# cl-volume-renderer/cl-volume-renderer

Hardware: AMD Instinct MI355X
Metric: msamples_per_sec (higher is better)
Workload: dtype f32

## Files before the change

### cl_volume_renderer_amd/csrc/bounce_device.hpp

```cpp
#pragma once
#include "render_device.hpp"

namespace clvr {

__device__ __forceinline__ VolumePacked make_volume(const RenderArgs &a) {
  return VolumePacked{a.grec, a.stepb, a.volume_lin, a.sdf_lin, a.X, a.Y, a.Z, a.NBX, a.NBY};
}

__device__ __forceinline__ uint32_t udivmod24(uint32_t n, uint32_t d, uint32_t &rem) {
  uint32_t q = (uint32_t)((float)n * __builtin_amdgcn_rcpf((float)d));
  uint32_t qd;
  asm("v_mul_u32_u24 %0, %1, %2" : "=v"(qd) : "v"(q), "v"(d));
  int32_t r = (int32_t)(n - qd);
  if (r < 0) { q -= 1u; r += (int32_t)d; }
  if (r >= (int32_t)d) { q += 1u; r -= (int32_t)d; }
  rem = (uint32_t)r;
  return q;
}

__device__ __forceinline__ unsigned prefix_count(unsigned long long mask) {
  return __builtin_amdgcn_mbcnt_hi((unsigned)(mask >> 32), __builtin_amdgcn_mbcnt_lo((unsigned)mask, 0u));
}
__device__ __forceinline__ unsigned lane_id() { return prefix_count(~0ull); }

enum : int { ST_IDLE = 0, ST_MARCH = 1, ST_CERT = 2, ST_EVENT = 8 };
enum : int { EV_START = 3,
             EV_HIT_COLOR_PENDING = 4,
             EV_CHECK = 5 };
constexpr int kCertNever = 255;

template <int MODE>
__device__ __forceinline__ void finish_item(const RenderArgs &a, int64_t entry, uint32_t hit, uint32_t gx, uint32_t gy,
                                            uint32_t bv_r, uint32_t bv_g, uint32_t bv_b) {
  const uint32_t cr = (bv_r / 2u) & 0xFFFFu, cg = (bv_g / 2u) & 0xFFFFu, cb = (bv_b / 2u) & 0xFFFFu;
  if (MODE == CLWH_ACCUM_VOXEL_CACHE && a.grants == nullptr) {
    cache_add(a.cache, entry, cr, cg, cb, 0u);
  } else {
    const unsigned long long packed = (unsigned long long)cr | ((unsigned long long)cg << 16) |
                                      ((unsigned long long)cb << 32) | (1ull << 48);
    atomicAdd(a.delta + hit, packed);
  }
  if (a.contrib_out) {
    uint32_t *q = a.contrib_out + ((size_t)gy * (size_t)a.launch_w + gx) * 4;
    q[0] = cr; q[1] = cg; q[2] = cb; q[3] = 1u;
  }
}

constexpr int kFixupDwords = 32;

__device__ __forceinline__ bool certify_exit(const RenderArgs &a, f3 p, f3 d, int budget, int &away) {
  const unsigned cx = min((unsigned)(int)p.x >> a.macro_shift, (unsigned)a.MNX - 1u), cy = min((unsigned)(int)p.y >> a.macro_shift, (unsigned)a.MNY - 1u),
                 cz = min((unsigned)(int)p.z >> a.macro_shift, (unsigned)a.MNZ - 1u);
  const unsigned octant = (d.x < 0.0f ? 1u : 0u) | (d.y < 0.0f ? 2u : 0u) | (d.z < 0.0f ? 4u : 0u);
  const int entry = a.macro[(((cz * (unsigned)a.MNY + cy) * (unsigned)a.MNX + cx) << 3) | octant];
  const bool refused = (entry & (int)kCertRefused) != 0;
  const int box_min = refused ? 0 : entry;
  away = refused ? ((entry & 0x7F) - 1) << a.macro_shift : 0;
  const float dmin = fminf(fminf(fabsf(d.x), fabsf(d.y)), fabsf(d.z));
  const float dsum = d.x + d.y + d.z;
  const float T = (float)((budget - 5) * box_min);
  const float fx = d.x < 0.0f ? p.x : (float)a.X - p.x, fy = d.y < 0.0f ? p.y : (float)a.Y - p.y, fz = d.z < 0.0f ? p.z : (float)a.Z - p.z;
  const bool leaves = T * fabsf(d.x) >= fx || T * fabsf(d.y) >= fy || T * fabsf(d.z) >= fz;
  return box_min != 0 && budget > 5 && leaves && dmin >= 0.0009765625f && dsum == dsum;
}
__device__ __forceinline__ bool certify_exit(const RenderArgs &a, f3 p, f3 d, int budget) {
  int away;
  return certify_exit(a, p, d, budget, away);
}

template <int SMALL>
__device__ __forceinline__ void index_tables_to_lds(VolumePacked &vol, const RenderArgs &a, int threads) {
  extern __shared__ uint32_t lds_parts[];
  if (SMALL == 2) {
    vol.parts = lds_parts;
    vol.parts_y0 = a.X;
    vol.parts_z0 = a.X + a.Y;
    for (int k = (int)threadIdx.x; k < a.X + a.Y + a.Z; k += threads)
      lds_parts[k] = k < a.X ? vol.part_x<1>((unsigned)k) : (k < a.X + a.Y ? vol.part_y<1>((unsigned)(k - a.X)) : vol.part_z<1>((unsigned)(k - a.X - a.Y)));
  }
}
__device__ __forceinline__ unsigned home_queue_of(const RenderArgs &a, unsigned waves_per_block) {
  unsigned home_queue = (unsigned)__builtin_amdgcn_s_getreg((3 << 11) | 20) & 7u;
  if (a.unit_affinity == 1) home_queue = (blockIdx.x * waves_per_block + (threadIdx.x >> 6)) & 7u;
  if (a.unit_affinity == 2) home_queue = 0u;
  return home_queue;
}

#ifdef CLVR_BOUNCE_STATS
constexpr bool kBounceStats = true;
#else
constexpr bool kBounceStats = false;
#endif
template <bool ON> struct BounceStatsT;
template <> struct BounceStatsT<false> {
  __device__ void step(int) {}
  __device__ void cert_begin(int, int) {}
  __device__ void cert_end(int, int) {}
  __device__ void closing_half(int) {}
  __device__ void event_phase(int) {}
  __device__ void refill(uint32_t) {}
  __device__ void fresh_items(int, int) {}
  __device__ void swap_point() {}
  template <bool TWO_RAYS> __device__ void flush(uint32_t *) {}
};
template <> struct BounceStatsT<true> {
  uint32_t step_iters = 0, step_lanes = 0, event_phases = 0, event_lanes = 0, refills = 0, refill_lanes = 0;
  uint32_t ev_kind[4] = {0, 0, 0, 0};
  uint32_t cert_phases = 0, cert_lanes = 0, cert_granted = 0;
  uint32_t step_idle = 0;
  uint32_t swaps = 0;
  uint32_t closing = 0, marching_before = 0;
  __device__ __forceinline__ void step(int st) {
    step_iters += 1; step_lanes += (uint32_t)__popcll(__ballot(st == ST_MARCH));
    step_idle += (uint32_t)__popcll(__ballot(st == ST_IDLE));
  }
  __device__ __forceinline__ void cert_begin(int st, int n_cert) {
    cert_phases += 1; cert_lanes += (uint32_t)n_cert;
    marching_before = (uint32_t)__popcll(__ballot(st == ST_MARCH));
  }
  __device__ __forceinline__ void cert_end(int st, int n_cert) { cert_granted += (uint32_t)(n_cert - (__popcll(__ballot(st == ST_MARCH)) - (int)marching_before)); }
  __device__ __forceinline__ void closing_half(int st) {
    closing = (uint32_t)__popcll(__ballot(st >= ST_EVENT));
    event_lanes += closing;
    ev_kind[1] += (uint32_t)__popcll(__ballot(st == ST_EVENT + EV_EXIT || st == ST_EVENT + EV_CHECK));
    ev_kind[2] += (uint32_t)__popcll(__ballot(st == ST_EVENT + EV_HIT || st == ST_EVENT + EV_HIT_COLOR_PENDING));
    ev_kind[3] += (uint32_t)__popcll(__ballot(st == ST_EVENT + EV_NONE));
  }
  __device__ __forceinline__ void event_phase(int st) {
    if (__ballot(st >= ST_EVENT) != 0ull) { event_phases += 1; event_lanes += (uint32_t)__popcll(__ballot(st >= ST_EVENT)); }
  }
  __device__ __forceinline__ void refill(uint32_t count) { refills += 1; refill_lanes += count; }
  __device__ __forceinline__ void fresh_items(int st, int o) {
    const uint32_t n_fresh = (uint32_t)__popcll(__ballot(st == ST_EVENT + EV_START && o == 1));
    ev_kind[0] += n_fresh; event_lanes += n_fresh;
    if (closing + n_fresh != 0u) event_phases += 1;
  }
  __device__ __forceinline__ void swap_point() { swaps += 1; }
  template <bool TWO_RAYS> __device__ __forceinline__ void flush(uint32_t *counters) {
    atomicAdd(&counters[CTR_STEP_ITERS], step_iters); atomicAdd(&counters[CTR_STEP_LANES], step_lanes);
    atomicAdd(&counters[CTR_EVENT_PHASES], event_phases); atomicAdd(&counters[CTR_EVENT_LANES], event_lanes);
    atomicAdd(&counters[CTR_REFILLS], refills); atomicAdd(&counters[CTR_REFILL_LANES], refill_lanes);
    if (TWO_RAYS) { atomicAdd(&counters[CTR_SWAPS], swaps); return; }
    for (int k = 0; k < 4; ++k) atomicAdd(&counters[CTR_EV_KIND + k], ev_kind[k]);
    atomicAdd(&counters[CTR_CERT_PHASES], cert_phases); atomicAdd(&counters[CTR_CERT_LANES], cert_lanes);
    atomicAdd(&counters[CTR_CERT_GRANTED], cert_granted); atomicAdd(&counters[CTR_STEP_IDLE], step_idle);
  }
};
using BounceStats = BounceStatsT<kBounceStats>;

}
```

### cl_volume_renderer_amd/csrc/clwh_context.hip

```cpp
#include <algorithm>
#include <cstdio>
#include <cstdlib>
#include <cstring>
#include <mutex>
#include <new>

#include "clwh_host.hpp"

using namespace clvr;

static thread_local int g_last_hip_error = 0;
void clvr::note_hip_error(hipError_t e) { g_last_hip_error = (int)e; }

static std::atomic<uint64_t> g_content_version{0};
static std::mutex g_cells_mutex;
static std::map<const void *, std::weak_ptr<VersionCell>> g_version_cells;
void clwh_touch(clwh_mem *m) { m->cell->v.store(++g_content_version, std::memory_order_relaxed); }

static std::shared_ptr<VersionCell> version_cell_of(const void *dptr) {
  std::lock_guard<std::mutex> lock(g_cells_mutex);
  auto it = g_version_cells.find(dptr);
  if (it != g_version_cells.end())
    if (auto live = it->second.lock()) return live;
  auto cell = std::make_shared<VersionCell>();
  g_version_cells[dptr] = cell;
  if (g_version_cells.size() > 4096) {
    for (auto i = g_version_cells.begin(); i != g_version_cells.end();)
      i = i->second.expired() ? g_version_cells.erase(i) : std::next(i);
  }
  return cell;
}

static size_t elem_size(int kind) {
  switch (kind) {
    case CLWH_ELEM_S8: case CLWH_ELEM_U8: return 1;
    case CLWH_ELEM_S16: case CLWH_ELEM_U16: return 2;
    case CLWH_ELEM_S32: case CLWH_ELEM_U32: case CLWH_ELEM_F32: return 4;
    default: return 0;
  }
}


void clvr::tf_to_dev(const clwh_tf &tf, TfDev &d) {
  std::memset(&d, 0, sizeof d);
  d.n = tf.n;
  for (int k = 0; k < tf.n; ++k) {
    const clwh_tf_rule &r = tf.rules[k];
    TfRuleDev &o = d.rules[k];
    o.v_lo = r.v_lo; o.v_hi = r.v_hi; o.g_lo = r.g_lo; o.g_hi = r.g_hi;
    o.flags = (r.use_gradient ? TF_USE_GRADIENT : 0u) | (r.writes_color ? TF_WRITES_COLOR : 0u) |
              (r.terminal ? TF_TERMINAL : 0u);
    o.color = ((uint32_t)r.color[0] & 255u) | (((uint32_t)r.color[1] & 255u) << 8) |
              (((uint32_t)r.color[2] & 255u) << 16) | (((uint32_t)r.color[3] & 255u) << 24);
    if (r.use_gradient) d.uses_gradient = 1;
  }
  for (int k = 0; k < tf.n && !d.uses_gradient; ++k) {
    const clwh_tf_rule &r = tf.rules[k];
    if (r.v_lo <= 0 && 0 <= r.v_hi) { d.border_class = k + 1; break; }
    if (r.terminal) break;
  }
}

int clvr::jit_for_source(clwh_ctx *ctx, const char *source, std::shared_ptr<JitTf> &out) {
  auto it = ctx->classes.cache.find(source);
  if (it != ctx->classes.cache.end()) {
    out = it->second;
    return CLWH_OK;
  }
  auto j = std::make_shared<JitTf>();
  j->source = source;
  std::string log;
  const int rc = tf_jit_compile(source, j->code, log);
  if (rc != CLWH_OK) {
    if (!log.empty()) std::fprintf(stderr, "clwhip: transfer-function source is neither in the rule grammar nor compilable:\n%s\n", log.c_str());
    return rc;
  }
  ctx->classes.cache[source] = j;
  out = j;
  return CLWH_OK;
}

int clvr::ensure_classes(clwh_ctx *ctx, const std::shared_ptr<JitTf> &jit, const clwh_mem *volume, TfDev &tf_out, const uint8_t **cls_out) {
  TfClasses &c = ctx->classes;
  if (c.cls.ptr && c.vol == volume->dptr && c.vol_ver == volume->version() && c.source == jit->source) {
    tf_out = c.tf;
    *cls_out = c.cls.as<uint8_t>();
    return CLWH_OK;
  }
  if (!jit->module) {
    HIP_TRY(hipModuleLoadData(&jit->module, jit->code.data()));
    HIP_TRY(hipModuleGetFunction(&jit->classify, jit->module, "clvr_tf_classify"));
  }
  const size_t voxels = volume->dims[0] * volume->dims[1] * volume->dims[2];
  CLWH_TRY(c.cls.reserve(ctx->stream, voxels));
  constexpr int kColors = CLWH_TF_MAX_RULES;
  CLWH_TRY(c.palette.reserve(ctx->stream, (kColors + 2) * sizeof(unsigned long long)));
  unsigned long long *palette = c.palette.as<unsigned long long>();
  HIP_TRY(hipMemsetAsync(palette, 0xFF, kColors * sizeof(unsigned long long), ctx->stream));
  HIP_TRY(hipMemsetAsync(palette + kColors, 0, 2 * sizeof(unsigned long long), ctx->stream));
  const void *vol = volume->dptr;
  int X = (int)volume->dims[0], Y = (int)volume->dims[1], Z = (int)volume->dims[2], max_colors = kColors;
  unsigned char *cls = c.cls.as<unsigned char>();
  int *error = reinterpret_cast<int *>(palette + kColors);
  int *border = reinterpret_cast<int *>(palette + kColors + 1);
  void *args[] = {&vol, &X, &Y, &Z, &cls, &palette, &max_colors, &error, &border};
  const size_t blocks = std::min<size_t>((voxels + 255u) / 256u, (size_t)1u << 23);
  HIP_TRY(hipModuleLaunchKernel(jit->classify, (unsigned)blocks, 1, 1, 256, 1, 1, 0, ctx->stream, args, nullptr));
  unsigned long long host[kColors + 2];
  HIP_TRY(hipMemcpyAsync(host, palette, sizeof host, hipMemcpyDeviceToHost, ctx->stream));
  HIP_TRY(hipStreamSynchronize(ctx->stream));
  c.vol = nullptr;
  if ((int)(host[kColors] & 0xFFFFFFFFull) != 0) return CLWH_ERR_TF_UNSUPPORTED;
  TfDev t;
  std::memset(&t, 0, sizeof t);
  t.opaque = 1;
  for (int k = 0; k < kColors && host[k] != ~0ull; ++k) {
    t.rules[k].flags = (host[k] >> 32) & 1ull ? TF_WRITES_COLOR : 0u;
    t.rules[k].color = (uint32_t)(host[k] & 0xFFFFFFFFull);
    t.n = k + 1;
  }
  t.border_class = (int32_t)(host[kColors + 1] & 0xFFull);
  c.tf = t;
  c.vol = volume->dptr;
  c.vol_ver = volume->version();
  c.source = jit->source;
  tf_out = t;
  *cls_out = cls;
  return CLWH_OK;
}


Tuning clvr::tuning_from_environment() {
  Tuning t;
  auto clamped = [](const char *e, int lo, int hi) { return std::max(lo, std::min(hi, std::atoi(e))); };
  if (const char *e = std::getenv("CLWH_TUNE_STEP")) t.step_min_lanes = clamped(e, 0, 64);
  if (const char *e = std::getenv("CLWH_TUNE_REFILL")) t.refill_min_lanes = clamped(e, 0, 64);
  if (const char *e = std::getenv("CLWH_TUNE_LITERAL_GRADIENT")) t.literal_gradient = std::atoi(e) != 0;
  if (const char *e = std::getenv("CLWH_TUNE_AFFINITY")) t.unit_affinity = std::atoi(e);
  if (const char *e = std::getenv("CLWH_TUNE_QUEUES")) t.unit_queues = clamped(e, 1, 8);
  if (const char *e = std::getenv("CLWH_TUNE_GROUP")) t.unit_group = std::max(1, std::atoi(e));
  if (const char *e = std::getenv("CLWH_TUNE_CHUNK_BLOCK_LOG2")) t.unit_block_log2 = clamped(e, 0, 8);
  if (const char *e = std::getenv("CLWH_TUNE_BLOCKS")) t.bounce_max_blocks = (uint32_t)std::max(1, std::atoi(e));
  if (const char *e = std::getenv("CLWH_TUNE_MACRO_SHIFT")) t.macro_shift = std::atoi(e);
  if (const char *e = std::getenv("CLWH_TUNE_LONG_LAUNCH")) t.force_long_launch = std::atoi(e) != 0;
  if (const char *e = std::getenv("CLWH_TUNE_BOUNCE_RAYS")) t.bounce_rays = std::atoi(e) == 2 ? 2 : 1;
  if (const char *e = std::getenv("CLWH_TUNE_SDF")) t.sdf_front = std::strcmp(e, "front") == 0;
  if (const char *e = std::getenv("CLWH_TUNE_SLICE_COARSE")) t.slice_coarse = std::atoi(e) != 0;
  if (const char *e = std::getenv("CLWH_TUNE_SDFBIT_WAVES")) t.sdfbit_waves = std::atoi(e) == 16 ? 16 : 8;
  if (const char *e = std::getenv("CLWH_TUNE_SDFBIT_GRID")) t.sdfbit_grid = std::max(1, std::atoi(e));
  if (const char *e = std::getenv("CLWH_TUNE_SDFBIT_REC")) t.sdfbit_rec_lds = std::strcmp(e, "lds") == 0 ? 1 : 0;
  if (const char *e = std::getenv("CLWH_TUNE_CERT")) t.cert_min_step = clamped(e, 0, 127);
  if (const char *e = std::getenv("CLWH_TUNE_CERT_HINT")) t.cert_hint = std::atoi(e) != 0;
  return t;
}

int clvr::check_device_flags(clwh_ctx *ctx) {
  PassScratch &p = ctx->pass;
  if (!p.fixup_overflow_pending || !p.sticky_flags.ptr) return CLWH_OK;
  uint32_t flag = 0;
  HIP_TRY(hipMemcpyAsync(&flag, p.sticky_flags.ptr, sizeof flag, hipMemcpyDeviceToHost, ctx->stream));
  HIP_TRY(hipStreamSynchronize(ctx->stream));
  p.fixup_overflow_pending = false;
  if (!flag) return CLWH_OK;
  HIP_TRY(hipMemsetAsync(p.sticky_flags.ptr, 0, sizeof(uint32_t), ctx->stream));
  return CLWH_ERR_INTERNAL_OVERFLOW;
}

int clvr::timed_begin(clwh_ctx *ctx, int which, hipEvent_t *end) {
  LaunchTimers &t = ctx->timers;
  if (!t.enabled) return CLWH_OK;
  if (t.used == t.pairs.size()) {
    LaunchTimers::Pair &fresh = t.pairs.emplace_back();
    int rc = fresh.begin.ensure(hipEventDefault);
    if (rc == CLWH_OK) rc = fresh.end.ensure(hipEventDefault);
    if (rc != CLWH_OK) {
      t.pairs.pop_back();
      return rc;
    }
  }
  LaunchTimers::Pair &p = t.pairs[t.used++];
  p.which = which;
  HIP_TRY(hipEventRecord(p.begin.ev, ctx->stream));
  *end = p.end.ev;
  return CLWH_OK;
}

static int order_streams(clwh_ctx *ctx, hipStream_t first, hipStream_t then) {
  HIP_TRY(hipSetDevice(ctx->device));
  CLWH_TRY(ctx->handoff.ensure(hipEventDisableTiming));
  HIP_TRY(hipEventRecord(ctx->handoff.ev, first));
  HIP_TRY(hipStreamWaitEvent(then, ctx->handoff.ev, 0));
  return CLWH_OK;
}

extern "C" {

int clwh_ctx_create_on_stream(int device, void *hip_stream, clwh_ctx **out) {
  if (!out) return CLWH_ERR_INVALID_VALUE;
  *out = nullptr;
  int count = 0;
  hipError_t e = hipGetDeviceCount(&count);
  if (e != hipSuccess || count <= 0) {
    note_hip_error(e);
    return CLWH_ERR_NO_DEVICE;
  }
  if (device < 0 || device >= count) return CLWH_ERR_NO_DEVICE;
  HIP_TRY(hipSetDevice(device));
  clwh_ctx *c = new (std::nothrow) clwh_ctx();
  if (!c) return CLWH_ERR_OUT_OF_MEMORY;
  c->device = device;
  c->stream = (hipStream_t)hip_stream;
  c->own_stream = false;
  c->tune = tuning_from_environment();
  *out = c;
  return CLWH_OK;
}

int clwh_ctx_create(int device, clwh_ctx **out) {
  CLWH_TRY(clwh_ctx_create_on_stream(device, nullptr, out));
  hipStream_t s;
  hipError_t e = hipStreamCreateWithFlags(&s, hipStreamNonBlocking);
  if (e != hipSuccess) {
    note_hip_error(e);
    delete *out;
    *out = nullptr;
    return CLWH_ERR_HIP;
  }
  (*out)->stream = s;
  (*out)->own_stream = true;
  return CLWH_OK;
}

int clwh_ctx_destroy(clwh_ctx *ctx) {
  if (!ctx) return CLWH_ERR_INVALID_VALUE;
  (void)hipSetDevice(ctx->device);
  (void)hipStreamSynchronize(ctx->stream);
  for (auto &kv : ctx->classes.cache)
    if (kv.second->module) (void)hipModuleUnload(kv.second->module);
  ctx->scene.reset();
  const hipStream_t owned = ctx->own_stream ? ctx->stream : nullptr;
  delete ctx;
  if (owned) (void)hipStreamDestroy(owned);
  return CLWH_OK;
}

int clwh_ctx_finish(clwh_ctx *ctx) {
  if (!ctx) return CLWH_ERR_INVALID_VALUE;
  HIP_TRY(hipStreamSynchronize(ctx->stream));
  return check_device_flags(ctx);
}

int clwh_ctx_acquire_from(clwh_ctx *ctx, void *hip_stream) {
  if (!ctx) return CLWH_ERR_INVALID_VALUE;
  return order_streams(ctx, (hipStream_t)hip_stream, ctx->stream);
}

int clwh_ctx_release_to(clwh_ctx *ctx, void *hip_stream) {
  if (!ctx) return CLWH_ERR_INVALID_VALUE;
  return order_streams(ctx, ctx->stream, (hipStream_t)hip_stream);
}

void *clwh_ctx_stream(clwh_ctx *ctx) { return ctx ? (void *)ctx->stream : nullptr; }
int clwh_ctx_device(clwh_ctx *ctx) { return ctx ? ctx->device : -1; }

int clwh_ctx_set_timing(clwh_ctx *ctx, int enabled) {
  if (!ctx) return CLWH_ERR_INVALID_VALUE;
  ctx->timers.enabled = enabled != 0;
  ctx->timers.used = 0;
  return CLWH_OK;
}

int clwh_ctx_timing_read_all(clwh_ctx *ctx, float *ms, int32_t *launches, int32_t n) {
  if (!ctx || !ms || !launches || n <= 0) return CLWH_ERR_INVALID_VALUE;
  for (int k = 0; k < n; ++k) { ms[k] = 0.0f; launches[k] = 0; }
  HIP_TRY(hipSetDevice(ctx->device));
  LaunchTimers &timers = ctx->timers;
  for (size_t i = 0; i < timers.used; ++i) {
    const LaunchTimers::Pair &p = timers.pairs[i];
    HIP_TRY(hipEventSynchronize(p.end.ev));
    float t = 0.0f;
    HIP_TRY(hipEventElapsedTime(&t, p.begin.ev, p.end.ev));
    if (p.which >= 0 && p.which < n) { ms[p.which] += t; launches[p.which] += 1; }
  }
  timers.used = 0;
  return CLWH_OK;
}

int clwh_ctx_timing_read(clwh_ctx *ctx, float *total_ms, int32_t *launches) {
  if (!ctx || !total_ms || !launches) return CLWH_ERR_INVALID_VALUE;
  float ms[CLWH_TIMER_COUNT];
  int32_t n[CLWH_TIMER_COUNT];
  const int rc = clwh_ctx_timing_read_all(ctx, ms, n, CLWH_TIMER_COUNT);
  *total_ms = ms[CLWH_TIMER_BOUNCE];
  *launches = n[CLWH_TIMER_BOUNCE];
  return rc;
}


static int mem_new(clwh_ctx *ctx, void *dptr, size_t bytes, bool owned, clwh_mem **out) {
  clwh_mem *m = new (std::nothrow) clwh_mem();
  if (!m) return CLWH_ERR_OUT_OF_MEMORY;
  m->ctx = ctx;
  m->dptr = dptr;
  m->bytes = bytes;
  m->owned = owned;
  m->cell = version_cell_of(dptr);
  touch(m);
  *out = m;
  return CLWH_OK;
}

int clwh_mem_create(clwh_ctx *ctx, size_t bytes, int flags, clwh_mem **out) {
  if (!ctx || !out || bytes == 0) return CLWH_ERR_INVALID_VALUE;
  *out = nullptr;
  HIP_TRY(hipSetDevice(ctx->device));
  DeviceBuffer fresh;
  CLWH_TRY(fresh.reserve(ctx->stream, bytes));
  CLWH_TRY(mem_new(ctx, fresh.ptr, bytes, true, out));
  (void)fresh.release();
  (*out)->flags = flags;
  return CLWH_OK;
}

int clwh_mem_wrap(clwh_ctx *ctx, void *device_ptr, size_t bytes, clwh_mem **out) {
  if (!ctx || !out || !device_ptr || bytes == 0) return CLWH_ERR_INVALID_VALUE;
  *out = nullptr;
  return mem_new(ctx, device_ptr, bytes, false, out);
}

static bool image_format_ok(int channels, int elem_kind) {
  return elem_size(elem_kind) != 0 && (channels == 1 || channels == 2 || channels == 4);
}

static int image_describe(clwh_mem *m, const size_t dims[3], int channels, int elem_kind) {
  if (!image_format_ok(channels, elem_kind)) return CLWH_ERR_INVALID_VALUE;
  m->is_image = true;
  for (int k = 0; k < 3; ++k) m->dims[k] = dims[k];
  m->channels = channels;
  m->elem_kind = elem_kind;
  return CLWH_OK;
}

static void image_dims(const size_t in[3], size_t d[3]) {
  for (int k = 0; k < 3; ++k) d[k] = in[k] == 0 ? 1 : in[k];
}

int clwh_image_create(clwh_ctx *ctx, const size_t dims[3], int channels, int elem_kind, int flags, clwh_mem **out) {
  if (!ctx || !out || !dims) return CLWH_ERR_INVALID_VALUE;
  *out = nullptr;
  if (!image_format_ok(channels, elem_kind)) return CLWH_ERR_INVALID_VALUE;
  size_t d[3];
  image_dims(dims, d);
  if (!(d[0] > 1)) return CLWH_ERR_INVALID_VALUE;
  const size_t bytes = d[0] * d[1] * d[2] * (size_t)channels * elem_size(elem_kind);
  CLWH_TRY(clwh_mem_create(ctx, bytes, flags, out));
  return image_describe(*out, d, channels, elem_kind);
}

int clwh_image_wrap(clwh_ctx *ctx, void *device_ptr, const size_t dims[3], int channels, int elem_kind, clwh_mem **out) {
  if (!ctx || !out || !dims || !device_ptr) return CLWH_ERR_INVALID_VALUE;
  *out = nullptr;
  const size_t es = elem_size(elem_kind);
  if (es == 0) return CLWH_ERR_INVALID_VALUE;
  size_t d[3];
  image_dims(dims, d);
  CLWH_TRY(mem_new(ctx, device_ptr, d[0] * d[1] * d[2] * (size_t)channels * es, false, out));
  const int rc = image_describe(*out, d, channels, elem_kind);
  if (rc != CLWH_OK) {
    delete *out;
    *out = nullptr;
  }
  return rc;
}

int clwh_mem_push(clwh_ctx *ctx, clwh_mem *mem, const void *host, size_t bytes) {
  if (!ctx || !mem || !host) return CLWH_ERR_INVALID_VALUE;
  if (bytes != mem->bytes) return CLWH_ERR_SIZE_MISMATCH;
  HIP_TRY(hipSetDevice(ctx->device));
  HIP_TRY(hipMemcpyAsync(mem->dptr, host, bytes, hipMemcpyHostToDevice, ctx->stream));
  HIP_TRY(hipStreamSynchronize(ctx->stream));
  touch(mem);
  return CLWH_OK;
}

int clwh_mem_pull(clwh_ctx *ctx, clwh_mem *mem, void *host, size_t bytes) {
  if (!ctx || !mem || !host) return CLWH_ERR_INVALID_VALUE;
  if (bytes != mem->bytes) return CLWH_ERR_SIZE_MISMATCH;
  HIP_TRY(hipSetDevice(ctx->device));
  HIP_TRY(hipMemcpyAsync(host, mem->dptr, bytes, hipMemcpyDeviceToHost, ctx->stream));
  HIP_TRY(hipStreamSynchronize(ctx->stream));
  return check_device_flags(ctx);
}

int clwh_mem_release(clwh_mem *mem) {
  if (!mem) return CLWH_ERR_INVALID_VALUE;
  int rc = CLWH_OK;
  if (mem->owned && mem->dptr) {
    (void)hipSetDevice(mem->ctx->device);
    (void)hipStreamSynchronize(mem->ctx->stream);
    hipError_t e = hipFree(mem->dptr);
    if (e != hipSuccess) {
      note_hip_error(e);
      rc = CLWH_ERR_HIP;
    }
  }
  delete mem;
  return rc;
}

int clwh_host_register(void *host, size_t bytes) {
  if (!host || bytes == 0) return CLWH_ERR_INVALID_VALUE;
  HIP_TRY(hipHostRegister(host, bytes, hipHostRegisterDefault));
  return CLWH_OK;
}

int clwh_host_unregister(void *host) {
  if (!host) return CLWH_ERR_INVALID_VALUE;
  HIP_TRY(hipHostUnregister(host));
  return CLWH_OK;
}

void *clwh_mem_device_ptr(clwh_mem *mem) { return mem ? mem->dptr : nullptr; }
size_t clwh_mem_size(clwh_mem *mem) { return mem ? mem->bytes : 0; }
int clwh_mem_mark_dirty(clwh_mem *mem) {
  if (!mem) return CLWH_ERR_INVALID_VALUE;
  touch(mem);
  return CLWH_OK;
}

int clwh_buffer_reset(clwh_ctx *ctx, clwh_mem *buffer_volume) {
  if (!ctx || !buffer_volume) return CLWH_ERR_INVALID_VALUE;
  HIP_TRY(hipSetDevice(ctx->device));
  HIP_TRY(hipMemsetAsync(buffer_volume->dptr, 0, buffer_volume->bytes, ctx->stream));
  touch(buffer_volume);
  return CLWH_OK;
}


const char *clwh_strerror(int status) {
  switch (status) {
    case CLWH_OK: return "CLWH_OK";
    case CLWH_ERR_INVALID_VALUE: return "CLWH_ERR_INVALID_VALUE";
    case CLWH_ERR_NO_DEVICE: return "CLWH_ERR_NO_DEVICE";
    case CLWH_ERR_OUT_OF_MEMORY: return "CLWH_ERR_OUT_OF_MEMORY";
    case CLWH_ERR_HIP: return "CLWH_ERR_HIP";
    case CLWH_ERR_UNKNOWN_KERNEL: return "CLWH_ERR_UNKNOWN_KERNEL";
    case CLWH_ERR_TF_UNSUPPORTED: return "CLWH_ERR_TF_UNSUPPORTED";
    case CLWH_ERR_BAD_ARGS: return "CLWH_ERR_BAD_ARGS";
    case CLWH_ERR_BAD_NDRANGE: return "CLWH_ERR_BAD_NDRANGE";
    case CLWH_ERR_SIZE_MISMATCH: return "CLWH_ERR_SIZE_MISMATCH";
    case CLWH_ERR_INTERNAL_OVERFLOW: return "CLWH_ERR_INTERNAL_OVERFLOW";
    default: return "CLWH_ERR_UNKNOWN";
  }
}

int clwh_last_hip_error(void) { return g_last_hip_error; }
const char *clwh_version(void) { return "clwhip 0.1 (gfx950)"; }

}
```

### cl_volume_renderer_amd/csrc/clwh_host.hpp

```cpp
#pragma once

#include <atomic>
#include <deque>
#include <map>
#include <memory>
#include <string>
#include <vector>

#include "clwh_internal.hpp"

namespace clvr {

void note_hip_error(hipError_t e);
inline int hip_failed(hipError_t e) {
  note_hip_error(e);
  return e == hipErrorOutOfMemory ? CLWH_ERR_OUT_OF_MEMORY : CLWH_ERR_HIP;
}
#define HIP_TRY(expr)                                   \
  do {                                                  \
    hipError_t _e = (expr);                             \
    if (_e != hipSuccess) return clvr::hip_failed(_e);  \
  } while (0)
#define CLWH_TRY(expr)                \
  do {                                \
    int _rc = (expr);                 \
    if (_rc != CLWH_OK) return _rc;   \
  } while (0)

struct NoCopy {
  NoCopy() = default;
  NoCopy(const NoCopy &) = delete;
  NoCopy &operator=(const NoCopy &) = delete;
};

struct DeviceBuffer : NoCopy {
  void *ptr = nullptr;
  size_t bytes = 0;
  ~DeviceBuffer() { if (ptr) (void)hipFree(ptr); }
  template <class T>
  T *as() const { return static_cast<T *>(ptr); }
  void *release() {
    void *p = ptr;
    ptr = nullptr;
    bytes = 0;
    return p;
  }
  int reserve(hipStream_t stream, size_t need, bool *reallocated = nullptr) {
    if (reallocated) *reallocated = bytes < need;
    if (bytes >= need) return CLWH_OK;
    if (ptr) {
      HIP_TRY(hipStreamSynchronize(stream));
      HIP_TRY(hipFree(ptr));
      (void)release();
    }
    HIP_TRY(hipMalloc(&ptr, need));
    bytes = need;
    return CLWH_OK;
  }
};

struct Event : NoCopy {
  hipEvent_t ev = nullptr;
  ~Event() { if (ev) (void)hipEventDestroy(ev); }
  int ensure(unsigned flags) {
    if (!ev) HIP_TRY(hipEventCreateWithFlags(&ev, flags));
    return CLWH_OK;
  }
};

struct PinnedWord : NoCopy {
  uint32_t *ptr = nullptr;
  ~PinnedWord() { if (ptr) (void)hipHostFree(ptr); }
  int ensure() {
    if (!ptr) HIP_TRY(hipHostMalloc((void **)&ptr, 64, hipHostMallocDefault));
    return CLWH_OK;
  }
};

int tf_jit_compile(const char *user_source, std::vector<char> &code, std::string &log);
struct JitTf {
  std::string source;
  std::vector<char> code;
  hipModule_t module = nullptr;
  hipFunction_t classify = nullptr;
};

struct PackedScene {
  int device = 0;
  DeviceBuffer data;
  const void *vol = nullptr, *sdf = nullptr;
  uint64_t vol_ver = 0, sdf_ver = 0;
  TfDev tf{};
  std::string tf_identity;
  int32_t macro_shift = 0;
  int32_t dims[3] = {0, 0, 0};
  uint64_t generation = 0;
  Event ready;
  bool stale = false;
  ~PackedScene();
};

struct VersionCell {
  std::atomic<uint64_t> v{0};
};


struct Tuning {
  int32_t step_min_lanes = 0;
  int32_t refill_min_lanes = 0;
  int32_t macro_shift = 0;
  int32_t bounce_rays = 1;
  int32_t force_long_launch = 0;
  int32_t literal_gradient = 0;
  int32_t unit_block_log2 = 4;
  int32_t unit_group = 1, unit_affinity = 0, unit_queues = 8;
  int32_t cert_hint = 1;
  int32_t cert_min_step = -1;
  uint32_t bounce_max_blocks = 2048;
  int32_t sdfbit_waves = 8;
  int32_t sdfbit_grid = 512;
  int32_t sdfbit_rec_lds = 0;
  int32_t sdf_front = 0;
  int32_t slice_coarse = 1;
};
Tuning tuning_from_environment();

struct PrimaryHits {
  struct Key {
    float cam_pos[3], cam_dir[3];
    int32_t frame_w, frame_h, launch_w, launch_h, tile_rank, tile_world;
    int64_t cache_entries;
    int32_t mode, shading;
    uint64_t packed_generation;
    const void *env;
    uint64_t env_version;
    int32_t env_w, env_h;
  } key{};
  bool valid = false;
  DeviceBuffer pix_slot, hits;
  uint32_t n_hits = 0;
  bool n_hits_known = false;
  PinnedWord host_n_hits;
  Event n_hits_event;
  bool n_hits_in_flight = false;
  uint32_t last_known_n_hits = 0;
};

struct PassScratch {
  static constexpr size_t kCounters = CTR_QUEUE_STRIDE * 9;
  DeviceBuffer counters;
  DeviceBuffer fixups, delta;
  DeviceBuffer sticky_flags;
  bool fixup_overflow_pending = false;
};

struct VoxelPlan {
  DeviceBuffer plan;
  DeviceBuffer temp;
  bool valid = false;
  uint32_t n = 0;
};

struct TfClasses {
  std::map<std::string, std::shared_ptr<JitTf>> cache;
  DeviceBuffer cls;
  DeviceBuffer palette;
  const void *vol = nullptr;
  uint64_t vol_ver = 0;
  std::string source;
  TfDev tf{};
};

struct SdfScratch {
  DeviceBuffer counters;
  DeviceBuffer flags;
  DeviceBuffer bits;
#ifdef CLVR_SDFBIT_TIMING
  DeviceBuffer timing;
#endif
};

struct GrowScratch {
  DeviceBuffer admissible, tiles, seeds;
  PinnedWord host;
};

struct ProjectionData {
  DeviceBuffer data;
  bool valid = false;
  const void *vol = nullptr;
  uint64_t vol_ver = 0;
  size_t dims[3] = {0, 0, 0};
  DeviceBuffer dilated;
  bool dilated_valid = false;
  DeviceBuffer mesh_counts, mesh_temp, mesh_points;
  DeviceBuffer lut_prefix;
  bool lut_valid = false;
  const void *lut = nullptr;
  uint64_t lut_ver = 0;
  int32_t lut_len = 0;
};

struct LaunchTimers {
  struct Pair {
    Event begin, end;
    int which = 0;
  };
  bool enabled = false;
  std::deque<Pair> pairs;
  size_t used = 0;
};

}

struct clwh_ctx {
  int device = 0;
  hipStream_t stream = nullptr;
  bool own_stream = false;
  clvr::Event handoff;
  clvr::Tuning tune;
  clvr::PrimaryHits primary;
  clvr::PassScratch pass;
  clvr::VoxelPlan vox;
  clvr::TfClasses classes;
  clvr::SdfScratch sdf;
  clvr::GrowScratch grow;
  clvr::ProjectionData proj;
  clvr::DeviceBuffer bilateral_weights;
  std::shared_ptr<clvr::PackedScene> scene;
  clvr::LaunchTimers timers;
};

struct clwh_mem {
  clwh_ctx *ctx = nullptr;
  void *dptr = nullptr;
  size_t bytes = 0;
  bool owned = false;
  bool is_image = false;
  size_t dims[3] = {1, 1, 1};
  int channels = 1;
  int elem_kind = CLWH_ELEM_U8;
  int flags = 0;
  std::shared_ptr<clvr::VersionCell> cell;
  uint64_t version() const { return cell ? cell->v.load(std::memory_order_relaxed) : 0; }
};

enum clwh_kernel_id {
  CLWH_K_EMPTY = 0,
  CLWH_K_RENDER,
  CLWH_K_SDF_BASE,
  CLWH_K_SDF_LAYER,
  CLWH_K_BUFFER_RESET,
  CLWH_K_FETCH_STATS,
  CLWH_K_APPLY_CLIP,
  CLWH_K_TF_SORT_VALUES,
  CLWH_K_TF_FLUSH_COLOR_FRAME,
  CLWH_K_BILATERAL_FILTER
};

struct clwh_kernel {
  clwh_ctx *ctx = nullptr;
  int id = CLWH_K_EMPTY;
  clwh_tf tf{};
  bool has_tf = false;
  std::shared_ptr<clvr::JitTf> jit;
};

void clwh_touch(clwh_mem *m);

namespace clvr {

inline void touch(clwh_mem *m) { clwh_touch(m); }

int check_device_flags(clwh_ctx *ctx);

void tf_to_dev(const clwh_tf &tf, TfDev &d);
int jit_for_source(clwh_ctx *ctx, const char *source, std::shared_ptr<JitTf> &out);
int ensure_classes(clwh_ctx *ctx, const std::shared_ptr<JitTf> &jit, const clwh_mem *volume, TfDev &tf_out, const uint8_t **cls_out);
inline int kernel_tf(clwh_kernel *k, const clwh_mem *volume, TfDev &tf_out, const uint8_t **cls_out) {
  if (k->jit) return ensure_classes(k->ctx, k->jit, volume, tf_out, cls_out);
  tf_to_dev(k->tf, tf_out);
  return CLWH_OK;
}

inline bool is_image(const clwh_mem *m, int dims_n, int channels, int elem_kind) {
  if (!m || !m->is_image || m->channels != channels || m->elem_kind != elem_kind) return false;
  if (dims_n == 2) return m->dims[2] == 1;
  return true;
}
inline bool is_plain_buffer(const clwh_mem *m) { return m && m->dptr && !m->is_image; }
inline bool same_dims(const clwh_mem *a, const clwh_mem *b) {
  return a->dims[0] == b->dims[0] && a->dims[1] == b->dims[1] && a->dims[2] == b->dims[2];
}
inline bool launch_size_ok(uint32_t w, uint32_t h) { return w != 0 && h != 0 && (w % 8) == 0 && (h % 8) == 0; }
inline bool fits_grid_yz(const clwh_mem *m) { return m->dims[1] <= 65535 && m->dims[2] <= 65535; }
inline bool dims_fit_int32(const clwh_mem *m) { return m->dims[0] <= 0x7fffffffu && m->dims[1] <= 0x7fffffffu && m->dims[2] <= 0x7fffffffu; }
inline void env_into_args(RenderArgs &a, const clwh_mem *env) {
  a.env = (const uint32_t *)env->dptr;
  a.env_w = (int32_t)env->dims[0];
  a.env_h = (int32_t)env->dims[1];
}

int ensure_projection_data(clwh_ctx *ctx, const clwh_mem *volume, ViewVolume &v);
int ensure_dilated_table(clwh_ctx *ctx, ViewVolume &v);

int timed_begin(clwh_ctx *ctx, int which, hipEvent_t *end);
template <class F>
int timed(clwh_ctx *ctx, int which, F &&launches) {
  hipEvent_t end = nullptr;
  CLWH_TRY(timed_begin(ctx, which, &end));
  HIP_TRY(launches());
  if (end) HIP_TRY(hipEventRecord(end, ctx->stream));
  return CLWH_OK;
}

}
```

### cl_volume_renderer_amd/csrc/clwh_internal.hpp

```cpp
#pragma once

#include <hip/hip_runtime.h>
#include <stdint.h>

#include "../../include/clwh.h"

namespace clvr {

struct TfRuleDev {
  int32_t v_lo, v_hi, g_lo, g_hi;
  uint32_t flags;
  uint32_t color;
};
struct TfDev {
  int32_t n;
  int32_t uses_gradient;
  int32_t literal_gradient_taps;
  int32_t opaque;
  int32_t border_class;
  TfRuleDev rules[CLWH_TF_MAX_RULES];
};

enum : uint32_t { TF_USE_GRADIENT = 1u, TF_WRITES_COLOR = 2u, TF_TERMINAL = 4u };

struct HitRec {
  float origin[3];
  float direction[3];
  float normal[3];
  uint32_t color;
  int32_t entry_lo;
  int32_t entry_hi;
  uint32_t xy;
  uint32_t pslot;
  uint32_t pad[2];
};
static_assert(sizeof(HitRec) == 64, "HitRec must be one 64-byte line");

enum : uint32_t { PIX_HIT = 0x80000000u };

constexpr uint32_t kCertMinStep = 2u;
constexpr uint32_t kCertRefused = 0x80u;

enum : uint32_t {
  CTR_HITS = 0, CTR_FIXUPS = 2,
  CTR_STEP_ITERS = 8, CTR_STEP_LANES, CTR_EVENT_PHASES, CTR_EVENT_LANES, CTR_REFILLS, CTR_REFILL_LANES,
  CTR_EV_KIND,
  CTR_CERT_PHASES = CTR_EV_KIND + 4, CTR_CERT_LANES, CTR_CERT_GRANTED,
  CTR_SWAPS, CTR_STEP_IDLE, CTR_STATS_END,
  CTR_QUEUE_STRIDE = 32,
};
struct RenderArgs {
  int32_t X, Y, Z;
  const uint2 *grec;
  const uint8_t *stepb;
  const int16_t *volume_lin;
  const int8_t *sdf_lin;
  const uint8_t *macro;
  int32_t MNX, MNY, MNZ, macro_shift;
  int32_t cert_min_step;
  int32_t cert_min_lanes;
  int32_t cert_hint;
  int32_t NBX, NBY;
  const uint32_t *env;
  int32_t env_w, env_h;
  uint32_t *cache;
  int64_t cache_entries;
  uint32_t *frame;
  int32_t frame_w, frame_h;
  int32_t launch_w, launch_h;
  int32_t tiles_x, tiles_y, tiles_per_row;
  int32_t tile_rank, tile_world;
  float cam_pos[3];
  float cam_dir[3];
  int32_t mode;
  float4 *accum;
  unsigned long long *delta;
  const uint32_t *grants;
  uint32_t *pix_slot;
  HitRec *hits;
  uint32_t *counters;
  uint32_t *fixups;
  uint32_t fixup_capacity;
  uint32_t *sticky_flags;
  uint32_t n_hits;
  uint32_t n_hits_estimate;
  int32_t n_hits_on_device;
  int32_t shading;
  int64_t *hit_index_out;
  uint32_t *contrib_out;
  uint32_t num_tile_slots;
  int32_t n_seeds;
  int32_t seeds[CLWH_MAX_SEEDS];
  int32_t step_min_lanes;
  int32_t refill_min_lanes;
  int32_t force_long_launch;
  int32_t bounce_rays;
  uint32_t bounce_max_blocks;
  int32_t unit_group;
  int32_t unit_block_log2;
  int32_t unit_queues;
  int32_t unit_affinity;
  TfDev tf;
};

struct RepackArgs {
  const int16_t *volume;
  const int8_t *sdf;
  int32_t X, Y, Z;
  int32_t NBX, NBY, NBZ;
  uint2 *grec;
  uint8_t *stepb;
  uint32_t *brick_min;
  const uint8_t *cls_in;
  TfDev tf;
};

struct SdfArgs {
  const int16_t *volume;
  int32_t X, Y, Z;
  int8_t *ping;
  int8_t *pong;
  int32_t max_iterations;
  int32_t iteration;
  int32_t *counters;
  int32_t *done;
  int32_t *counter_out;
  const uint8_t *cls_in;
  TfDev tf;
};

hipError_t launch_repack(const RepackArgs &a, hipStream_t s);
inline int macro_cell_shift(int X, int Y, int Z, int forced) {
  if (forced >= 3 && forced <= 8) return forced;
  auto cells = [&](int sh) { return (int64_t)((X >> sh) + 1) * ((Y >> sh) + 1) * ((Z >> sh) + 1); };
  int shift = 4;
  if (cells(4) > 40000) {
    shift = 5;
    while (shift < 8 && cells(shift) > 300000) ++shift;
  }
  return shift;
}
hipError_t launch_macro_table(const uint32_t *brick_min, int NBX, int NBY, int NBZ, uint8_t *macro, int X, int Y, int Z, int shift, hipStream_t s);
hipError_t launch_primary(const RenderArgs &a, hipStream_t s);
hipError_t launch_bounce(const RenderArgs &a, hipStream_t s);
inline bool bounce_queues_fit(uint32_t n_hits, int32_t unit_block_log2, int32_t n_seeds) {
  return (uint64_t)(((n_hits + 63u) >> 6) + 8u * (1u << unit_block_log2)) * (uint64_t)n_seeds < (1ull << 24);
}
hipError_t launch_env_fixup(const RenderArgs &a, hipStream_t s);
hipError_t launch_commit(const RenderArgs &a, hipStream_t s);
constexpr int64_t kVoxKeyInvalid = (int64_t)1 << 38;
constexpr int64_t kVoxKeyNone = ((int64_t)1 << 38) + 1;
hipError_t launch_vox_keys(const RenderArgs &a, int64_t *keys, uint32_t *iota, uint32_t n, hipStream_t s);
hipError_t launch_vox_grant(const RenderArgs &a, const int64_t *sorted_keys, const uint32_t *order, uint32_t n, uint32_t *grants, hipStream_t s);
hipError_t launch_commit_voxel(const RenderArgs &a, hipStream_t s);
hipError_t sort_entry_pairs(void *temp, size_t &temp_bytes, const int64_t *keys_in, int64_t *keys_out, const uint32_t *vals_in,
                            uint32_t *vals_out, size_t n, unsigned end_bit, hipStream_t s);
hipError_t launch_resolve(const RenderArgs &a, hipStream_t s);
hipError_t launch_ao(const RenderArgs &a, hipStream_t s);
hipError_t launch_accum_resolve(const RenderArgs &a, const float4 *accum_all, hipStream_t s);
hipError_t launch_accum_resolve_tiles(const RenderArgs &a, const float4 *accum, uint32_t *tiles_out, hipStream_t s);
hipError_t launch_frame_from_tiles(const RenderArgs &a, const uint32_t *tiles_all, hipStream_t s);
struct SdfFrontArgs {
  int8_t *sdf;
  int32_t X, Y, Z;
  int32_t TX, TY, TZ;
  const uint8_t *flags_cur;
  uint8_t *flags_next;
  uint8_t *flags_clear;
  uint8_t *tile_done;
  int32_t iteration;
  int32_t max_iterations;
  int32_t *counters;
};

struct SdfBitArgs {
  int8_t *sdf;
  const uint32_t *ev;
  const uint32_t *r_in;
  uint32_t *r_out;
  uint8_t *state;
  uint8_t *wake;
  int32_t launch;
  int32_t *presence;
  int32_t X, Y, Z, WP;
  int32_t BX, BY, BZ, core_z;
  int32_t r0, steps;
  uint32_t *planes;
  size_t plane_words;
  uint32_t *list;
  uint32_t *list_count;
  uint32_t *list_head;
#ifdef CLVR_SDFBIT_TIMING
  unsigned long long *timing;
#endif
};
void sdfbit_block_grid(int X, int Y, int Z, int waves, int32_t *BX, int32_t *BY, int32_t *BZ, int32_t *core_z);
hipError_t launch_sdfbit_events(const SdfArgs &a, uint32_t *ev, int32_t WP, hipStream_t s);
hipError_t launch_sdfbit_seed(const SdfBitArgs &a, hipStream_t s);
hipError_t launch_sdfbit_expand(const SdfBitArgs &a, const uint32_t *reached, int32_t max_iterations, hipStream_t s);
hipError_t launch_sdfbit_state(const SdfBitArgs &a, hipStream_t s);
hipError_t launch_sdfbit_layers(const SdfBitArgs &a, int waves, unsigned grid_blocks, bool rec_in_lds, hipStream_t s);

inline unsigned row_block(int X) { return X <= 64 ? 64u : (X <= 128 ? 128u : 256u); }
inline dim3 row_grid(int X, int Y, int Z) { return dim3(((unsigned)X + row_block(X) - 1u) / row_block(X), (unsigned)Y, (unsigned)Z); }
hipError_t launch_sdf_base(const SdfArgs &a, hipStream_t s);
hipError_t launch_sdf_base_front(const SdfArgs &a, uint8_t *flags, int32_t TX, int32_t TY, hipStream_t s);
hipError_t launch_sdf_front(const SdfFrontArgs &a, hipStream_t s);
hipError_t launch_sdf_layer(const SdfArgs &a, hipStream_t s);
hipError_t launch_fetch_stats(const int16_t *vol, int X, int Y, int Z, int32_t *stats, hipStream_t s);
hipError_t launch_tf_sort_values(const int16_t *vol, int X, int Y, int Z, uint32_t *frame, int width, int height,
                                 float min_v, float max_v, float min_g, float max_g, hipStream_t s);
hipError_t launch_tf_flush_color_frame(uint32_t *color_frame, int fw, int fh, const int32_t *frame, const int32_t *lookup,
                                       int lookup_len, hipStream_t s);
hipError_t launch_bilateral_filter(const int16_t *src, int X, int Y, int Z, int16_t *dst, const float *weights, hipStream_t s);
hipError_t launch_apply_clip(const int16_t *src, int SX, int SY, int SZ, int16_t *dst, int DX, int DY, int DZ,
                             const uint32_t *start, const uint32_t *len, hipStream_t s);


struct ViewVolume {
  const int16_t *bricks;
  const uint32_t *table, *dilated, *coarse;
  int32_t X, Y, Z, NBX, NBY, NBZ, CNX, CNY;
};
struct ViewFrame {
  uint32_t *frame;
  int32_t frame_w, frame_h;
  int32_t launch_w, launch_h, tiles_x, num_tiles;
};
struct ViewCamera {
  float cam_pos[3], cam_dir[3];
  float step, t_near, t_far;
  int32_t k_cap;
};

struct ProjRepackArgs {
  const int16_t *volume;
  int32_t X, Y, Z, NBX, NBY, NBZ;
  int16_t *bricks;
  uint32_t *table;
};
struct ProjArgs {
  ViewVolume vol;
  ViewFrame fr;
  ViewCamera cam;
  float window_center, window_width;
  float *values;
  float *t_extreme;
};
hipError_t launch_proj_repack(const ProjRepackArgs &a, hipStream_t s);
hipError_t launch_projection(const ProjArgs &a, int mode, bool dense, hipStream_t s);

struct CompArgs {
  ViewVolume vol;
  ViewFrame fr;
  ViewCamera cam;
  const float4 *lut;
  const uint32_t *prefix;
  int32_t lut_first, lut_len;
  float alpha_stop, ambient;
  float4 *rgba;
  float *t_first;
  float *t_stop;
};
hipError_t launch_comp_prefix(const float4 *lut, int32_t lut_len, uint32_t *prefix, hipStream_t s);
hipError_t launch_composite(const CompArgs &a, bool shade, bool dense, hipStream_t s);

struct IsoArgs {
  ViewVolume vol;
  ViewFrame fr;
  ViewCamera cam;
  int64_t threshold;
  int32_t skip_bound;
  int32_t refine;
  float color[3], ambient;
  float *t_hit;
  float4 *normal;
};
hipError_t launch_iso_dilate(const ViewVolume &v, uint32_t *dilated, hipStream_t s);
hipError_t launch_isosurface(const IsoArgs &a, bool below, bool dense, hipStream_t s);

struct SliceArgs {
  ViewVolume vol;
  ViewFrame fr;
  int32_t use_coarse;
  float origin[3], du[3], dv[3], normal[3];
  float step;
  float window_center, window_width;
  int32_t slab_samples;
  float *values;
  float *t_extreme;
};
hipError_t launch_slice(const SliceArgs &a, int mode, bool dense, hipStream_t s);

struct MeshArgs {
  ViewVolume vol;
  uint64_t n_bricks;
  int32_t lo[3], hi[3];
  int64_t threshold;
  int32_t in_bound;
  int32_t below, skip;
  uint64_t *counts;
  const uint64_t *bases;
  uint32_t *points;
  float *positions;
  float *normals;
  uint64_t *keys;
  uint32_t *triangles;
};
hipError_t launch_mesh_count(const MeshArgs &a, hipStream_t s);
hipError_t launch_mesh_scan(void *temp, size_t &temp_bytes, const uint64_t *counts, uint64_t *bases, size_t n, hipStream_t s);
hipError_t launch_mesh_fill(const MeshArgs &a, hipStream_t s);

constexpr int kGrowBatch = 8;
struct GrowDeviceResult {
  unsigned long long count, sum, sum_sq;
  int32_t vmin, vmax;
  uint32_t lo[3], hi[3];
};
struct GrowArgs {
  const int16_t *volume;
  unsigned long long *mask;
  unsigned long long *adm;
  int32_t X, Y, Z, W64;
  int32_t TX, TY, TZ;
  int32_t lo, hi;
  int32_t box_lo[3], box_hi[3];
  int32_t conn26, from_mask, dense;
  uint32_t *stamps;
  uint32_t *list;
  uint32_t *counters;
  const uint32_t *seeds;
  uint32_t n_seeds;
  GrowDeviceResult *result;
};
hipError_t launch_grow_admissible(const GrowArgs &a, hipStream_t s);
hipError_t launch_grow_seeds(const GrowArgs &a, hipStream_t s);
hipError_t launch_grow_round(const GrowArgs &a, uint32_t round, int slot, hipStream_t s);
hipError_t launch_grow_reduce(const GrowArgs &a, hipStream_t s);
hipError_t launch_apply_mask(const int16_t *in, int16_t *out, const unsigned long long *mask, int32_t X, int32_t Y, int32_t Z, int32_t W64,
                             int32_t fill, int32_t invert, hipStream_t s);

}
```

### cl_volume_renderer_amd/csrc/clwh_render.hip

```cpp
#include <algorithm>
#include <cstdio>
#include <cstring>
#include <mutex>

#include "clwh_host.hpp"

using namespace clvr;


static std::mutex g_scenes_mutex;
static std::vector<std::weak_ptr<PackedScene>> g_packed_scenes;
static std::atomic<uint64_t> g_packed_generation{0};

PackedScene::~PackedScene() {
  (void)hipSetDevice(device);
  (void)hipDeviceSynchronize();
}

struct PackedLayout {
  int X, Y, Z, NBX, NBY, NBZ, mshift, MNX, MNY, MNZ;
  size_t records, n_bricks, off_stepb, off_brick_min, off_macro, bytes;
};
static PackedLayout packed_layout(const clwh_mem *volume, int forced_macro_shift) {
  PackedLayout L;
  L.X = (int)volume->dims[0]; L.Y = (int)volume->dims[1]; L.Z = (int)volume->dims[2];
  L.NBX = (L.X + 7) / 8; L.NBY = (L.Y + 7) / 8; L.NBZ = (L.Z + 7) / 8;
  L.records = (size_t)L.NBX * L.NBY * L.NBZ * 512u;
  L.n_bricks = (size_t)L.NBX * L.NBY * L.NBZ;
  L.mshift = macro_cell_shift(L.X, L.Y, L.Z, forced_macro_shift);
  const int mcell = 1 << L.mshift;
  L.MNX = (L.X + mcell - 1) >> L.mshift; L.MNY = (L.Y + mcell - 1) >> L.mshift; L.MNZ = (L.Z + mcell - 1) >> L.mshift;
  L.off_stepb = L.records * sizeof(uint2);
  L.off_brick_min = (L.records * (sizeof(uint2) + 1u) + 15u) & ~(size_t)15u;
  L.off_macro = (L.off_brick_min + L.n_bricks * sizeof(uint32_t) + 15u) & ~(size_t)15u;
  L.bytes = L.off_macro + (size_t)L.MNX * L.MNY * L.MNZ * 8u;
  return L;
}

static bool packed_matches(const PackedScene &p, int device, const PackedLayout &L, const clwh_mem *volume, const clwh_mem *sdf,
                           const TfDev &tf, const std::string &tf_identity) {
  return !p.stale && p.device == device && p.data.bytes == L.bytes && p.macro_shift == L.mshift && p.vol == volume->dptr &&
         p.sdf == sdf->dptr && p.vol_ver == volume->version() && p.sdf_ver == sdf->version() &&
         !std::memcmp(&p.tf, &tf, sizeof tf) && p.tf_identity == tf_identity;
}

static int ensure_packed(clwh_ctx *ctx, const PackedLayout &L, const clwh_mem *volume, const clwh_mem *sdf, const TfDev &tf,
                         const uint8_t *cls_in, const std::string &tf_identity) {
  if (ctx->scene && packed_matches(*ctx->scene, ctx->device, L, volume, sdf, tf, tf_identity)) return CLWH_OK;
  std::shared_ptr<PackedScene> entry;
  {
    std::lock_guard<std::mutex> lock(g_scenes_mutex);
    for (auto it = g_packed_scenes.begin(); it != g_packed_scenes.end();) {
      std::shared_ptr<PackedScene> live = it->lock();
      if (!live) { it = g_packed_scenes.erase(it); continue; }
      if (!entry && packed_matches(*live, ctx->device, L, volume, sdf, tf, tf_identity)) entry = live;
      ++it;
    }
  }
  if (entry) {
    ctx->scene.reset();
    HIP_TRY(hipStreamWaitEvent(ctx->stream, entry->ready.ev, 0));
    ctx->scene = entry;
    return CLWH_OK;
  }
  if (ctx->scene && ctx->scene.use_count() == 1 && ctx->scene->data.bytes == L.bytes) {
    entry = ctx->scene;
  } else {
    ctx->scene.reset();
    entry = std::make_shared<PackedScene>();
    entry->device = ctx->device;
    CLWH_TRY(entry->data.reserve(ctx->stream, L.bytes));
    CLWH_TRY(entry->ready.ensure(hipEventDisableTiming));
  }
  ctx->scene.reset();
  {
    std::lock_guard<std::mutex> lock(g_scenes_mutex);
    entry->stale = true;
  }
  uint8_t *data = entry->data.as<uint8_t>();
  RepackArgs r;
  std::memset(&r, 0, sizeof r);
  r.volume = (const int16_t *)volume->dptr;
  r.sdf = (const int8_t *)sdf->dptr;
  r.X = L.X; r.Y = L.Y; r.Z = L.Z;
  r.NBX = L.NBX; r.NBY = L.NBY; r.NBZ = L.NBZ;
  r.grec = reinterpret_cast<uint2 *>(data);
  r.stepb = data + L.off_stepb;
  r.brick_min = reinterpret_cast<uint32_t *>(data + L.off_brick_min);
  HIP_TRY(hipMemsetAsync(r.brick_min, 0xFF, L.n_bricks * sizeof(uint32_t), ctx->stream));
  r.cls_in = cls_in;
  r.tf = tf;
  CLWH_TRY(timed(ctx, CLWH_TIMER_REPACK, [&] {
    const hipError_t e = launch_repack(r, ctx->stream);
    if (e != hipSuccess) return e;
    return launch_macro_table(r.brick_min, L.NBX, L.NBY, L.NBZ, data + L.off_macro, L.X, L.Y, L.Z, L.mshift, ctx->stream);
  }));
  HIP_TRY(hipEventRecord(entry->ready.ev, ctx->stream));
  ctx->scene = entry;
  {
    std::lock_guard<std::mutex> lock(g_scenes_mutex);
    entry->vol = volume->dptr;
    entry->sdf = sdf->dptr;
    entry->vol_ver = volume->version();
    entry->sdf_ver = sdf->version();
    entry->tf = tf;
    entry->tf_identity = tf_identity;
    entry->macro_shift = L.mshift;
    entry->dims[0] = L.X; entry->dims[1] = L.Y; entry->dims[2] = L.Z;
    entry->generation = ++g_packed_generation;
    entry->stale = false;
    bool listed = false;
    for (auto &w : g_packed_scenes)
      if (w.lock() == entry) listed = true;
    if (!listed) g_packed_scenes.push_back(entry);
  }
  return CLWH_OK;
}


static void describe_frame(RenderArgs &a, int32_t launch_w, int32_t launch_h, int32_t frame_w, int32_t frame_h,
                           int32_t rank, int32_t world, const float cam_pos[3], const float cam_dir[3]) {
  a.launch_w = launch_w;
  a.launch_h = launch_h;
  a.frame_w = frame_w;
  a.frame_h = frame_h;
  a.tiles_x = launch_w / 8;
  a.tiles_y = launch_h / 8;
  a.tile_rank = rank;
  a.tile_world = world;
  a.tiles_per_row = (a.tiles_x + world - 1) / world;
  a.num_tile_slots = (uint32_t)a.tiles_y * (uint32_t)a.tiles_per_row;
  for (int q = 0; q < 3; ++q) {
    a.cam_pos[q] = cam_pos[q];
    a.cam_dir[q] = cam_dir[q];
  }
}

static size_t pixel_slots(const RenderArgs &a) { return (size_t)a.num_tile_slots * 64u; }
static size_t launch_pixels(const RenderArgs &a) { return (size_t)a.launch_w * (size_t)a.launch_h; }
static bool is_planned(const RenderArgs &a) { return a.mode == CLWH_ACCUM_VOXEL_CACHE && a.n_seeds > 1; }

static int validate_desc(const clwh_render_desc *d) {
  if (!is_image(d->volume, 3, 1, CLWH_ELEM_S16) || !is_image(d->sdf, 3, 1, CLWH_ELEM_S8) ||
      !is_image(d->env, 2, 4, CLWH_ELEM_U8))
    return CLWH_ERR_BAD_ARGS;
  if (d->frame && !is_image(d->frame, 2, 4, CLWH_ELEM_U8)) return CLWH_ERR_BAD_ARGS;
  if (!same_dims(d->volume, d->sdf)) return CLWH_ERR_SIZE_MISMATCH;
  if (!launch_size_ok(d->width, d->height)) return CLWH_ERR_BAD_NDRANGE;
  if (d->width > 65535u || d->height > 65535u) return CLWH_ERR_BAD_NDRANGE;
  if (d->env->dims[0] > 32768u || d->env->dims[1] > 32768u) return CLWH_ERR_INVALID_VALUE;
  if (!dims_fit_int32(d->volume)) return CLWH_ERR_INVALID_VALUE;
  const int world = d->tile_world < 1 ? 1 : d->tile_world;
  if (d->tile_rank < 0 || d->tile_rank >= world) return CLWH_ERR_INVALID_VALUE;
  if (d->n_seeds < 0 || d->n_seeds > CLWH_MAX_SEEDS) return CLWH_ERR_INVALID_VALUE;
  if (d->n_seeds > 1 && d->contrib) return CLWH_ERR_BAD_ARGS;
  if (d->shading != CLWH_SHADE_LIGHT && d->shading != CLWH_SHADE_AO) return CLWH_ERR_INVALID_VALUE;
  if (d->shading == CLWH_SHADE_AO && d->accum_mode != CLWH_ACCUM_VOXEL_CACHE) return CLWH_ERR_BAD_ARGS;
  return CLWH_OK;
}

static int describe_launch(const clwh_ctx *ctx, const clwh_render_desc *d, RenderArgs &a) {
  std::memset(&a, 0, sizeof a);
  a.X = (int32_t)d->volume->dims[0];
  a.Y = (int32_t)d->volume->dims[1];
  a.Z = (int32_t)d->volume->dims[2];
  env_into_args(a, d->env);
  const int32_t fw = d->frame ? (int32_t)d->frame->dims[0] : (int32_t)d->width;
  const int32_t fh = d->frame ? (int32_t)d->frame->dims[1] : (int32_t)d->height;
  const int world = d->tile_world < 1 ? 1 : d->tile_world;
  describe_frame(a, (int32_t)d->width, (int32_t)d->height, fw, fh, d->tile_rank, world, d->cam_pos, d->cam_dir);
  a.frame = d->frame ? (uint32_t *)d->frame->dptr : nullptr;
  a.mode = d->accum_mode;
  a.shading = d->shading;
  if (a.mode == CLWH_ACCUM_VOXEL_CACHE) {
    if (!d->buffer_volume || d->buffer_volume->bytes < 8) return CLWH_ERR_BAD_ARGS;
    a.cache = (uint32_t *)d->buffer_volume->dptr;
    a.cache_entries = (int64_t)(d->buffer_volume->bytes / (d->shading == CLWH_SHADE_AO ? 4 : 8));
  } else if (a.mode == CLWH_ACCUM_IMAGE_SPACE) {
    const int64_t need = clwh_accum_len(d->width, d->height, world) * 16;
    if (!d->accum || (int64_t)d->accum->bytes < need) return CLWH_ERR_BAD_ARGS;
    a.accum = (float4 *)d->accum->dptr;
  } else {
    return CLWH_ERR_INVALID_VALUE;
  }
  if (d->hit_index) {
    if (d->hit_index->bytes < launch_pixels(a) * 8) return CLWH_ERR_SIZE_MISMATCH;
    a.hit_index_out = (int64_t *)d->hit_index->dptr;
  }
  if (d->contrib) {
    if (d->contrib->bytes < launch_pixels(a) * 16) return CLWH_ERR_SIZE_MISMATCH;
    a.contrib_out = (uint32_t *)d->contrib->dptr;
  }
  if (d->n_seeds > 0) {
    a.n_seeds = d->n_seeds;
    for (int q = 0; q < d->n_seeds; ++q) a.seeds[q] = d->seeds[q];
  } else {
    a.n_seeds = 1;
    a.seeds[0] = d->seed;
  }
  const Tuning &t = ctx->tune;
  a.step_min_lanes = t.step_min_lanes;
  a.refill_min_lanes = t.refill_min_lanes;
  a.force_long_launch = t.force_long_launch;
  a.bounce_rays = t.bounce_rays;
  a.bounce_max_blocks = t.bounce_max_blocks;
  a.unit_group = t.unit_group;
  a.unit_block_log2 = t.unit_block_log2;
  a.unit_affinity = t.unit_affinity;
  a.unit_queues = t.unit_queues;
  a.cert_hint = t.cert_hint;
  return CLWH_OK;
}

static int bind_scene(clwh_kernel *k, const clwh_render_desc *d, RenderArgs &a) {
  clwh_ctx *ctx = k->ctx;
  const uint8_t *cls_in = nullptr;
  CLWH_TRY(kernel_tf(k, d->volume, a.tf, &cls_in));
  a.tf.literal_gradient_taps = ctx->tune.literal_gradient;
  const PackedLayout L = packed_layout(d->volume, ctx->tune.macro_shift);
  CLWH_TRY(ensure_packed(ctx, L, d->volume, d->sdf, a.tf, cls_in, k->jit ? k->jit->source : std::string()));
  const uint8_t *packed = ctx->scene->data.as<uint8_t>();
  a.grec = reinterpret_cast<const uint2 *>(packed);
  a.NBX = L.NBX;
  a.NBY = L.NBY;
  a.stepb = packed + L.off_stepb;
  a.volume_lin = (const int16_t *)d->volume->dptr;
  a.sdf_lin = (const int8_t *)d->sdf->dptr;
  a.macro = packed + L.off_macro;
  a.macro_shift = L.mshift;
  a.MNX = L.MNX; a.MNY = L.MNY; a.MNZ = L.MNZ;
  bool zero_may_hit = a.tf.border_class != 0;
  for (int q = 0; q < a.tf.n && a.tf.uses_gradient && !a.tf.opaque; ++q)
    if (a.tf.rules[q].v_lo <= 0 && 0 <= a.tf.rules[q].v_hi) zero_may_hit = true;
  const int cert_auto = a.macro_shift < 4 ? 12 >> (4 - a.macro_shift) : std::min(12 << (a.macro_shift - 4), 48);
  a.cert_min_step = zero_may_hit ? 0 : (ctx->tune.cert_min_step >= 0 ? ctx->tune.cert_min_step : cert_auto);
  return CLWH_OK;
}

static int ensure_primary_hits(clwh_ctx *ctx, const clwh_render_desc *d, RenderArgs &a) {
  PrimaryHits &p = ctx->primary;
  PassScratch &s = ctx->pass;
  const size_t slots = pixel_slots(a);
  CLWH_TRY(p.pix_slot.reserve(ctx->stream, slots * sizeof(uint32_t)));
  CLWH_TRY(p.hits.reserve(ctx->stream, slots * sizeof(HitRec)));
  CLWH_TRY(s.counters.reserve(ctx->stream, PassScratch::kCounters * sizeof(uint32_t)));
  bool fresh_flags = false;
  CLWH_TRY(s.sticky_flags.reserve(ctx->stream, 64, &fresh_flags));
  if (fresh_flags) HIP_TRY(hipMemsetAsync(s.sticky_flags.ptr, 0, 64, ctx->stream));
  a.sticky_flags = s.sticky_flags.as<uint32_t>();
  a.pix_slot = p.pix_slot.as<uint32_t>();
  a.hits = p.hits.as<HitRec>();
  a.counters = s.counters.as<uint32_t>();

  PrimaryHits::Key key;
  std::memset(&key, 0, sizeof key);
  for (int q = 0; q < 3; ++q) {
    key.cam_pos[q] = a.cam_pos[q];
    key.cam_dir[q] = a.cam_dir[q];
  }
  key.frame_w = a.frame_w; key.frame_h = a.frame_h;
  key.launch_w = a.launch_w; key.launch_h = a.launch_h;
  key.tile_rank = a.tile_rank; key.tile_world = a.tile_world;
  key.cache_entries = a.cache_entries;
  key.mode = a.mode;
  key.shading = a.shading;
  key.packed_generation = ctx->scene->generation;
  key.env = d->env->dptr;
  key.env_version = d->env->version();
  key.env_w = a.env_w; key.env_h = a.env_h;
  if (p.valid && std::memcmp(&key, &p.key, sizeof key) == 0 && !a.hit_index_out) return CLWH_OK;
  p.valid = false;
  HIP_TRY(hipMemsetAsync(a.counters, 0, PassScratch::kCounters * sizeof(uint32_t), ctx->stream));
  CLWH_TRY(timed(ctx, CLWH_TIMER_PRIMARY, [&] { return launch_primary(a, ctx->stream); }));
  CLWH_TRY(p.host_n_hits.ensure());
  CLWH_TRY(p.n_hits_event.ensure(hipEventDisableTiming));
  HIP_TRY(hipMemcpyAsync(p.host_n_hits.ptr, a.counters + CTR_HITS, sizeof(uint32_t), hipMemcpyDeviceToHost, ctx->stream));
  HIP_TRY(hipEventRecord(p.n_hits_event.ev, ctx->stream));
  p.n_hits_in_flight = true;
  ctx->vox.valid = false;
  p.n_hits_known = false;
  p.key = key;
  p.valid = true;
  return CLWH_OK;
}

static int pick_up_hit_count(clwh_ctx *ctx, RenderArgs &a) {
  PrimaryHits &p = ctx->primary;
  if (p.n_hits_in_flight && !p.n_hits_known) {
    if (hipEventQuery(p.n_hits_event.ev) == hipSuccess) {
      p.n_hits = *p.host_n_hits.ptr;
      p.n_hits_known = true;
      p.n_hits_in_flight = false;
      p.last_known_n_hits = p.n_hits;
    } else {
      (void)hipGetLastError();
    }
  }
  const size_t slots = pixel_slots(a);
  a.n_hits_on_device = !p.n_hits_known;
  a.n_hits = p.n_hits_known ? p.n_hits : (uint32_t)std::min<size_t>(slots, 0xFFFFFFFFu);
  a.n_hits_estimate = a.n_hits;
  if (!p.n_hits_known && p.last_known_n_hits != 0)
    a.n_hits_estimate = (uint32_t)std::min<uint64_t>(a.n_hits, std::max<uint64_t>(2ull * p.last_known_n_hits, slots / 4u));
  if (!bounce_queues_fit(a.n_hits, ctx->tune.unit_block_log2, a.n_seeds)) return CLWH_ERR_INVALID_VALUE;
  return CLWH_OK;
}

static int size_pass_buffers(clwh_ctx *ctx, RenderArgs &a) {
  PassScratch &s = ctx->pass;
  const double rate = std::min(1.0, std::max(1.0 / 64.0, 3.0 * 8.0e-6 * (0.16 * a.env_w + 0.32 * a.env_h)));
  const size_t fix_cap = std::max<size_t>((size_t)((double)a.n_hits_estimate * (double)a.n_seeds * rate), 4096u);
  CLWH_TRY(s.fixups.reserve(ctx->stream, fix_cap * 128u));
  a.fixups = s.fixups.as<uint32_t>();
  a.fixup_capacity = (uint32_t)std::min<size_t>(s.fixups.bytes / 128u, 0x7fffffffu);
  if (a.mode == CLWH_ACCUM_IMAGE_SPACE || is_planned(a)) {
    bool fresh = false;
    CLWH_TRY(s.delta.reserve(ctx->stream, std::max<size_t>(pixel_slots(a), 1) * sizeof(unsigned long long), &fresh));
    a.delta = s.delta.as<unsigned long long>();
    if (fresh) HIP_TRY(hipMemsetAsync(s.delta.ptr, 0, s.delta.bytes, ctx->stream));
  }
  return CLWH_OK;
}

static int plan_voxel_grants(clwh_ctx *ctx, RenderArgs &a) {
  if (!is_planned(a)) return CLWH_OK;
  VoxelPlan &v = ctx->vox;
  constexpr size_t kPerElement = 2 * sizeof(int64_t) + 3 * sizeof(uint32_t);
  bool moved = false;
  CLWH_TRY(v.plan.reserve(ctx->stream, pixel_slots(a) * kPerElement, &moved));
  if (moved) v.valid = false;
  const size_t have = v.plan.bytes / kPerElement;
  int64_t *keys_in = v.plan.as<int64_t>(), *keys = keys_in + have;
  uint32_t *iota = reinterpret_cast<uint32_t *>(keys + have), *order = iota + have, *grants = order + have;
  if (!v.valid) {
    const uint32_t n = a.n_hits;
    HIP_TRY(launch_vox_keys(a, keys_in, iota, n, ctx->stream));
    size_t need = 0;
    HIP_TRY(sort_entry_pairs(nullptr, need, keys_in, keys, iota, order, n, 39u, ctx->stream));
    CLWH_TRY(v.temp.reserve(ctx->stream, std::max<size_t>(need, 16)));
    size_t tb = v.temp.bytes;
    HIP_TRY(sort_entry_pairs(v.temp.ptr, tb, keys_in, keys, iota, order, n, 39u, ctx->stream));
    v.valid = true;
    v.n = n;
  }
  HIP_TRY(launch_vox_grant(a, keys, order, v.n, grants, ctx->stream));
  a.grants = grants;
  return CLWH_OK;
}

#ifdef CLVR_BOUNCE_STATS
static int print_bounce_stats(clwh_ctx *ctx, const RenderArgs &a) {
  uint32_t h[CTR_STATS_END];
  HIP_TRY(hipMemcpyAsync(h, a.counters, sizeof h, hipMemcpyDeviceToHost, ctx->stream));
  HIP_TRY(hipStreamSynchronize(ctx->stream));
  auto per = [&](int sum, int n) { return h[n] ? (double)h[sum] / h[n] : 0.0; };
  std::fprintf(stderr, "[bounce stats] items=%llu step_iters=%u avg_march_lanes=%.2f event_phases=%u avg_event_lanes=%.2f "
               "refills=%u avg_refill=%.2f events start/exit/hit/none=%u/%u/%u/%u cert_phases=%u avg_cert_lanes=%.2f cert_granted=%u\n",
               (unsigned long long)h[CTR_HITS] * (unsigned long long)a.n_seeds, h[CTR_STEP_ITERS], per(CTR_STEP_LANES, CTR_STEP_ITERS),
               h[CTR_EVENT_PHASES], per(CTR_EVENT_LANES, CTR_EVENT_PHASES), h[CTR_REFILLS], per(CTR_REFILL_LANES, CTR_REFILLS), h[CTR_EV_KIND],
               h[CTR_EV_KIND + 1], h[CTR_EV_KIND + 2], h[CTR_EV_KIND + 3], h[CTR_CERT_PHASES], per(CTR_CERT_LANES, CTR_CERT_PHASES), h[CTR_CERT_GRANTED]);
  if (h[CTR_SWAPS]) std::fprintf(stderr, "[bounce stats] two rays per lane: %u swap points\n", h[CTR_SWAPS]);
  std::fprintf(stderr, "[bounce stats] per step iteration: avg_idle_lanes=%.2f (lane sum %u)\n", per(CTR_STEP_IDLE, CTR_STEP_ITERS), h[CTR_STEP_IDLE]);
  return CLWH_OK;
}
#endif

static int run_pass(clwh_ctx *ctx, const RenderArgs &a) {
  CLWH_TRY(timed(ctx, CLWH_TIMER_BOUNCE, [&] { return launch_bounce(a, ctx->stream); }));
#ifdef CLVR_BOUNCE_STATS
  CLWH_TRY(print_bounce_stats(ctx, a));
#endif
  CLWH_TRY(timed(ctx, CLWH_TIMER_FIXUP, [&] {
    hipError_t e = launch_env_fixup(a, ctx->stream);
    if (e == hipSuccess) e = launch_commit(a, ctx->stream);
    if (e == hipSuccess && is_planned(a)) e = launch_commit_voxel(a, ctx->stream);
    return e;
  }));
  ctx->pass.fixup_overflow_pending = true;
  return CLWH_OK;
}

extern "C" {

int64_t clwh_cache_len(uint32_t X, uint32_t Y, uint32_t Z) {
  return ((int64_t)X * Z * Y + (int64_t)X * Z + X + 1) * 4;
}

int64_t clwh_accum_len(uint32_t width, uint32_t height, int32_t tile_world) {
  if (tile_world < 1) tile_world = 1;
  const int64_t tiles_x = width / 8, tiles_y = height / 8;
  const int64_t tiles_per_row = (tiles_x + tile_world - 1) / tile_world;
  return tiles_y * tiles_per_row * 64;
}

int clwh_render(clwh_kernel *k, const clwh_render_desc *d) {
  if (!k || !d || k->id != CLWH_K_RENDER || !k->has_tf) return CLWH_ERR_INVALID_VALUE;
  clwh_ctx *ctx = k->ctx;
  RenderArgs a;
  CLWH_TRY(validate_desc(d));
  CLWH_TRY(describe_launch(ctx, d, a));
  HIP_TRY(hipSetDevice(ctx->device));
  CLWH_TRY(bind_scene(k, d, a));
  CLWH_TRY(ensure_primary_hits(ctx, d, a));
  CLWH_TRY(pick_up_hit_count(ctx, a));

  HIP_TRY(hipMemsetAsync(a.counters + CTR_HITS + 1, 0, (PassScratch::kCounters - CTR_HITS - 1) * sizeof(uint32_t), ctx->stream));
  if (a.contrib_out) HIP_TRY(hipMemsetAsync(a.contrib_out, 0, launch_pixels(a) * 16, ctx->stream));

  if (d->resolve_only) {
    if (!a.frame) return CLWH_ERR_BAD_ARGS;
  } else if (d->shading == CLWH_SHADE_AO) {
    CLWH_TRY(timed(ctx, CLWH_TIMER_AO, [&] { return launch_ao(a, ctx->stream); }));
  } else {
    CLWH_TRY(size_pass_buffers(ctx, a));
    CLWH_TRY(plan_voxel_grants(ctx, a));
    CLWH_TRY(run_pass(ctx, a));
  }
  if ((d->write_frame || d->resolve_only) && a.frame)
    CLWH_TRY(timed(ctx, CLWH_TIMER_RESOLVE, [&] { return launch_resolve(a, ctx->stream); }));
  if (d->frame) touch(d->frame);
  return CLWH_OK;
}


int clwh_accum_resolve(clwh_ctx *ctx, clwh_mem *accum_all, int32_t tile_world, uint32_t width, uint32_t height,
                       clwh_mem *frame, clwh_mem *env, const float cam_pos[3], const float cam_dir[3]) {
  if (!ctx || !accum_all || !frame || !env || !cam_pos || !cam_dir || tile_world < 1) return CLWH_ERR_INVALID_VALUE;
  if (!is_image(frame, 2, 4, CLWH_ELEM_U8) || !is_image(env, 2, 4, CLWH_ELEM_U8)) return CLWH_ERR_BAD_ARGS;
  if (!launch_size_ok(width, height)) return CLWH_ERR_BAD_NDRANGE;
  const int64_t need = clwh_accum_len(width, height, tile_world) * 16 * tile_world;
  if ((int64_t)accum_all->bytes < need) return CLWH_ERR_SIZE_MISMATCH;
  RenderArgs a;
  std::memset(&a, 0, sizeof a);
  describe_frame(a, (int32_t)width, (int32_t)height, (int32_t)frame->dims[0], (int32_t)frame->dims[1], 0, tile_world,
                 cam_pos, cam_dir);
  a.frame = (uint32_t *)frame->dptr;
  env_into_args(a, env);
  HIP_TRY(hipSetDevice(ctx->device));
  CLWH_TRY(timed(ctx, CLWH_TIMER_RESOLVE, [&] { return launch_accum_resolve(a, (const float4 *)accum_all->dptr, ctx->stream); }));
  touch(frame);
  return CLWH_OK;
}

int clwh_accum_resolve_tiles(clwh_ctx *ctx, clwh_mem *accum, int32_t tile_rank, int32_t tile_world, uint32_t width, uint32_t height,
                             clwh_mem *tiles_rgba8, clwh_mem *env, const float cam_pos[3], const float cam_dir[3]) {
  if (!ctx || !accum || !tiles_rgba8 || !env || !cam_pos || !cam_dir || tile_world < 1 || tile_rank < 0 || tile_rank >= tile_world)
    return CLWH_ERR_INVALID_VALUE;
  if (!is_image(env, 2, 4, CLWH_ELEM_U8)) return CLWH_ERR_BAD_ARGS;
  if (!launch_size_ok(width, height)) return CLWH_ERR_BAD_NDRANGE;
  const int64_t n = clwh_accum_len(width, height, tile_world);
  if ((int64_t)accum->bytes < n * 16 || (int64_t)tiles_rgba8->bytes < n * 4) return CLWH_ERR_SIZE_MISMATCH;
  RenderArgs a;
  std::memset(&a, 0, sizeof a);
  describe_frame(a, (int32_t)width, (int32_t)height, (int32_t)width, (int32_t)height, tile_rank, tile_world, cam_pos, cam_dir);
  env_into_args(a, env);
  HIP_TRY(hipSetDevice(ctx->device));
  CLWH_TRY(timed(ctx, CLWH_TIMER_RESOLVE, [&] {
    return launch_accum_resolve_tiles(a, (const float4 *)accum->dptr, (uint32_t *)tiles_rgba8->dptr, ctx->stream);
  }));
  touch(tiles_rgba8);
  return CLWH_OK;
}

int clwh_frame_from_tiles(clwh_ctx *ctx, clwh_mem *tiles_all, int32_t tile_world, uint32_t width, uint32_t height, clwh_mem *frame) {
  if (!ctx || !tiles_all || !frame || tile_world < 1) return CLWH_ERR_INVALID_VALUE;
  if (!is_image(frame, 2, 4, CLWH_ELEM_U8)) return CLWH_ERR_BAD_ARGS;
  if (!launch_size_ok(width, height)) return CLWH_ERR_BAD_NDRANGE;
  if ((int64_t)tiles_all->bytes < clwh_accum_len(width, height, tile_world) * 4 * tile_world) return CLWH_ERR_SIZE_MISMATCH;
  const float zero[3] = {0.0f, 0.0f, 0.0f};
  RenderArgs a;
  std::memset(&a, 0, sizeof a);
  describe_frame(a, (int32_t)width, (int32_t)height, (int32_t)frame->dims[0], (int32_t)frame->dims[1], 0, tile_world, zero, zero);
  a.frame = (uint32_t *)frame->dptr;
  HIP_TRY(hipSetDevice(ctx->device));
  HIP_TRY(launch_frame_from_tiles(a, (const uint32_t *)tiles_all->dptr, ctx->stream));
  touch(frame);
  return CLWH_OK;
}


int clwh_ctx_invalidate_derived(clwh_ctx *ctx, int what) {
  if (!ctx) return CLWH_ERR_INVALID_VALUE;
  if ((what & CLWH_DERIVED_SCENE) && ctx->scene) {
    {
      std::lock_guard<std::mutex> lock(g_scenes_mutex);
      ctx->scene->stale = true;
    }
    if (ctx->scene.use_count() > 1) ctx->scene.reset();
  }
  if (what & (CLWH_DERIVED_SCENE | CLWH_DERIVED_CAMERA)) ctx->primary.valid = false;
  if (what & CLWH_DERIVED_PROJECTION) ctx->proj.valid = ctx->proj.lut_valid = ctx->proj.dilated_valid = false;
  return CLWH_OK;
}

int clwh_ctx_scene_info(clwh_ctx *ctx, uint64_t *scene_id, uint64_t *bytes, int32_t *holders) {
  if (!ctx) return CLWH_ERR_INVALID_VALUE;
  std::lock_guard<std::mutex> lock(g_scenes_mutex);
  if (scene_id) *scene_id = ctx->scene ? ctx->scene->generation : 0;
  if (bytes) *bytes = ctx->scene ? ctx->scene->data.bytes : 0;
  if (holders) *holders = ctx->scene ? (int32_t)ctx->scene.use_count() : 0;
  return CLWH_OK;
}

int clwh_debug_macro_table(clwh_ctx *ctx, void *host_out, uint64_t capacity, int32_t info_out[4]) {
  if (!ctx || !info_out) return CLWH_ERR_INVALID_VALUE;
  if (!ctx->scene) return CLWH_ERR_BAD_ARGS;
  PackedLayout L;
  {
    std::lock_guard<std::mutex> lock(g_scenes_mutex);
    clwh_mem shape{};
    for (int q = 0; q < 3; ++q) shape.dims[q] = (size_t)ctx->scene->dims[q];
    L = packed_layout(&shape, ctx->scene->macro_shift);
  }
  info_out[0] = L.MNX; info_out[1] = L.MNY; info_out[2] = L.MNZ; info_out[3] = L.mshift;
  const size_t bytes = L.bytes - L.off_macro;
  if (!host_out) return CLWH_OK;
  if (capacity < bytes || ctx->scene->data.bytes != L.bytes) return CLWH_ERR_SIZE_MISMATCH;
  HIP_TRY(hipSetDevice(ctx->device));
  HIP_TRY(hipMemcpyAsync(host_out, ctx->scene->data.as<uint8_t>() + L.off_macro, bytes, hipMemcpyDeviceToHost, ctx->stream));
  HIP_TRY(hipStreamSynchronize(ctx->stream));
  return CLWH_OK;
}

}
```

### cl_volume_renderer_amd/csrc/primary_kernels.hip

```cpp
#include "bounce_device.hpp"

namespace clvr {

template <bool USE_GRAD>
__global__ __launch_bounds__(64) void k_primary(const RenderArgs a) {
  const uint32_t slot = xcd_contiguous_slot(blockIdx.x, a.num_tile_slots);
  int tx, ty;
  if (!tile_from_slot(a, slot, tx, ty)) return;
  const uint32_t lane = threadIdx.x;
  const uint32_t x = (uint32_t)tx * 8u + (lane & 7u);
  const uint32_t y = (uint32_t)ty * 8u + (lane >> 3);
  const uint32_t pslot = slot * 64u + lane;

  const VolumePacked vol = make_volume(a);
  const f3 cam_o = f3{a.cam_pos[0], a.cam_pos[1], a.cam_pos[2]};
  const f3 cam_d = f3{a.cam_dir[0], a.cam_dir[1], a.cam_dir[2]};
  const Ray vray = generate_ray(cam_o, cam_d, (int)x, (int)y, a.frame_w, a.frame_h);
  const float dx = (float)a.X, dy = (float)a.Y, dz = (float)a.Z;

  bool cut_ok;
  f3 cut_point;
  if (!(within(vray.origin.x, dx) && within(vray.origin.y, dy) && within(vray.origin.z, dz))) {
    cut_ok = cut_box(dx, dy, dz, vray, cut_point);
  } else {
    cut_ok = true;
    cut_point = vray.origin;
  }

  bool hit = false;
  Ray current_ray{cut_point, vray.direction};
  uint32_t current_color = 0u;
  if (cut_ok) {
    int ev;
    current_ray = march_to_next_event<USE_GRAD>(vol, a.tf, current_ray, ev, current_color);
    hit = (ev == EV_HIT);
  }

  const unsigned long long hit_mask = __ballot(hit);
  uint32_t base = 0u;
  if (hit_mask != 0ull) {
    const int leader = __ffsll((long long)hit_mask) - 1;
    if ((int)lane == leader) base = atomicAdd(&a.counters[CTR_HITS], (uint32_t)__popcll(hit_mask));
    base = __shfl(base, leader);
  }

  int64_t raw_entry = -1;
  if (hit) {
    const uint32_t h = base + prefix_count(hit_mask);
    const f3 normal = -normalize3(gradient_nn(vol, current_ray.origin));
    raw_entry = cache_entry_of(a.X, a.Z, current_ray.origin);
    int64_t entry = raw_entry;
    if (a.mode == CLWH_ACCUM_VOXEL_CACHE && !(entry >= 0 && entry < a.cache_entries)) entry = -2;
    uint4 q0, q1, q2, q3;
    q0.x = __float_as_uint(current_ray.origin.x); q0.y = __float_as_uint(current_ray.origin.y);
    q0.z = __float_as_uint(current_ray.origin.z); q0.w = __float_as_uint(current_ray.direction.x);
    q1.x = __float_as_uint(current_ray.direction.y); q1.y = __float_as_uint(current_ray.direction.z);
    q1.z = __float_as_uint(normal.x); q1.w = __float_as_uint(normal.y);
    q2.x = __float_as_uint(normal.z); q2.y = current_color;
    q2.z = (uint32_t)((uint64_t)entry & 0xFFFFFFFFull); q2.w = (uint32_t)((uint64_t)entry >> 32);
    q3.x = x | (y << 16); q3.y = pslot; q3.z = 0u; q3.w = 0u;
    uint4 *dst = reinterpret_cast<uint4 *>(&a.hits[h]);
    dst[0] = q0; dst[1] = q1; dst[2] = q2; dst[3] = q3;
    a.pix_slot[pslot] = PIX_HIT | h;
  } else {
    const uint32_t e = sample_environment_map(a.env, a.env_w, a.env_h, vray.direction);
    a.pix_slot[pslot] = e & 0x00FFFFFFu;
  }
  if (a.hit_index_out) a.hit_index_out[(size_t)y * (size_t)a.launch_w + x] = raw_entry;
}

template <bool USE_GRAD>
__global__ __launch_bounds__(256) void k_ao(const RenderArgs a) {
  const uint32_t n_hits = a.n_hits_on_device ? a.counters[CTR_HITS] : a.n_hits;
  const uint32_t h = blockIdx.x * blockDim.x + threadIdx.x;
  if (h >= n_hits) return;
  const VolumePacked vol = make_volume(a);
  const uint4 *src = reinterpret_cast<const uint4 *>(&a.hits[h]);
  const uint4 q0 = src[0], q1 = src[1], q2 = src[2], q3 = src[3];
  const f3 hit_origin = f3{__uint_as_float(q0.x), __uint_as_float(q0.y), __uint_as_float(q0.z)};
  const f3 hit_direction = f3{__uint_as_float(q0.w), __uint_as_float(q1.x), __uint_as_float(q1.y)};
  const f3 normal = f3{__uint_as_float(q1.z), __uint_as_float(q1.w), __uint_as_float(q2.x)};
  const int64_t entry = (int64_t)(((uint64_t)q2.w << 32) | (uint64_t)q2.z);
  const uint32_t gx = q3.x & 0xFFFFu, gy = q3.x >> 16;
  if (entry < 0) return;
  uint32_t *word = a.cache + entry;
  for (int s = 0; s < a.n_seeds; ++s) {
    const uint32_t old = atomicAdd(word, 1u);
    uint32_t granted = 1u, occluded = 0u;
    if ((old & 0xFFFFu) >= 100u) {
      atomicSub(word, 1u);
      granted = 0u;
    } else {
      Ray r{hit_origin + hit_direction, hemisphere_direction(gx, gy, normal, a.seeds[s])};
      for (int k = 0; k < 7; ++k) {
        const int sd = (int)(vol.step_i(f2i(r.origin.x), f2i(r.origin.y), f2i(r.origin.z)) & 0x7Fu);
        r.origin = r.origin + r.direction * cl_max((float)sd, 0.5f);
      }
      int ev;
      uint32_t color = 0u;
      march_to_next_event<USE_GRAD>(vol, a.tf, r, ev, color);
      if (ev == EV_HIT) {
        atomicAdd(word, 0x10000u);
        occluded = 1u;
      }
    }
    if (a.contrib_out) {
      uint32_t *q = a.contrib_out + ((size_t)gy * (size_t)a.launch_w + gx) * 4;
      q[0] = occluded; q[1] = 0u; q[2] = 0u; q[3] = granted;
    }
  }
}

hipError_t launch_primary(const RenderArgs &a, hipStream_t s) {
  if (a.tf.uses_gradient)
    hipLaunchKernelGGL(k_primary<true>, dim3(a.num_tile_slots), dim3(64), 0, s, a);
  else
    hipLaunchKernelGGL(k_primary<false>, dim3(a.num_tile_slots), dim3(64), 0, s, a);
  return hipGetLastError();
}
hipError_t launch_ao(const RenderArgs &a, hipStream_t s) {
  if (a.n_hits == 0) return hipSuccess;
  const dim3 grid((a.n_hits + 255u) / 256u), block(256);
  if (a.tf.uses_gradient) hipLaunchKernelGGL(k_ao<true>, grid, block, 0, s, a);
  else hipLaunchKernelGGL(k_ao<false>, grid, block, 0, s, a);
  return hipGetLastError();
}

}
```

### cl_volume_renderer_amd/csrc/render_kernels.hip

```cpp
#include <algorithm>

#include "bounce_two_rays.hpp"

namespace clvr {

#ifndef CLVR_CERT_PHASE_MIN_LANES
#define CLVR_CERT_PHASE_MIN_LANES 16
#endif
constexpr int kCertPhaseMinLanes = CLVR_CERT_PHASE_MIN_LANES;
#ifndef CLVR_BOUNCE_WAVES_PER_SIMD
#define CLVR_BOUNCE_WAVES_PER_SIMD 7
#endif
#ifndef CLVR_BOUNCE_THREADS
#define CLVR_BOUNCE_THREADS 256
#endif
constexpr int kBounceThreads = CLVR_BOUNCE_THREADS;

template <bool USE_GRAD, int MODE, bool SMALL_VOLUME>
__global__ __launch_bounds__(kBounceThreads, CLVR_BOUNCE_WAVES_PER_SIMD) void k_bounce(const RenderArgs a) {
  constexpr int SMALL = SMALL_VOLUME ? 2 : 0;
  VolumePacked vol = make_volume(a);
  index_tables_to_lds<SMALL>(vol, a, kBounceThreads);
  __shared__ float div255[256];
  if (threadIdx.x < 256u) div255[threadIdx.x] = (float)threadIdx.x / 255.0f;
  __syncthreads();
  const uint32_t n_hits = a.n_hits_on_device ? a.counters[CTR_HITS] : a.n_hits;
  const uint32_t n_chunks = (n_hits + 63u) >> 6;
  const unsigned lane = lane_id();
  const unsigned home_queue = home_queue_of(a, (unsigned)(kBounceThreads / 64));
  unsigned queue_dry = 0u;
  enum : int { C_START_X, C_START_Y, C_START_Z,
               C_NORMAL_X, C_NORMAL_Y, C_NORMAL_Z,
               C_ENTRY_LO, C_ENTRY_HI, C_PIXEL, C_HIT, C_SEED,
               C_FIX,
               C_BV_R, C_BV_G, C_BV_B, C_FIELDS };
  __shared__ uint32_t cold[C_FIELDS][kBounceThreads];
#define COLD(f) cold[f][threadIdx.x]
  Ray ray{{0, 0, 0}, {0, 0, 0}};
  float atten = 0.0f, r_energy = 0.0f, g_energy = 0.0f, b_energy = 0.0f;
  uint32_t color = 0u;
  int o = 0, i = 0;
  int st = ST_IDLE;
  int sd = 0;
  uint32_t march = 0u;
  constexpr uint32_t kOneStep = 1u << 24, kCertReady = 1u << 23;
  const bool cert_hint = a.cert_hint != 0;
  const int cert_min_lanes = a.cert_min_lanes;
  const int cert_at = a.cert_min_step != 0 ? a.cert_min_step : kCertNever;
  bool exhausted = false;
  BounceStats stats;

  for (;;) {
    if (__ballot(st == ST_MARCH) != 0ull) {
      do {
        stats.step(st);
        if (st == ST_MARCH) {
          ray.origin = ray.origin + ray.direction * fmaxf((float)sd, 0.5f);
          march += (uint32_t)sd - kOneStep;
          if (!USE_GRAD) {
            const bool has_voxel = __float_as_uint(ray.origin.x) < __float_as_uint((float)a.X) &&
                                   __float_as_uint(ray.origin.y) < __float_as_uint((float)a.Y) &&
                                   __float_as_uint(ray.origin.z) < __float_as_uint((float)a.Z);
            if (has_voxel) {
              const unsigned q = vol.template step_marched<SMALL>(ray.origin.x, ray.origin.y, ray.origin.z);
              sd = (int)(q & 0x7Fu);
              if (q & 0x80u) st = ST_EVENT + EV_HIT_COLOR_PENDING;
              else if (march < kOneStep) st = ST_EVENT + EV_NONE;
              else if (sd >= cert_at && (march & kCertReady)) st = ST_CERT;
            } else {
              st = ST_EVENT + EV_CHECK;
            }
          } else if (exited_volume(vol, ray.origin)) {
            st = ST_EVENT + EV_EXIT;
          } else {
            int next_sd;
            bool pending = false;
            const bool is_hit = classify_step<USE_GRAD, SMALL, true>(vol, a.tf, ray.origin, color, next_sd, &pending);
            if (is_hit) {
              st = ST_EVENT + (pending ? EV_HIT_COLOR_PENDING : EV_HIT);
            } else if (march < kOneStep) {
              st = ST_EVENT + EV_NONE;
            } else {
              sd = next_sd;
              if (sd >= cert_at && (march & kCertReady)) st = ST_CERT;
            }
          }
        }
        const int n_cert = __popcll(__ballot(st == ST_CERT));
        if (n_cert != 0 && (n_cert >= cert_min_lanes || __popcll(__ballot(st == ST_MARCH)) < a.step_min_lanes)) {
          stats.cert_begin(st, n_cert);
          if (st == ST_CERT) {
            int away;
            if (certify_exit(a, ray.origin, ray.direction, (int)(march >> 24), away)) {
              st = ST_EVENT + EV_EXIT;
            } else {
              march = (march & ~(kOneStep - 1u)) | (kCertReady - (uint32_t)(cert_hint ? away : 0));
              st = ST_MARCH;
            }
          }
          stats.cert_end(st, n_cert);
        }
      } while (__popcll(__ballot(st == ST_MARCH)) >= a.step_min_lanes);
    }

    stats.closing_half(st);
    if (st >= ST_EVENT) {
      int ev = st - ST_EVENT;
      if (ev == EV_CHECK) {
        for (;;) {
          if (exited_volume(vol, ray.origin)) { ev = EV_EXIT; break; }
          int next_sd;
          bool pending = false;
          if (classify_step<USE_GRAD, SMALL, true>(vol, a.tf, ray.origin, color, next_sd, &pending)) {
            ev = pending ? EV_HIT_COLOR_PENDING : EV_HIT;
            break;
          }
          if (march < kOneStep) { ev = EV_NONE; break; }
          ray.origin = ray.origin + ray.direction * fmaxf((float)next_sd, 0.5f);
          march -= kOneStep;
        }
      }
      bool ended = false;

      if (ev == EV_EXIT) {
        const float factor = i == 8 ? 8.0f / 8.0f : (i == 9 ? 8.0f / 9.0f : (i == 10 ? 8.0f / 10.0f : 8.0f / (float)i));
        const float p_r = atten * r_energy, p_g = atten * g_energy, p_b = atten * b_energy;
        uint32_t light = 0u;
        const uint32_t fix_word = COLD(C_FIX);
        int fix = (int)(fix_word >> 2) - 2, npend = (int)(fix_word & 3u);
        bool certain = (fix == -1) && sample_environment_map_fast(a.env, a.env_w, a.env_h, ray.direction, light);
        if (certain) {
          COLD(C_BV_R) = f2u((float)COLD(C_BV_R) + p_r * (float)(light & 255u) * factor / 1.0f);
          COLD(C_BV_G) = f2u((float)COLD(C_BV_G) + p_g * (float)((light >> 8) & 255u) * factor / 1.0f);
          COLD(C_BV_B) = f2u((float)COLD(C_BV_B) + p_b * (float)((light >> 16) & 255u) * factor / 1.0f);
        } else {
          if (fix == -1) {
            const uint32_t slot = atomicAdd(&a.counters[CTR_FIXUPS], 1u);
            if (slot < a.fixup_capacity) {
              fix = (int)slot;
              uint32_t *rec = a.fixups + (size_t)slot * kFixupDwords;
              rec[0] = COLD(C_HIT);
              rec[1] = COLD(C_ENTRY_LO);
              rec[2] = COLD(C_ENTRY_HI);
              rec[3] = COLD(C_PIXEL);
              rec[4] = COLD(C_BV_R); rec[5] = COLD(C_BV_G); rec[6] = COLD(C_BV_B);
            } else {
              a.sticky_flags[0] = 1u;
              fix = -2;
            }
          }
          if (fix >= 0) {
            uint32_t *e = a.fixups + (size_t)fix * kFixupDwords + 8 + 7 * npend;
            e[0] = __float_as_uint(p_r); e[1] = __float_as_uint(p_g); e[2] = __float_as_uint(p_b);
            e[3] = __float_as_uint(factor);
            e[4] = __float_as_uint(ray.direction.x); e[5] = __float_as_uint(ray.direction.y);
            e[6] = __float_as_uint(ray.direction.z);
            npend += 1;
          }
          COLD(C_FIX) = ((uint32_t)(fix + 2) << 2) | (uint32_t)npend;
        }
        o += 1;
        ev = EV_START;
        ended = true;
      } else if (ev == EV_HIT || ev == EV_HIT_COLOR_PENDING) {
        i += 1;
        if (i > 10) {
          o += 1;
          ended = true;
        }
      } else if (ev == EV_NONE) {
        i += 1;
        if (i > 10) {
          o += 1;
          ev = EV_START;
          ended = true;
        }
      }

      if (ended && o > 2) {
        const int fix = (int)(COLD(C_FIX) >> 2) - 2;
        if (fix == -1)
          finish_item<MODE>(a, (int64_t)(((uint64_t)COLD(C_ENTRY_HI) << 32) | (uint64_t)COLD(C_ENTRY_LO)), COLD(C_HIT), COLD(C_PIXEL) & 0xFFFFu,
                            COLD(C_PIXEL) >> 16, COLD(C_BV_R), COLD(C_BV_G), COLD(C_BV_B));
        else if (fix >= 0) a.fixups[(size_t)fix * kFixupDwords + 7] = COLD(C_FIX) & 3u;
        st = ST_IDLE;
      } else {
        st = ST_EVENT + ev;
      }
    }

    const unsigned long long idle_mask = __ballot(st == ST_IDLE);
    const uint32_t n_idle = (uint32_t)__popcll(idle_mask);
    if (!exhausted && n_idle >= (uint32_t)a.refill_min_lanes) {
      const uint32_t NQ = (uint32_t)a.unit_queues, S = (uint32_t)a.n_seeds, G = (uint32_t)a.unit_group;
      const uint32_t KB = (uint32_t)a.unit_block_log2, n_blocks = (n_chunks + (1u << KB) - 1u) >> KB;
      uint32_t base = 0u, count = 0u, q_sel = 0u;
      if (lane == 0u) {
        for (uint32_t tries = 0; tries < NQ && count == 0u; ++tries) {
          const uint32_t q = (home_queue + tries) % NQ;
          const uint32_t blocks_q = (n_blocks + NQ - 1u - q) / NQ;
          const uint32_t chunks_q = blocks_q << KB;
          if (chunks_q == 0u || ((queue_dry >> q) & 1u)) continue;
          const uint32_t total = chunks_q * S * 64u;
          const uint32_t p = atomicAdd(&a.counters[CTR_QUEUE_STRIDE * (q + 1u)], n_idle);
          if (p + n_idle >= total) queue_dry |= 1u << q;
          if (p < total) {
            base = p;
            count = min(n_idle, total - p);
            q_sel = q;
          }
        }
      }
      base = __shfl(base, 0);
      count = __shfl(count, 0);
      q_sel = __shfl(q_sel, 0);
      stats.refill(count);
      if (count == 0u) {
        exhausted = true;
      } else if (st == ST_IDLE) {
        const uint32_t rank = (uint32_t)__popcll(idle_mask & ((1ull << lane) - 1ull));
        if (rank < count) {
          const uint32_t item = base + rank, p = item >> 6;
          const uint32_t chunks_q = ((n_blocks + NQ - 1u - q_sel) / NQ) << KB;
          uint32_t r, c_in;
          const uint32_t g = udivmod24(p, G * S, r);
          const uint32_t in_group = min(G, chunks_q - g * G);
          const uint32_t s = udivmod24(r, in_group, c_in), ch = g * G + c_in;
          const uint32_t chunk = ((q_sel + NQ * (ch >> KB)) << KB) + (ch & ((1u << KB) - 1u));
          const uint32_t h = chunk * 64u + (item & 63u);
          if (h < n_hits) {
            const uint4 *src = reinterpret_cast<const uint4 *>(&a.hits[h]);
            const uint4 q0 = src[0], q1 = src[1], q2 = src[2], q3 = src[3];
            const f3 hit_origin = f3{__uint_as_float(q0.x), __uint_as_float(q0.y), __uint_as_float(q0.z)};
            const f3 hit_direction = f3{__uint_as_float(q0.w), __uint_as_float(q1.x), __uint_as_float(q1.y)};
            const f3 start = hit_origin + hit_direction;
            color = q2.y;
            const int64_t entry = (int64_t)(((uint64_t)q2.w << 32) | (uint64_t)q2.z);
            bool granted = true;
            if (MODE == CLWH_ACCUM_VOXEL_CACHE)
              granted = a.grants ? s < a.grants[h] : (entry >= 0 && cache_take_token(a.cache, entry, 256u));
            if (granted) {
              COLD(C_START_X) = __float_as_uint(start.x); COLD(C_START_Y) = __float_as_uint(start.y); COLD(C_START_Z) = __float_as_uint(start.z);
              COLD(C_NORMAL_X) = q1.z; COLD(C_NORMAL_Y) = q1.w; COLD(C_NORMAL_Z) = q2.x;
              COLD(C_ENTRY_LO) = q2.z; COLD(C_ENTRY_HI) = q2.w;
              COLD(C_PIXEL) = q3.x;
              COLD(C_HIT) = h;
              COLD(C_SEED) = (uint32_t)a.seeds[s];
              COLD(C_FIX) = (uint32_t)(-1 + 2) << 2;
              COLD(C_BV_R) = 0u; COLD(C_BV_G) = 0u; COLD(C_BV_B) = 0u;
              r_energy = div255[color & 255u];
              g_energy = div255[(color >> 8) & 255u];
              b_energy = div255[(color >> 16) & 255u];
              o = 1;
              st = ST_EVENT + EV_START;
            } else if (a.contrib_out) {
              uint32_t *q = a.contrib_out + ((size_t)(q3.x >> 16) * (size_t)a.launch_w + (q3.x & 0xFFFFu)) * 4;
              q[0] = 0u; q[1] = 0u; q[2] = 0u; q[3] = 0u;
            }
          }
        }
      }
    }
    stats.fresh_items(st, o);
    if (__ballot(st != ST_IDLE) == 0ull) {
      if (exhausted && lane == 0u) stats.flush<false>(a.counters);
      if (exhausted) break;
      continue;
    }

    if (st >= ST_EVENT) {
      const int ev = st - ST_EVENT;
      bool start_path = (ev == EV_START);
      bool bounce = false, from_hit = false;
      f3 bn{0, 0, 0}, bstart{0, 0, 0};
      int bseed = 0;

      if (ev == EV_HIT || ev == EV_HIT_COLOR_PENDING) {
        bn = -normalize3(hit_gradient_and_color<SMALL>(vol, a.tf, ray.origin, ev == EV_HIT_COLOR_PENDING, color));
        bstart = ray.origin + ray.direction;
        bseed = o + i - 1;
        bounce = true;
        from_hit = true;
        if (i > 10) {
          r_energy *= div255[color & 255u];
          g_energy *= div255[(color >> 8) & 255u];
          b_energy *= div255[(color >> 16) & 255u];
          bounce = false;
          start_path = true;
        }
      }

      if (start_path) {
        bn = f3{__uint_as_float(COLD(C_NORMAL_X)), __uint_as_float(COLD(C_NORMAL_Y)), __uint_as_float(COLD(C_NORMAL_Z))};
        bstart = f3{__uint_as_float(COLD(C_START_X)), __uint_as_float(COLD(C_START_Y)), __uint_as_float(COLD(C_START_Z))};
        bseed = o;
        bounce = true;
        from_hit = false;
      }

      if (bounce) {
        const float roughness = div255[color >> 24];
        const uint32_t pixel = COLD(C_PIXEL);
        Ray nr;
        nr.direction = hemisphere_reflective(pixel & 0xFFFFu, pixel >> 16, bn, (int)COLD(C_SEED) + bseed, roughness);
        nr.origin = bstart + bn * 2.0f;
        const float d = fabsf(dot3(nr.direction, bn));
        if (from_hit) {
          atten *= d;
          r_energy *= div255[color & 255u];
          g_energy *= div255[(color >> 8) & 255u];
          b_energy *= div255[(color >> 16) & 255u];
        } else {
          atten = d;
          i = 8;
        }
        ray = nr;
      }

      sd = (int)(vol.template step_i<SMALL>(f2i(ray.origin.x), f2i(ray.origin.y), f2i(ray.origin.z)) & 0x7Fu);
      march = 70u * kOneStep + kCertReady;
      st = ST_MARCH;
    }
  }
#undef COLD
}

hipError_t launch_bounce(const RenderArgs &a_in, hipStream_t s) {
  RenderArgs a = a_in;
  const uint64_t total = (uint64_t)a.n_hits * (uint64_t)a.n_seeds;
  if (total == 0) return hipSuccess;
  const uint64_t waves_needed = (total + 63u) / 64u;
  constexpr unsigned wpb = (unsigned)kBounceThreads / 64u;
  const unsigned blocks = (unsigned)std::min<uint64_t>((waves_needed + wpb - 1u) / wpb, ((uint64_t)a.bounce_max_blocks * 4u + wpb - 1u) / wpb);
  const dim3 grid(blocks), block(kBounceThreads);
  const uint64_t waves_likely = ((uint64_t)a.n_hits_estimate * (uint64_t)a.n_seeds + 63u) / 64u;
  const bool long_launch = a.force_long_launch || waves_likely >= 6u * (uint64_t)blocks * wpb;
  if (a.step_min_lanes <= 0) a.step_min_lanes = long_launch ? 16 : 1;
  if (a.refill_min_lanes <= 0) a.refill_min_lanes = long_launch ? 16 : 64;
  a.cert_min_lanes = kCertPhaseMinLanes;
  if (!long_launch) a.cert_min_step = 0;
  if (!bounce_queues_fit(a.n_hits, a.unit_block_log2, a.n_seeds)) return hipErrorInvalidValue;
  const bool g = a.tf.uses_gradient != 0;
  const bool small = (uint64_t)a.NBX * (uint64_t)a.NBY * (uint64_t)((a.Z + 7) / 8) < (1ull << 23) &&
                     a.X + a.Y + a.Z <= VolumePacked::kPartsMaxEntries;
  const size_t lds_parts_bytes = small ? (size_t)(a.X + a.Y + a.Z) * sizeof(uint32_t) : 0u;
  const bool two_rays = a.bounce_rays == 2 && long_launch && a.n_hits < (1u << 26) && kBounceThreads == 256;
  if (two_rays) a.fixup_capacity = std::min<uint32_t>(a.fixup_capacity, (1u << 27) - 4u);
#define CLVR_LAUNCH_BOUNCE(G, M)                                                                    \
  do {                                                                                              \
    if (two_rays) {                                                                                 \
      if (small) hipLaunchKernelGGL((k_bounce2<G, M, true>), grid, block, lds_parts_bytes, s, a);  \
      else hipLaunchKernelGGL((k_bounce2<G, M, false>), grid, block, 0, s, a);                     \
    } else if (small) hipLaunchKernelGGL((k_bounce<G, M, true>), grid, block, lds_parts_bytes, s, a); \
    else hipLaunchKernelGGL((k_bounce<G, M, false>), grid, block, 0, s, a);                        \
  } while (0)
  if (a.mode == CLWH_ACCUM_VOXEL_CACHE) {
    if (g) CLVR_LAUNCH_BOUNCE(true, CLWH_ACCUM_VOXEL_CACHE);
    else CLVR_LAUNCH_BOUNCE(false, CLWH_ACCUM_VOXEL_CACHE);
  } else {
    if (g) CLVR_LAUNCH_BOUNCE(true, CLWH_ACCUM_IMAGE_SPACE);
    else CLVR_LAUNCH_BOUNCE(false, CLWH_ACCUM_IMAGE_SPACE);
  }
#undef CLVR_LAUNCH_BOUNCE
  return hipGetLastError();
}

}
```

### cl_volume_renderer_amd/csrc/scene_kernels.hip

```cpp
#include "render_device.hpp"

namespace clvr {

#ifndef CLVR_REPACK_X
#define CLVR_REPACK_X 64
#endif
constexpr int kRepackX = CLVR_REPACK_X;
constexpr int kRepackPitch = kRepackX + 16;
constexpr int kRepackX0 = 8;
__global__ __launch_bounds__(256) void k_repack(const RepackArgs a) {
  __shared__ __attribute__((aligned(16))) int16_t s_val[10][10][kRepackPitch];
  __shared__ __attribute__((aligned(16))) int8_t s_sdf[8][8][kRepackX];
  const int x0 = (int)blockIdx.x * kRepackX, y0 = (int)blockIdx.y * 8, z0 = (int)blockIdx.z * 8;
  const unsigned tid = threadIdx.x;
  if ((a.X & 15) == 0 && x0 + kRepackX <= a.X && ((reinterpret_cast<uintptr_t>(a.volume) | reinterpret_cast<uintptr_t>(a.sdf)) & 15u) == 0u) {
    constexpr unsigned kChunks = kRepackX / 8;
    for (unsigned i = tid; i < 10u * 10u * kChunks; i += 256u) {
      const unsigned row = i / kChunks, c = i % kChunks;
      const int ry = (int)(row % 10u), rz = (int)(row / 10u);
      const int y = y0 - 1 + ry, z = z0 - 1 + rz;
      uint4 v = uint4{0u, 0u, 0u, 0u};
      int16_t left = 0, right = 0;
      if ((unsigned)y < (unsigned)a.Y && (unsigned)z < (unsigned)a.Z) {
        const int16_t *src = a.volume + ((size_t)z * (size_t)a.Y + (size_t)y) * (size_t)a.X + (size_t)x0;
        v = *reinterpret_cast<const uint4 *>(src + 8 * c);
        if (c == 0u && x0 > 0) left = src[-1];
        if (c == kChunks - 1u && x0 + kRepackX < a.X) right = src[kRepackX];
      }
      *reinterpret_cast<uint4 *>(&s_val[rz][ry][kRepackX0 + 8 * (int)c]) = v;
      if (c == 0u) s_val[rz][ry][kRepackX0 - 1] = left;
      if (c == kChunks - 1u) s_val[rz][ry][kRepackX0 + kRepackX] = right;
    }
    constexpr unsigned kSdfChunks = kRepackX / 16;
    for (unsigned i = tid; i < 8u * 8u * kSdfChunks; i += 256u) {
      const unsigned row = i / kSdfChunks, c = i % kSdfChunks;
      const int ry = (int)(row & 7u), rz = (int)(row >> 3);
      const int y = y0 + ry, z = z0 + rz;
      uint4 v = uint4{0u, 0u, 0u, 0u};
      if (y < a.Y && z < a.Z) v = *reinterpret_cast<const uint4 *>(a.sdf + ((size_t)z * (size_t)a.Y + (size_t)y) * (size_t)a.X + (size_t)x0 + 16u * c);
      *reinterpret_cast<uint4 *>(&s_sdf[rz][ry][16 * (int)c]) = v;
    }
  } else {
    constexpr unsigned kRX = kRepackX + 2;
    for (unsigned i = tid; i < 10u * 10u * kRX; i += 256u) {
      const int rx = (int)(i % kRX), ry = (int)((i / kRX) % 10u), rz = (int)(i / (10u * kRX));
      const int x = x0 - 1 + rx, y = y0 - 1 + ry, z = z0 - 1 + rz;
      int16_t v = 0;
      if ((unsigned)x < (unsigned)a.X && (unsigned)y < (unsigned)a.Y && (unsigned)z < (unsigned)a.Z)
        v = a.volume[((size_t)z * (size_t)a.Y + (size_t)y) * (size_t)a.X + (size_t)x];
      s_val[rz][ry][kRepackX0 - 1 + rx] = v;
    }
    for (unsigned i = tid; i < 8u * 8u * (unsigned)kRepackX; i += 256u) {
      const int rx = (int)(i % (unsigned)kRepackX), ry = (int)((i / (unsigned)kRepackX) % 8u), rz = (int)(i / (8u * (unsigned)kRepackX));
      const int x = x0 + rx, y = y0 + ry, z = z0 + rz;
      int8_t v = 0;
      if (x < a.X && y < a.Y && z < a.Z) v = a.sdf[((size_t)z * (size_t)a.Y + (size_t)y) * (size_t)a.X + (size_t)x];
      s_sdf[rz][ry][rx] = v;
    }
  }
  __syncthreads();
  const unsigned wave = tid >> 6, lane = tid & 63u;
  const size_t brick_row = ((size_t)blockIdx.z * (size_t)a.NBY + (size_t)blockIdx.y) * (size_t)a.NBX;
  for (unsigned half = 0u; half < 2u; ++half) {
   const unsigned sub = wave + 4u * half;
   unsigned ix, iy, iz;
   VolumePacked::inner_coords(sub * 64u + lane, ix, iy, iz);
   const int ly = (int)iy, lz = (int)iz, y = y0 + ly, z = z0 + lz;
   for (unsigned bq = 0u; bq < (unsigned)(kRepackX / 8); ++bq) {
    const int bx = (int)blockIdx.x * (kRepackX / 8) + (int)bq;
    if (bx >= a.NBX) break;
    const int lx = (int)(bq * 8u + ix);
    const int x = x0 + lx;
    uint2 r = uint2{0u, 0u};
    uint8_t q = 0u;
    bool record_read = false;
    uint32_t free_min = 255u;
    if (x < a.X && y < a.Y && z < a.Z) {
      const int cx = kRepackX0 + lx;
      const int value = s_val[lz + 1][ly + 1][cx];
      const int sd = s_sdf[lz][ly][lx];
      const int dx = s_val[lz + 1][ly + 1][cx + 1] - s_val[lz + 1][ly + 1][cx - 1];
      const int dy = s_val[lz + 1][ly + 2][cx] - s_val[lz + 1][ly][cx];
      const int dz = s_val[lz + 2][ly + 1][cx] - s_val[lz][ly + 1][cx];
      int gradient = 0;
      if (a.tf.uses_gradient) {
        const float gx = (float)dx, gy = (float)dy, gz = (float)dz;
        gradient = (int)(short)f2i(sqrtf((gx * gx + gy * gy) + gz * gz));
      }
      unsigned cls = a.cls_in ? a.cls_in[((size_t)z * (size_t)a.Y + (size_t)y) * (size_t)a.X + (size_t)x] : 0u;
      bool maybe = cls != 0u, decided = a.cls_in != nullptr;
      for (int k = 0; k < a.tf.n; ++k) {
        const TfRuleDev &rule = a.tf.rules[k];
        const bool in_window = value >= rule.v_lo && value <= rule.v_hi;
        bool m = in_window;
        if (rule.flags & TF_USE_GRADIENT) m = m && gradient >= rule.g_lo && gradient <= rule.g_hi;
        maybe = maybe || (!decided && in_window);
        if (!decided && m && cls == 0u) cls = (unsigned)k + 1u;
        decided = decided || m || (rule.flags & TF_TERMINAL) != 0;
      }
      r = VolumePacked::pack_hit(dx, dy, dz, cls);
      q = (uint8_t)((cls ? 0x80u : 0u) | (uint32_t)(sd > 0 ? sd : 0));
      free_min = (maybe || sd <= 0) ? 0u : (uint32_t)sd;
      record_read = maybe;
    }
    const size_t out = ((brick_row + (size_t)bx) << 9) + sub * 64u + lane;
    if (__ballot(record_read) != 0ull) a.grec[out] = r;
    a.stepb[out] = q;
    free_min = wave_min_u32(free_min);
    if (lane == 0u) atomicMin(&a.brick_min[brick_row + (size_t)bx], free_min);
   }
  }
}

__global__ __launch_bounds__(256) void k_macro_table(const uint32_t *__restrict__ brick_min, int NBX, int NBY, int NBZ,
                                                     uint2 *__restrict__ macro, int MNX, int MNY, int MNZ, int shift) {
  const int c = (int)(blockIdx.x * blockDim.x + threadIdx.x);
  if (c >= MNX * MNY * MNZ) return;
  const int cx = c % MNX, cy = (c / MNX) % MNY, cz = c / (MNX * MNY);
  uint32_t m = 255u;
  const int bpc = 1 << (shift - 3);
  for (int bz = cz * bpc; bz <= min(cz * bpc + bpc - 1, NBZ - 1); ++bz)
    for (int by = cy * bpc; by <= min(cy * bpc + bpc - 1, NBY - 1); ++by)
      for (int bx = cx * bpc; bx <= min(cx * bpc + bpc - 1, NBX - 1); ++bx)
        m = min(m, brick_min[((size_t)bz * (size_t)NBY + (size_t)by) * (size_t)NBX + (size_t)bx]);
  if (m < kCertMinStep) m = 0u;
  m *= 0x01010101u;
  macro[c] = make_uint2(m, m);
}

__device__ __forceinline__ uint2 min_bytes(uint2 a, uint2 b) {
  uint2 r;
  r.x = r.y = 0u;
  for (int k = 0; k < 32; k += 8) {
    r.x |= min((a.x >> k) & 0xFFu, (b.x >> k) & 0xFFu) << k;
    r.y |= min((a.y >> k) & 0xFFu, (b.y >> k) & 0xFFu) << k;
  }
  return r;
}
__global__ __launch_bounds__(64) void k_macro_octants(uint2 *__restrict__ macro, int MNX, int MNY, int MNZ, int axis) {
  const int n[3] = {MNX, MNY, MNZ};
  const int len = n[axis], u_n = n[(axis + 1) % 3], v_n = n[(axis + 2) % 3];
  const int line = (int)(blockIdx.x * blockDim.x + threadIdx.x);
  if (line >= u_n * v_n) return;
  int c[3];
  c[(axis + 1) % 3] = line % u_n;
  c[(axis + 2) % 3] = line / u_n;
  const uint2 neg = axis == 0 ? make_uint2(0xFF00FF00u, 0xFF00FF00u) : (axis == 1 ? make_uint2(0xFFFF0000u, 0xFFFF0000u) : make_uint2(0u, 0xFFFFFFFFu));
  auto at = [&](int i) -> uint2 & {
    c[axis] = i;
    return macro[((size_t)c[2] * (size_t)MNY + (size_t)c[1]) * (size_t)MNX + (size_t)c[0]];
  };
  uint2 run = make_uint2(0xFFFFFFFFu, 0xFFFFFFFFu);
  for (int i = len - 1; i >= 0; --i) {
    const uint2 v = at(i);
    run = min_bytes(run, v);
    at(i) = make_uint2((v.x & neg.x) | (run.x & ~neg.x), (v.y & neg.y) | (run.y & ~neg.y));
  }
  run = make_uint2(0xFFFFFFFFu, 0xFFFFFFFFu);
  for (int i = 0; i < len; ++i) {
    const uint2 v = at(i);
    run = min_bytes(run, v);
    at(i) = make_uint2((v.x & ~neg.x) | (run.x & neg.x), (v.y & ~neg.y) | (run.y & neg.y));
  }
}
__global__ __launch_bounds__(256) void k_macro_bounds(uint2 *__restrict__ macro, int MNX, int MNY, int MNZ) {
  const int c = (int)(blockIdx.x * blockDim.x + threadIdx.x);
  if (c >= MNX * MNY * MNZ) return;
  const uint2 v = macro[c];
  uint2 r = make_uint2(0u, 0u);
  for (int o = 0; o < 8; ++o) {
    uint32_t m = ((o < 4 ? v.x : v.y) >> ((o & 3) * 8)) & 0xFFu;
    if (m == 255u) m = 0u;
    if (o < 4) r.x |= m << (o * 8); else r.y |= m << ((o - 4) * 8);
  }
  macro[c] = r;
}
__global__ __launch_bounds__(256) void k_macro_hints(uint2 *__restrict__ macro, int MNX, int MNY, int MNZ) {
  const int c = (int)(blockIdx.x * blockDim.x + threadIdx.x);
  if (c >= MNX * MNY * MNZ) return;
  const int cx = c % MNX, cy = (c / MNX) % MNY, cz = c / (MNX * MNY);
  const uint8_t *bytes = reinterpret_cast<const uint8_t *>(macro);
  const uint2 v = macro[c];
  uint2 r = v;
  for (int o = 0; o < 8; ++o) {
    const uint32_t m = ((o < 4 ? v.x : v.y) >> ((o & 3) * 8)) & 0xFFu;
    if (m != 0u && !(m & kCertRefused)) continue;
    const int sx = (o & 1) ? -1 : 1, sy = (o & 2) ? -1 : 1, sz = (o & 4) ? -1 : 1;
    uint32_t g = 1u;
    for (; g < 127u; ++g) {
      const int x = cx + sx * (int)g, y = cy + sy * (int)g, z = cz + sz * (int)g;
      if ((unsigned)x >= (unsigned)MNX || (unsigned)y >= (unsigned)MNY || (unsigned)z >= (unsigned)MNZ) break;
      const uint32_t n = bytes[((((size_t)z * (size_t)MNY + (size_t)y) * (size_t)MNX + (size_t)x) << 3) | (size_t)o];
      if (n != 0u && !(n & kCertRefused)) break;
    }
    const uint32_t e = kCertRefused | g;
    if (o < 4) r.x = (r.x & ~(0xFFu << (o * 8))) | (e << (o * 8)); else r.y = (r.y & ~(0xFFu << ((o - 4) * 8))) | (e << ((o - 4) * 8));
  }
  macro[c] = r;
}

hipError_t launch_repack(const RepackArgs &a, hipStream_t s) {
  const dim3 grid(((unsigned)a.NBX + (unsigned)(kRepackX / 8) - 1u) / (unsigned)(kRepackX / 8), (unsigned)a.NBY, (unsigned)a.NBZ);
  hipLaunchKernelGGL(k_repack, grid, dim3(256), 0, s, a);
  return hipGetLastError();
}
hipError_t launch_macro_table(const uint32_t *brick_min, int NBX, int NBY, int NBZ, uint8_t *macro8, int X, int Y, int Z, int shift, hipStream_t s) {
  const int M = 1 << shift;
  const int MNX = (X + M - 1) >> shift, MNY = (Y + M - 1) >> shift, MNZ = (Z + M - 1) >> shift;
  uint2 *macro = reinterpret_cast<uint2 *>(macro8);
  const unsigned n = (unsigned)(MNX * MNY * MNZ);
  hipLaunchKernelGGL(k_macro_table, dim3((n + 255u) / 256u), dim3(256), 0, s, brick_min, NBX, NBY, NBZ, macro, MNX, MNY, MNZ, shift);
  const int lines[3] = {MNY * MNZ, MNZ * MNX, MNX * MNY};
  for (int axis = 0; axis < 3; ++axis)
    hipLaunchKernelGGL(k_macro_octants, dim3(((unsigned)lines[axis] + 63u) / 64u), dim3(64), 0, s, macro, MNX, MNY, MNZ, axis);
  hipLaunchKernelGGL(k_macro_bounds, dim3((n + 255u) / 256u), dim3(256), 0, s, macro, MNX, MNY, MNZ);
  hipLaunchKernelGGL(k_macro_hints, dim3((n + 255u) / 256u), dim3(256), 0, s, macro, MNX, MNY, MNZ);
  return hipGetLastError();
}

}
```

### cl_volume_renderer_amd/ffi.py

```python
from __future__ import annotations

import ctypes as C
import os

import numpy as np

_HERE = os.path.dirname(os.path.abspath(__file__))
LIB_PATH = os.environ.get("CLWH_LIBRARY") or os.path.join(_HERE, "libclwhip.so")

OK = 0
ELEM_S8, ELEM_S16, ELEM_S32, ELEM_U8, ELEM_U16, ELEM_U32, ELEM_F32 = range(7)
ARG_MEM, ARG_I32, ARG_U32, ARG_F32, ARG_I64, ARG_U64, ARG_F64 = range(7)
ACCUM_VOXEL_CACHE, ACCUM_IMAGE_SPACE = 0, 1
DERIVED_SCENE, DERIVED_CAMERA, DERIVED_PROJECTION = 1, 2, 4
PROJ_MAX, PROJ_MIN, PROJ_MEAN = 0, 1, 2
PROJ_DENSE = 1
COMP_DENSE, COMP_SHADE = 1, 2
ISO_DENSE, ISO_BELOW = 1, 2
SLICE_MAX, SLICE_MIN, SLICE_MEAN = 0, 1, 2
SLICE_DENSE = 1
MESH_DENSE, MESH_BELOW = 1, 2
GROW_26, GROW_FROM_MASK, GROW_DENSE = 1, 2, 4
GROW_MAX_SEEDS = 65536
MASK_INVERT = 1
SHADE_LIGHT, SHADE_AO = 0, 1
TIMERS = ("bounce", "primary", "fixup", "resolve", "repack", "ao")
MAX_SEEDS = 64
TF_MAX_RULES = 16

_ELEM_OF_DTYPE = {
    np.dtype(np.int8): ELEM_S8, np.dtype(np.int16): ELEM_S16, np.dtype(np.int32): ELEM_S32,
    np.dtype(np.uint8): ELEM_U8, np.dtype(np.uint16): ELEM_U16, np.dtype(np.uint32): ELEM_U32,
    np.dtype(np.float32): ELEM_F32,
}


class ClwhError(RuntimeError):
    def __init__(self, status, where):
        self.status = status
        name = lib().clwh_strerror(status).decode()
        super().__init__("%s failed: %s (hip error %d)" % (where, name, lib().clwh_last_hip_error()))


class _ArgValue(C.Union):
    _fields_ = [("mem", C.c_void_p), ("i32", C.c_int32), ("u32", C.c_uint32), ("f32", C.c_float),
                ("i64", C.c_int64), ("u64", C.c_uint64), ("f64", C.c_double)]


class Arg(C.Structure):
    _fields_ = [("kind", C.c_int32), ("reserved", C.c_int32), ("v", _ArgValue)]


class TfRule(C.Structure):
    _fields_ = [("v_lo", C.c_int32), ("v_hi", C.c_int32), ("g_lo", C.c_int32), ("g_hi", C.c_int32),
                ("use_gradient", C.c_int32), ("writes_color", C.c_int32), ("terminal", C.c_int32),
                ("color", C.c_int32 * 4)]


class Tf(C.Structure):
    _fields_ = [("n", C.c_int32), ("rules", TfRule * TF_MAX_RULES)]

    def as_tuples(self):
        return [(r.v_lo, r.v_hi, r.g_lo, r.g_hi, r.use_gradient, r.writes_color, r.terminal, tuple(r.color))
                for r in list(self.rules)[: self.n]]


class RenderDesc(C.Structure):
    _fields_ = [
        ("frame", C.c_void_p), ("volume", C.c_void_p), ("sdf", C.c_void_p), ("env", C.c_void_p),
        ("buffer_volume", C.c_void_p),
        ("cam_pos", C.c_float * 3), ("cam_dir", C.c_float * 3), ("seed", C.c_int32),
        ("width", C.c_uint32), ("height", C.c_uint32),
        ("accum_mode", C.c_int32), ("accum", C.c_void_p),
        ("tile_rank", C.c_int32), ("tile_world", C.c_int32),
        ("write_frame", C.c_int32),
        ("hit_index", C.c_void_p), ("contrib", C.c_void_p),
        ("n_seeds", C.c_int32), ("seeds", C.c_int32 * 64),
        ("shading", C.c_int32), ("resolve_only", C.c_int32),
    ]


class ProjectionDesc(C.Structure):
    _fields_ = [
        ("frame", C.c_void_p), ("volume", C.c_void_p),
        ("cam_pos", C.c_float * 3), ("cam_dir", C.c_float * 3),
        ("width", C.c_uint32), ("height", C.c_uint32),
        ("mode", C.c_int32), ("flags", C.c_int32),
        ("step", C.c_float), ("t_near", C.c_float), ("t_far", C.c_float),
        ("window_center", C.c_float), ("window_width", C.c_float),
        ("values", C.c_void_p), ("t_extreme", C.c_void_p),
    ]


class CompositeDesc(C.Structure):
    _fields_ = [
        ("frame", C.c_void_p), ("volume", C.c_void_p),
        ("cam_pos", C.c_float * 3), ("cam_dir", C.c_float * 3),
        ("width", C.c_uint32), ("height", C.c_uint32),
        ("flags", C.c_int32),
        ("step", C.c_float), ("t_near", C.c_float), ("t_far", C.c_float),
        ("lut", C.c_void_p), ("lut_first", C.c_int32), ("lut_len", C.c_int32),
        ("alpha_stop", C.c_float), ("ambient", C.c_float),
        ("rgba", C.c_void_p), ("t_first", C.c_void_p), ("t_stop", C.c_void_p),
    ]


class IsosurfaceDesc(C.Structure):
    _fields_ = [
        ("frame", C.c_void_p), ("volume", C.c_void_p),
        ("cam_pos", C.c_float * 3), ("cam_dir", C.c_float * 3),
        ("width", C.c_uint32), ("height", C.c_uint32),
        ("flags", C.c_int32),
        ("step", C.c_float), ("t_near", C.c_float), ("t_far", C.c_float),
        ("iso", C.c_float), ("refine", C.c_int32),
        ("color", C.c_float * 3), ("ambient", C.c_float),
        ("t_hit", C.c_void_p), ("normal", C.c_void_p),
    ]


class SliceDesc(C.Structure):
    _fields_ = [
        ("frame", C.c_void_p), ("volume", C.c_void_p),
        ("origin", C.c_float * 3), ("du", C.c_float * 3), ("dv", C.c_float * 3), ("normal", C.c_float * 3),
        ("width", C.c_uint32), ("height", C.c_uint32),
        ("mode", C.c_int32), ("flags", C.c_int32),
        ("slab_samples", C.c_int32), ("step", C.c_float),
        ("window_center", C.c_float), ("window_width", C.c_float),
        ("values", C.c_void_p), ("t_extreme", C.c_void_p),
    ]


class MeshDesc(C.Structure):
    _fields_ = [
        ("volume", C.c_void_p),
        ("iso", C.c_float), ("flags", C.c_int32),
        ("box_lo", C.c_uint32 * 3), ("box_hi", C.c_uint32 * 3),
        ("positions", C.c_void_p), ("normals", C.c_void_p), ("keys", C.c_void_p), ("triangles", C.c_void_p),
        ("vertex_capacity", C.c_uint64), ("triangle_capacity", C.c_uint64),
        ("n_vertices", C.POINTER(C.c_uint64)), ("n_triangles", C.POINTER(C.c_uint64)),
    ]


class GrowResult(C.Structure):
    _fields_ = [
        ("count", C.c_uint64),
        ("bbox_lo", C.c_uint32 * 3), ("bbox_hi", C.c_uint32 * 3),
        ("sum", C.c_int64), ("sum_sq", C.c_uint64),
        ("vmin", C.c_int32), ("vmax", C.c_int32),
        ("rounds", C.c_uint32), ("reserved", C.c_uint32),
    ]

    def as_dict(self):
        return {"count": int(self.count), "bbox_lo": tuple(self.bbox_lo), "bbox_hi": tuple(self.bbox_hi), "sum": int(self.sum),
                "sum_sq": int(self.sum_sq), "vmin": int(self.vmin), "vmax": int(self.vmax)}


class GrowDesc(C.Structure):
    _fields_ = [
        ("volume", C.c_void_p), ("mask", C.c_void_p),
        ("lo", C.c_int32), ("hi", C.c_int32), ("flags", C.c_int32),
        ("n_seeds", C.c_uint32), ("seeds", C.POINTER(C.c_uint32)),
        ("box_lo", C.c_uint32 * 3), ("box_hi", C.c_uint32 * 3),
        ("result", C.POINTER(GrowResult)),
    ]


class ApplyMaskDesc(C.Structure):
    _fields_ = [
        ("volume_in", C.c_void_p), ("volume_out", C.c_void_p), ("mask", C.c_void_p),
        ("fill", C.c_int32), ("flags", C.c_int32),
    ]


_SIZE3 = C.POINTER(C.c_size_t)
_PROTOTYPES = [
    ("clwh_ctx_create", C.c_int, [C.c_int, C.POINTER(C.c_void_p)]),
    ("clwh_ctx_create_on_stream", C.c_int, [C.c_int, C.c_void_p, C.POINTER(C.c_void_p)]),
    ("clwh_ctx_destroy", C.c_int, [C.c_void_p]),
    ("clwh_ctx_finish", C.c_int, [C.c_void_p]),
    ("clwh_ctx_stream", C.c_void_p, [C.c_void_p]),
    ("clwh_ctx_device", C.c_int, [C.c_void_p]),
    ("clwh_mem_create", C.c_int, [C.c_void_p, C.c_size_t, C.c_int, C.POINTER(C.c_void_p)]),
    ("clwh_mem_wrap", C.c_int, [C.c_void_p, C.c_void_p, C.c_size_t, C.POINTER(C.c_void_p)]),
    ("clwh_image_create", C.c_int, [C.c_void_p, _SIZE3, C.c_int, C.c_int, C.c_int, C.POINTER(C.c_void_p)]),
    ("clwh_image_wrap", C.c_int, [C.c_void_p, C.c_void_p, _SIZE3, C.c_int, C.c_int, C.POINTER(C.c_void_p)]),
    ("clwh_mem_push", C.c_int, [C.c_void_p, C.c_void_p, C.c_void_p, C.c_size_t]),
    ("clwh_mem_pull", C.c_int, [C.c_void_p, C.c_void_p, C.c_void_p, C.c_size_t]),
    ("clwh_mem_release", C.c_int, [C.c_void_p]),
    ("clwh_host_register", C.c_int, [C.c_void_p, C.c_size_t]),
    ("clwh_host_unregister", C.c_int, [C.c_void_p]),
    ("clwh_mem_device_ptr", C.c_void_p, [C.c_void_p]),
    ("clwh_mem_size", C.c_size_t, [C.c_void_p]),
    ("clwh_mem_mark_dirty", C.c_int, [C.c_void_p]),
    ("clwh_kernel_get", C.c_int, [C.c_void_p, C.c_char_p, C.c_char_p, C.c_char_p, C.POINTER(C.c_void_p)]),
    ("clwh_kernel_release", C.c_int, [C.c_void_p]),
    ("clwh_launch", C.c_int, [C.c_void_p, _SIZE3, _SIZE3, C.POINTER(Arg), C.c_int]),
    ("clwh_render", C.c_int, [C.c_void_p, C.POINTER(RenderDesc)]),
    ("clwh_cache_len", C.c_int64, [C.c_uint32, C.c_uint32, C.c_uint32]),
    ("clwh_accum_len", C.c_int64, [C.c_uint32, C.c_uint32, C.c_int32]),
    ("clwh_accum_resolve", C.c_int, [C.c_void_p, C.c_void_p, C.c_int32, C.c_uint32, C.c_uint32, C.c_void_p,
                                     C.c_void_p, C.POINTER(C.c_float), C.POINTER(C.c_float)]),
    ("clwh_accum_resolve_tiles", C.c_int, [C.c_void_p, C.c_void_p, C.c_int32, C.c_int32, C.c_uint32, C.c_uint32, C.c_void_p,
                                           C.c_void_p, C.POINTER(C.c_float), C.POINTER(C.c_float)]),
    ("clwh_frame_from_tiles", C.c_int, [C.c_void_p, C.c_void_p, C.c_int32, C.c_uint32, C.c_uint32, C.c_void_p]),
    ("clwh_ctx_invalidate_derived", C.c_int, [C.c_void_p, C.c_int]),
    ("clwh_ctx_scene_info", C.c_int, [C.c_void_p, C.POINTER(C.c_uint64), C.POINTER(C.c_uint64), C.POINTER(C.c_int32)]),
    ("clwh_render_projection", C.c_int, [C.c_void_p, C.POINTER(ProjectionDesc)]),
    ("clwh_render_composite", C.c_int, [C.c_void_p, C.POINTER(CompositeDesc)]),
    ("clwh_render_isosurface", C.c_int, [C.c_void_p, C.POINTER(IsosurfaceDesc)]),
    ("clwh_render_slice", C.c_int, [C.c_void_p, C.POINTER(SliceDesc)]),
    ("clwh_mesh_isosurface", C.c_int, [C.c_void_p, C.POINTER(MeshDesc)]),
    ("clwh_segment_grow", C.c_int, [C.c_void_p, C.POINTER(GrowDesc)]),
    ("clwh_volume_apply_mask", C.c_int, [C.c_void_p, C.POINTER(ApplyMaskDesc)]),
    ("clwh_sdf_build", C.c_int, [C.c_void_p, C.c_void_p, C.c_char_p, C.c_void_p, C.POINTER(C.c_int32)]),
    ("clwh_buffer_reset", C.c_int, [C.c_void_p, C.c_void_p]),
    ("clwh_cache_exchange_plan", C.c_int, [C.c_void_p, C.c_void_p, C.c_uint64, C.POINTER(C.c_void_p)]),
    ("clwh_cache_apply_contributions", C.c_int, [C.c_void_p, C.c_void_p, C.c_void_p, C.c_void_p, C.c_int32]),
    ("clwh_cache_exchange_plan_release", C.c_int, [C.c_void_p]),
    ("clwh_tf_parse", C.c_int, [C.c_char_p, C.POINTER(Tf)]),
    ("clwh_debug_float_conversions", C.c_int, [C.c_void_p, C.c_void_p, C.c_uint64, C.c_void_p, C.c_void_p]),
    ("clwh_debug_wave_min", C.c_int, [C.c_void_p, C.c_void_p, C.c_uint64, C.c_void_p]),
    ("clwh_debug_macro_table", C.c_int, [C.c_void_p, C.c_void_p, C.c_uint64, C.POINTER(C.c_int32)]),
    ("clwh_strerror", C.c_char_p, [C.c_int]),
    ("clwh_last_hip_error", C.c_int, []),
    ("clwh_version", C.c_char_p, []),
    ("clwh_ctx_acquire_from", C.c_int, [C.c_void_p, C.c_void_p]),
    ("clwh_ctx_release_to", C.c_int, [C.c_void_p, C.c_void_p]),
    ("clwh_ctx_set_timing", C.c_int, [C.c_void_p, C.c_int]),
    ("clwh_ctx_timing_read", C.c_int, [C.c_void_p, C.POINTER(C.c_float), C.POINTER(C.c_int32)]),
    ("clwh_ctx_timing_read_all", C.c_int, [C.c_void_p, C.POINTER(C.c_float), C.POINTER(C.c_int32), C.c_int32]),
]
EXPORTED_SYMBOLS = [p[0] for p in _PROTOTYPES]

_lib = None


def lib():
    global _lib
    if _lib is None:
        if not os.path.exists(LIB_PATH):
            raise RuntimeError(
                "libclwhip.so is missing (%s): build it with `python -m cl_volume_renderer_amd.build`; "
                "there is no CPU fallback for the product path" % LIB_PATH)
        L = C.CDLL(LIB_PATH)
        for name, res, args in _PROTOTYPES:
            if not hasattr(L, name) and os.environ.get("CLWH_LIBRARY"):
                continue
            f = getattr(L, name)
            f.restype = res
            f.argtypes = args
        _lib = L
    return _lib


def _check(status, where):
    if status != OK:
        raise ClwhError(status, where)


def parse_tf(source: str) -> Tf:
    tf = Tf()
    _check(lib().clwh_tf_parse(source.encode(), C.byref(tf)), "clwh_tf_parse")
    return tf


def cache_len(X, Y, Z) -> int:
    return int(lib().clwh_cache_len(X, Y, Z))


def accum_len(w, h, world=1) -> int:
    return int(lib().clwh_accum_len(w, h, world))


def _handle(mem):
    return mem.h if mem is not None else None


def _fill_view(d, frame, volume, cam_pos, cam_dir, width, height):
    d.frame, d.volume = frame.h, volume.h
    for k in range(3):
        d.cam_pos[k] = float(cam_pos[k])
        d.cam_dir[k] = float(cam_dir[k])
    d.width, d.height = int(width), int(height)


class Mem:
    def __init__(self, ctx, handle, nbytes, dtype=None, shape=None):
        self.ctx, self.h, self.nbytes, self.dtype, self.shape = ctx, C.c_void_p(handle), nbytes, dtype, shape

    def push(self, arr: np.ndarray):
        a = np.ascontiguousarray(arr)
        _check(lib().clwh_mem_push(self.ctx.h, self.h, a.ctypes.data, a.nbytes), "clwh_mem_push")

    def pull(self, dtype=None, shape=None) -> np.ndarray:
        dtype = np.dtype(dtype or self.dtype or np.uint8)
        out = np.empty(self.nbytes // dtype.itemsize, dtype=dtype)
        _check(lib().clwh_mem_pull(self.ctx.h, self.h, out.ctypes.data, out.nbytes), "clwh_mem_pull")
        shape = shape or self.shape
        return out.reshape(shape) if shape else out

    @property
    def device_ptr(self) -> int:
        return int(lib().clwh_mem_device_ptr(self.h) or 0)

    def release(self):
        if self.h:
            _check(lib().clwh_mem_release(self.h), "clwh_mem_release")
            self.h = None


class Kernel:
    def __init__(self, ctx, handle):
        self.ctx, self.h = ctx, C.c_void_p(handle)

    def launch(self, global_size, local_size, *args):
        g = (C.c_size_t * 3)(*(list(global_size) + [0, 0, 0])[:3])
        l = (C.c_size_t * 3)(*(list(local_size) + [0, 0, 0])[:3])
        arr = (Arg * max(len(args), 1))()
        for i, a in enumerate(args):
            if isinstance(a, Mem):
                arr[i].kind, arr[i].v.mem = ARG_MEM, a.h.value
            elif isinstance(a, (float, np.floating)):
                arr[i].kind, arr[i].v.f32 = ARG_F32, float(a)
            elif isinstance(a, np.unsignedinteger):
                arr[i].kind, arr[i].v.u32 = ARG_U32, int(a)
            elif isinstance(a, (int, np.integer)):
                arr[i].kind, arr[i].v.i32 = ARG_I32, int(a)
            else:
                raise TypeError("unsupported kernel argument %r" % (a,))
        _check(lib().clwh_launch(self.h, g, l, arr, len(args)), "clwh_launch")

    def render(self, *, frame, volume, sdf, env, cam_pos, cam_dir, seed, width, height, buffer_volume=None,
               accum=None, mode=ACCUM_VOXEL_CACHE, tile_rank=0, tile_world=1, write_frame=True,
               hit_index=None, contrib=None, seeds=None, shading=SHADE_LIGHT, resolve_only=False):
        d = RenderDesc()
        d.frame = frame.h if frame is not None else None
        d.volume, d.sdf, d.env = volume.h, sdf.h, env.h
        d.buffer_volume = buffer_volume.h if buffer_volume is not None else None
        for k in range(3):
            d.cam_pos[k] = float(cam_pos[k])
            d.cam_dir[k] = float(cam_dir[k])
        d.seed, d.width, d.height = int(seed), int(width), int(height)
        d.accum_mode = mode
        d.accum = accum.h if accum is not None else None
        d.tile_rank, d.tile_world = tile_rank, tile_world
        d.write_frame = 1 if write_frame else 0
        d.hit_index = hit_index.h if hit_index is not None else None
        d.contrib = contrib.h if contrib is not None else None
        d.shading = shading
        d.resolve_only = 1 if resolve_only else 0
        if seeds is not None:
            d.n_seeds = len(seeds)
            for i, sd in enumerate(seeds):
                d.seeds[i] = int(sd)
        _check(lib().clwh_render(self.h, C.byref(d)), "clwh_render")

    def release(self):
        if self.h:
            _check(lib().clwh_kernel_release(self.h), "clwh_kernel_release")
            self.h = None


class ExchangePlan:
    def __init__(self, ctx, handle):
        self.ctx, self.h = ctx, C.c_void_p(handle)

    def apply(self, buffer_volume: Mem, rgb: Mem, rgb_stride=3):
        _check(lib().clwh_cache_apply_contributions(self.ctx.h, self.h, buffer_volume.h, rgb.h, rgb_stride),
               "clwh_cache_apply_contributions")

    def release(self):
        if self.h:
            _check(lib().clwh_cache_exchange_plan_release(self.h), "clwh_cache_exchange_plan_release")
            self.h = None


class Context:
    def __init__(self, device=0, stream=None):
        h = C.c_void_p()
        if stream is None:
            _check(lib().clwh_ctx_create(device, C.byref(h)), "clwh_ctx_create")
        else:
            _check(lib().clwh_ctx_create_on_stream(device, C.c_void_p(stream), C.byref(h)),
                   "clwh_ctx_create_on_stream")
        self.h = h

    def buffer(self, nbytes, dtype=None, shape=None) -> Mem:
        h = C.c_void_p()
        _check(lib().clwh_mem_create(self.h, nbytes, 0, C.byref(h)), "clwh_mem_create")
        return Mem(self, h.value, nbytes, dtype, shape)

    def buffer_from(self, arr: np.ndarray) -> Mem:
        a = np.ascontiguousarray(arr)
        m = self.buffer(a.nbytes, a.dtype, a.shape)
        m.push(a)
        return m

    def wrap(self, device_ptr: int, nbytes: int, dtype=None, shape=None) -> Mem:
        h = C.c_void_p()
        _check(lib().clwh_mem_wrap(self.h, C.c_void_p(device_ptr), nbytes, C.byref(h)), "clwh_mem_wrap")
        return Mem(self, h.value, nbytes, dtype, shape)

    def image(self, dims, channels, dtype, shape=None) -> Mem:
        dtype = np.dtype(dtype)
        d = (C.c_size_t * 3)(*(list(dims) + [1, 1, 1])[:3])
        h = C.c_void_p()
        _check(lib().clwh_image_create(self.h, d, channels, _ELEM_OF_DTYPE[dtype], 0, C.byref(h)),
               "clwh_image_create")
        n = int(np.prod([max(int(x), 1) for x in list(dims)[:3]])) * channels * dtype.itemsize
        return Mem(self, h.value, n, dtype, shape)

    def image_from(self, arr: np.ndarray, channels=1) -> Mem:
        a = np.ascontiguousarray(arr)
        if channels == 1:
            dims = list(a.shape[::-1])
        else:
            assert a.shape[-1] == channels
            dims = list(a.shape[:-1][::-1])
        m = self.image(dims, channels, a.dtype, a.shape)
        m.push(a)
        return m

    def kernel(self, file: str, entry: str, prepend: str = "") -> Kernel:
        h = C.c_void_p()
        _check(lib().clwh_kernel_get(self.h, file.encode(), entry.encode(), prepend.encode(), C.byref(h)),
               "clwh_kernel_get")
        return Kernel(self, h.value)

    def sdf_build(self, volume: Mem, tf_source: str, sdf: Mem) -> int:
        n = C.c_int32(0)
        _check(lib().clwh_sdf_build(self.h, volume.h, tf_source.encode(), sdf.h, C.byref(n)), "clwh_sdf_build")
        return n.value

    def buffer_reset(self, buffer_volume: Mem):
        _check(lib().clwh_buffer_reset(self.h, buffer_volume.h), "clwh_buffer_reset")

    def exchange_plan(self, entries: Mem, n: int) -> "ExchangePlan":
        h = C.c_void_p()
        _check(lib().clwh_cache_exchange_plan(self.h, entries.h, int(n), C.byref(h)), "clwh_cache_exchange_plan")
        return ExchangePlan(self, h.value)

    def accum_resolve(self, accum_all: Mem, tile_world, width, height, frame: Mem, env: Mem, cam_pos, cam_dir):
        p = (C.c_float * 3)(*[float(x) for x in cam_pos])
        d = (C.c_float * 3)(*[float(x) for x in cam_dir])
        _check(lib().clwh_accum_resolve(self.h, accum_all.h, tile_world, width, height, frame.h, env.h, p, d),
               "clwh_accum_resolve")

    def accum_resolve_tiles(self, accum: Mem, tile_rank, tile_world, width, height, tiles_rgba8: Mem, env: Mem, cam_pos, cam_dir):
        p = (C.c_float * 3)(*[float(x) for x in cam_pos])
        d = (C.c_float * 3)(*[float(x) for x in cam_dir])
        _check(lib().clwh_accum_resolve_tiles(self.h, accum.h, tile_rank, tile_world, width, height, tiles_rgba8.h, env.h, p, d),
               "clwh_accum_resolve_tiles")

    def frame_from_tiles(self, tiles_all: Mem, tile_world, width, height, frame: Mem):
        _check(lib().clwh_frame_from_tiles(self.h, tiles_all.h, tile_world, width, height, frame.h), "clwh_frame_from_tiles")

    def invalidate_derived(self, scene=True, camera=True, projection=False):
        what = (DERIVED_SCENE if scene else 0) | (DERIVED_CAMERA if camera else 0) | (DERIVED_PROJECTION if projection else 0)
        _check(lib().clwh_ctx_invalidate_derived(self.h, what), "clwh_ctx_invalidate_derived")

    def render_projection(self, frame: Mem, volume: Mem, cam_pos, cam_dir, width, height, mode=PROJ_MAX, step=0.5,
                          window=(0.0, 1.0), t_near=0.0, t_far=float("inf"), values: Mem = None, t_extreme: Mem = None,
                          dense=False):
        d = ProjectionDesc()
        _fill_view(d, frame, volume, cam_pos, cam_dir, width, height)
        d.mode, d.flags = int(mode), PROJ_DENSE if dense else 0
        d.step, d.t_near, d.t_far = float(step), float(t_near), float(t_far)
        d.window_center, d.window_width = float(window[0]), float(window[1])
        d.values = _handle(values)
        d.t_extreme = _handle(t_extreme)
        _check(lib().clwh_render_projection(self.h, C.byref(d)), "clwh_render_projection")

    def render_composite(self, frame: Mem, volume: Mem, cam_pos, cam_dir, width, height, lut: Mem, lut_first, lut_len=None, step=0.5,
                         alpha_stop=0.95, flags=0, ambient=0.3, t_near=0.0, t_far=float("inf"), rgba: Mem = None,
                         t_first: Mem = None, t_stop: Mem = None):
        d = CompositeDesc()
        _fill_view(d, frame, volume, cam_pos, cam_dir, width, height)
        d.flags = int(flags)
        d.step, d.t_near, d.t_far = float(step), float(t_near), float(t_far)
        d.lut = _handle(lut)
        d.lut_first = int(lut_first)
        d.lut_len = int(lut_len if lut_len is not None else (lut.nbytes // 16 if lut is not None else 0))
        d.alpha_stop, d.ambient = float(alpha_stop), float(ambient)
        d.rgba = _handle(rgba)
        d.t_first = _handle(t_first)
        d.t_stop = _handle(t_stop)
        _check(lib().clwh_render_composite(self.h, C.byref(d)), "clwh_render_composite")

    def render_isosurface(self, frame: Mem, volume: Mem, cam_pos, cam_dir, width, height, iso, step=0.5, refine=8, flags=0,
                          color=(1.0, 1.0, 1.0), ambient=0.3, t_near=0.0, t_far=float("inf"), t_hit: Mem = None, normal: Mem = None):
        d = IsosurfaceDesc()
        _fill_view(d, frame, volume, cam_pos, cam_dir, width, height)
        for k in range(3):
            d.color[k] = float(color[k])
        d.flags = int(flags)
        d.step, d.t_near, d.t_far = float(step), float(t_near), float(t_far)
        d.iso, d.refine, d.ambient = float(iso), int(refine), float(ambient)
        d.t_hit = _handle(t_hit)
        d.normal = _handle(normal)
        _check(lib().clwh_render_isosurface(self.h, C.byref(d)), "clwh_render_isosurface")

    def render_slice(self, frame: Mem, volume: Mem, origin, du, dv, normal, width, height, mode=SLICE_MAX, slab_samples=1, step=0.5,
                     window=(0.0, 1.0), flags=0, values: Mem = None, t_extreme: Mem = None):
        d = SliceDesc()
        d.frame, d.volume = frame.h, volume.h
        for k in range(3):
            d.origin[k], d.du[k], d.dv[k], d.normal[k] = float(origin[k]), float(du[k]), float(dv[k]), float(normal[k])
        d.width, d.height = int(width), int(height)
        d.mode, d.flags = int(mode), int(flags)
        d.slab_samples, d.step = int(slab_samples), float(step)
        d.window_center, d.window_width = float(window[0]), float(window[1])
        d.values = _handle(values)
        d.t_extreme = _handle(t_extreme)
        _check(lib().clwh_render_slice(self.h, C.byref(d)), "clwh_render_slice")

    def mesh_isosurface_raw(self, volume: Mem, iso, flags=0, box=None, positions: Mem = None, normals: Mem = None, keys: Mem = None,
                            triangles: Mem = None, vertex_capacity=0, triangle_capacity=0):
        d = MeshDesc()
        nv, nt = C.c_uint64(0), C.c_uint64(0)
        d.volume = _handle(volume)
        d.iso, d.flags = float(iso), int(flags)
        if box is not None:
            for k in range(3):
                d.box_lo[k], d.box_hi[k] = int(box[0][k]), int(box[1][k])
        d.positions = _handle(positions)
        d.normals = _handle(normals)
        d.keys = _handle(keys)
        d.triangles = _handle(triangles)
        d.vertex_capacity, d.triangle_capacity = int(vertex_capacity), int(triangle_capacity)
        d.n_vertices, d.n_triangles = C.pointer(nv), C.pointer(nt)
        status = lib().clwh_mesh_isosurface(self.h, C.byref(d))
        return status, int(nv.value), int(nt.value)

    def mesh_isosurface(self, volume: Mem, iso, flags=0, box=None, normals=True, keys=False):
        status, nv, nt = self.mesh_isosurface_raw(volume, iso, flags, box)
        _check(status, "clwh_mesh_isosurface")
        out_n = np.zeros((nv, 3), np.float32) if normals else None
        out_k = np.zeros((nv,), np.uint64) if keys else None
        if nv == 0:
            return np.zeros((0, 3), np.float32), out_n, np.zeros((0, 3), np.uint32), out_k
        bufs = [self.buffer(nv * 12, np.float32, (nv, 3)), self.buffer(nv * 12, np.float32, (nv, 3)) if normals else None,
                self.buffer(nv * 8, np.uint64, (nv,)) if keys else None, self.buffer(max(nt, 1) * 12, np.uint32, (max(nt, 1), 3))]
        try:
            status, _, _ = self.mesh_isosurface_raw(volume, iso, flags, box, bufs[0], bufs[1], bufs[2], bufs[3], nv, nt)
            _check(status, "clwh_mesh_isosurface")
            return (bufs[0].pull(), bufs[1].pull() if normals else None, bufs[3].pull()[:nt], bufs[2].pull() if keys else None)
        finally:
            for b in bufs:
                if b is not None:
                    b.release()

    def grow_region_raw(self, volume: Mem, seeds, lo, hi, flags=0, box=None, mask: Mem = None):
        d, res = GrowDesc(), GrowResult()
        d.volume, d.mask = _handle(volume), _handle(mask)
        d.lo, d.hi, d.flags = int(lo), int(hi), int(flags)
        if seeds is not None:
            s = np.ascontiguousarray(np.asarray(seeds, dtype=np.uint32).reshape(-1, 3))
            d.n_seeds = len(s)
            d.seeds = s.ctypes.data_as(C.POINTER(C.c_uint32))
        if box is not None:
            for k in range(3):
                d.box_lo[k], d.box_hi[k] = int(box[0][k]), int(box[1][k])
        d.result = C.pointer(res)
        return lib().clwh_segment_grow(self.h, C.byref(d)), res

    def grow_region(self, volume: Mem, seeds, lo, hi, connectivity=6, box=None, mask: Mem = None, from_mask=False, dense=False):
        if connectivity not in (6, 26):
            raise ValueError("connectivity is 6 or 26")
        own = mask is None
        if own:
            from . import scene

            if volume.shape is None or len(volume.shape) != 3:
                raise ValueError("a volume without a [z][y][x] shape (a wrap): pass the mask buffer")
            X, Y, Z = volume.shape[::-1]
            n = scene.mask_words_per_row(X) * Y * Z
            mask = self.buffer(4 * n, np.uint32, (n,))
        flags = (GROW_26 if connectivity == 26 else 0) | (GROW_FROM_MASK if from_mask else 0) | (GROW_DENSE if dense else 0)
        status, res = self.grow_region_raw(volume, seeds, lo, hi, flags, box, mask)
        if status != OK and own:
            mask.release()
        _check(status, "clwh_segment_grow")
        return mask, res

    def apply_mask_raw(self, volume_in: Mem, mask: Mem, volume_out: Mem, fill=-32768, flags=0):
        d = ApplyMaskDesc()
        d.volume_in, d.volume_out, d.mask = _handle(volume_in), _handle(volume_out), _handle(mask)
        d.fill, d.flags = int(fill), int(flags)
        return lib().clwh_volume_apply_mask(self.h, C.byref(d))

    def apply_mask(self, volume: Mem, mask: Mem, out: Mem = None, fill=-32768, invert=False):
        _check(self.apply_mask_raw(volume, mask, out if out is not None else volume, fill, MASK_INVERT if invert else 0),
               "clwh_volume_apply_mask")

    def scene_info(self):
        sid, nb, holders = C.c_uint64(0), C.c_uint64(0), C.c_int32(0)
        _check(lib().clwh_ctx_scene_info(self.h, C.byref(sid), C.byref(nb), C.byref(holders)), "clwh_ctx_scene_info")
        return int(sid.value), int(nb.value), int(holders.value)

    def macro_table(self):
        info = (C.c_int32 * 4)()
        _check(lib().clwh_debug_macro_table(self.h, None, C.c_uint64(0), info), "clwh_debug_macro_table")
        out = np.empty((info[2], info[1], info[0], 8), np.uint8)
        _check(lib().clwh_debug_macro_table(self.h, out.ctypes.data_as(C.c_void_p), C.c_uint64(out.nbytes), info), "clwh_debug_macro_table")
        return out, int(info[3])

    def image_wrap(self, device_ptr: int, dims, channels, dtype, shape=None) -> Mem:
        dtype = np.dtype(dtype)
        d = (C.c_size_t * 3)(*(list(dims) + [1, 1, 1])[:3])
        h = C.c_void_p()
        _check(lib().clwh_image_wrap(self.h, C.c_void_p(device_ptr), d, channels, _ELEM_OF_DTYPE[dtype], C.byref(h)),
               "clwh_image_wrap")
        n = int(np.prod([max(int(x), 1) for x in list(dims)[:3]])) * channels * dtype.itemsize
        return Mem(self, h.value, n, dtype, shape)

    def acquire_from(self, stream: int):
        _check(lib().clwh_ctx_acquire_from(self.h, C.c_void_p(stream)), "clwh_ctx_acquire_from")

    def release_to(self, stream: int):
        _check(lib().clwh_ctx_release_to(self.h, C.c_void_p(stream)), "clwh_ctx_release_to")

    def finish(self):
        _check(lib().clwh_ctx_finish(self.h), "clwh_ctx_finish")

    def set_timing(self, enabled=True):
        _check(lib().clwh_ctx_set_timing(self.h, 1 if enabled else 0), "clwh_ctx_set_timing")

    def timing_read(self):
        ms, n = C.c_float(0), C.c_int32(0)
        _check(lib().clwh_ctx_timing_read(self.h, C.byref(ms), C.byref(n)), "clwh_ctx_timing_read")
        return float(ms.value), int(n.value)

    def timing_read_all(self):
        n = len(TIMERS)
        ms, cnt = (C.c_float * n)(), (C.c_int32 * n)()
        _check(lib().clwh_ctx_timing_read_all(self.h, ms, cnt, n), "clwh_ctx_timing_read_all")
        return {name: (float(ms[i]), int(cnt[i])) for i, name in enumerate(TIMERS)}

    @property
    def stream(self) -> int:
        return int(lib().clwh_ctx_stream(self.h) or 0)

    def destroy(self):
        if self.h:
            _check(lib().clwh_ctx_destroy(self.h), "clwh_ctx_destroy")
            self.h = None
```

### include/clwh.h

```cpp
#ifndef CLWH_H
#define CLWH_H

#include <stddef.h>
#include <stdint.h>

#ifdef __cplusplus
extern "C" {
#endif

typedef struct clwh_ctx clwh_ctx;
typedef struct clwh_mem clwh_mem;
typedef struct clwh_kernel clwh_kernel;

enum clwh_status {
  CLWH_OK = 0,
  CLWH_ERR_INVALID_VALUE = 1,
  CLWH_ERR_NO_DEVICE = 2,
  CLWH_ERR_OUT_OF_MEMORY = 3,
  CLWH_ERR_HIP = 4,
  CLWH_ERR_UNKNOWN_KERNEL = 5,
  CLWH_ERR_TF_UNSUPPORTED = 6,
  CLWH_ERR_BAD_ARGS = 7,
  CLWH_ERR_BAD_NDRANGE = 8,
  CLWH_ERR_SIZE_MISMATCH = 9,
  CLWH_ERR_INTERNAL_OVERFLOW = 10
};

enum clwh_elem_kind {
  CLWH_ELEM_S8 = 0, CLWH_ELEM_S16 = 1, CLWH_ELEM_S32 = 2,
  CLWH_ELEM_U8 = 3, CLWH_ELEM_U16 = 4, CLWH_ELEM_U32 = 5,
  CLWH_ELEM_F32 = 6
};

enum clwh_mem_flags { CLWH_MEM_READ_WRITE = 0, CLWH_MEM_READ_ONLY = 1 };

int clwh_ctx_create(int device, clwh_ctx **out);
int clwh_ctx_create_on_stream(int device, void *hip_stream, clwh_ctx **out);
int clwh_ctx_destroy(clwh_ctx *ctx);
int clwh_ctx_finish(clwh_ctx *ctx);
void *clwh_ctx_stream(clwh_ctx *ctx);
int clwh_ctx_device(clwh_ctx *ctx);

int clwh_mem_create(clwh_ctx *ctx, size_t bytes, int flags, clwh_mem **out);
int clwh_mem_wrap(clwh_ctx *ctx, void *device_ptr, size_t bytes, clwh_mem **out);
int clwh_image_create(clwh_ctx *ctx, const size_t dims[3], int channels, int elem_kind, int flags,
                      clwh_mem **out);
int clwh_image_wrap(clwh_ctx *ctx, void *device_ptr, const size_t dims[3], int channels,
                    int elem_kind, clwh_mem **out);
int clwh_mem_push(clwh_ctx *ctx, clwh_mem *mem, const void *host, size_t bytes);
int clwh_mem_pull(clwh_ctx *ctx, clwh_mem *mem, void *host, size_t bytes);
int clwh_mem_release(clwh_mem *mem);
int clwh_host_register(void *host, size_t bytes);
int clwh_host_unregister(void *host);
void *clwh_mem_device_ptr(clwh_mem *mem);
size_t clwh_mem_size(clwh_mem *mem);
int clwh_mem_mark_dirty(clwh_mem *mem);

int clwh_kernel_get(clwh_ctx *ctx, const char *file, const char *entry, const char *prepend,
                    clwh_kernel **out);
int clwh_kernel_release(clwh_kernel *k);

enum clwh_arg_kind { CLWH_ARG_MEM = 0, CLWH_ARG_I32 = 1, CLWH_ARG_U32 = 2, CLWH_ARG_F32 = 3,
                     CLWH_ARG_I64 = 4, CLWH_ARG_U64 = 5, CLWH_ARG_F64 = 6 };
typedef struct clwh_arg {
  int32_t kind;
  int32_t reserved;
  union {
    clwh_mem *mem;
    int32_t i32;
    uint32_t u32;
    float f32;
    int64_t i64;
    uint64_t u64;
    double f64;
  } v;
} clwh_arg;

int clwh_launch(clwh_kernel *k, const size_t global[3], const size_t local[3], const clwh_arg *args,
                int nargs);

enum clwh_accum_mode {
  CLWH_ACCUM_VOXEL_CACHE = 0,
  CLWH_ACCUM_IMAGE_SPACE = 1
};
enum clwh_shading { CLWH_SHADE_LIGHT = 0, CLWH_SHADE_AO = 1 };
typedef struct clwh_render_desc {
  clwh_mem *frame;
  clwh_mem *volume;
  clwh_mem *sdf;
  clwh_mem *env;
  clwh_mem *buffer_volume;
  float cam_pos[3];
  float cam_dir[3];
  int32_t seed;
  uint32_t width, height;
  int32_t accum_mode;
  clwh_mem *accum;
  int32_t tile_rank, tile_world;
  int32_t write_frame;
  clwh_mem *hit_index;
  clwh_mem *contrib;
  int32_t n_seeds;
  int32_t seeds[64];
  int32_t shading;
  int32_t resolve_only;
} clwh_render_desc;
#define CLWH_MAX_SEEDS 64
int clwh_render(clwh_kernel *render_kernel, const clwh_render_desc *desc);

int64_t clwh_cache_len(uint32_t X, uint32_t Y, uint32_t Z);
int64_t clwh_accum_len(uint32_t width, uint32_t height, int32_t tile_world);
int clwh_accum_resolve(clwh_ctx *ctx, clwh_mem *accum_all_ranks, int32_t tile_world, uint32_t width,
                       uint32_t height, clwh_mem *frame_rgba8, clwh_mem *env, const float cam_pos[3],
                       const float cam_dir[3]);
int clwh_accum_resolve_tiles(clwh_ctx *ctx, clwh_mem *accum, int32_t tile_rank, int32_t tile_world, uint32_t width,
                             uint32_t height, clwh_mem *tiles_rgba8, clwh_mem *env, const float cam_pos[3],
                             const float cam_dir[3]);
int clwh_frame_from_tiles(clwh_ctx *ctx, clwh_mem *tiles_all_ranks, int32_t tile_world, uint32_t width, uint32_t height,
                          clwh_mem *frame_rgba8);
enum clwh_derived { CLWH_DERIVED_SCENE = 1, CLWH_DERIVED_CAMERA = 2, CLWH_DERIVED_PROJECTION = 4 };
int clwh_ctx_invalidate_derived(clwh_ctx *ctx, int what);
int clwh_ctx_scene_info(clwh_ctx *ctx, uint64_t *scene_id, uint64_t *bytes, int32_t *holders);

enum clwh_projection { CLWH_PROJ_MAX = 0, CLWH_PROJ_MIN = 1, CLWH_PROJ_MEAN = 2 };
enum clwh_projection_flags { CLWH_PROJ_DENSE = 1 };
typedef struct clwh_projection_desc {
  clwh_mem *frame;
  clwh_mem *volume;
  float cam_pos[3], cam_dir[3];
  uint32_t width, height;
  int32_t mode, flags;
  float step;
  float t_near, t_far;
  float window_center, window_width;
  clwh_mem *values;
  clwh_mem *t_extreme;
} clwh_projection_desc;
int clwh_render_projection(clwh_ctx *ctx, const clwh_projection_desc *desc);

enum clwh_composite_flags {
  CLWH_COMP_DENSE = 1,
  CLWH_COMP_SHADE = 2
};
typedef struct clwh_composite_desc {
  clwh_mem *frame;
  clwh_mem *volume;
  float cam_pos[3], cam_dir[3];
  uint32_t width, height;
  int32_t flags;
  float step;
  float t_near, t_far;
  clwh_mem *lut;
  int32_t lut_first, lut_len;
  float alpha_stop;
  float ambient;
  clwh_mem *rgba;
  clwh_mem *t_first;
  clwh_mem *t_stop;
} clwh_composite_desc;
int clwh_render_composite(clwh_ctx *ctx, const clwh_composite_desc *desc);

enum clwh_isosurface_flags {
  CLWH_ISO_DENSE = 1,
  CLWH_ISO_BELOW = 2
};
typedef struct clwh_isosurface_desc {
  clwh_mem *frame;
  clwh_mem *volume;
  float cam_pos[3], cam_dir[3];
  uint32_t width, height;
  int32_t flags;
  float step;
  float t_near, t_far;
  float iso;
  int32_t refine;
  float color[3];
  float ambient;
  clwh_mem *t_hit;
  clwh_mem *normal;
} clwh_isosurface_desc;
int clwh_render_isosurface(clwh_ctx *ctx, const clwh_isosurface_desc *desc);

enum clwh_slice_mode { CLWH_SLICE_MAX = 0, CLWH_SLICE_MIN = 1, CLWH_SLICE_MEAN = 2 };
enum clwh_slice_flags { CLWH_SLICE_DENSE = 1 };
typedef struct clwh_slice_desc {
  clwh_mem *frame;
  clwh_mem *volume;
  float origin[3];
  float du[3], dv[3];
  float normal[3];
  uint32_t width, height;
  int32_t mode, flags;
  int32_t slab_samples;
  float step;
  float window_center, window_width;
  clwh_mem *values;
  clwh_mem *t_extreme;
} clwh_slice_desc;
int clwh_render_slice(clwh_ctx *ctx, const clwh_slice_desc *desc);

enum clwh_mesh_flags {
  CLWH_MESH_DENSE = 1,
  CLWH_MESH_BELOW = 2
};
typedef struct clwh_mesh_desc {
  clwh_mem *volume;
  float iso;
  int32_t flags;
  uint32_t box_lo[3], box_hi[3];
  clwh_mem *positions;
  clwh_mem *normals;
  clwh_mem *keys;
  clwh_mem *triangles;
  uint64_t vertex_capacity, triangle_capacity;
  uint64_t *n_vertices, *n_triangles;
} clwh_mesh_desc;
int clwh_mesh_isosurface(clwh_ctx *ctx, const clwh_mesh_desc *desc);

enum clwh_grow_flags {
  CLWH_GROW_26 = 1,
  CLWH_GROW_FROM_MASK = 2,
  CLWH_GROW_DENSE = 4
};
#define CLWH_GROW_MAX_SEEDS 65536
typedef struct clwh_grow_result {
  uint64_t count;
  uint32_t bbox_lo[3], bbox_hi[3];
  int64_t sum;
  uint64_t sum_sq;
  int32_t vmin, vmax;
  uint32_t rounds;
  uint32_t reserved;
} clwh_grow_result;
typedef struct clwh_grow_desc {
  clwh_mem *volume;
  clwh_mem *mask;
  int32_t lo, hi;
  int32_t flags;
  uint32_t n_seeds;
  const uint32_t *seeds;
  uint32_t box_lo[3], box_hi[3];
  clwh_grow_result *result;
} clwh_grow_desc;
int clwh_segment_grow(clwh_ctx *ctx, const clwh_grow_desc *desc);

enum clwh_apply_mask_flags { CLWH_MASK_INVERT = 1 };
typedef struct clwh_apply_mask_desc {
  clwh_mem *volume_in;
  clwh_mem *volume_out;
  clwh_mem *mask;
  int32_t fill;
  int32_t flags;
} clwh_apply_mask_desc;
int clwh_volume_apply_mask(clwh_ctx *ctx, const clwh_apply_mask_desc *desc);

int clwh_sdf_build(clwh_ctx *ctx, clwh_mem *volume, const char *tf_source, clwh_mem *sdf,
                   int32_t *n_launches);

int clwh_buffer_reset(clwh_ctx *ctx, clwh_mem *buffer_volume);

typedef struct clwh_exchange_plan clwh_exchange_plan;
int clwh_cache_exchange_plan(clwh_ctx *ctx, clwh_mem *entries, uint64_t n, clwh_exchange_plan **out);
int clwh_cache_apply_contributions(clwh_ctx *ctx, clwh_exchange_plan *plan, clwh_mem *buffer_volume, clwh_mem *rgb,
                                   int32_t rgb_stride);
int clwh_cache_exchange_plan_release(clwh_exchange_plan *plan);

int clwh_ctx_acquire_from(clwh_ctx *ctx, void *hip_stream);
int clwh_ctx_release_to(clwh_ctx *ctx, void *hip_stream);

#define CLWH_TF_MAX_RULES 16
typedef struct clwh_tf_rule {
  int32_t v_lo, v_hi;
  int32_t g_lo, g_hi;
  int32_t use_gradient;
  int32_t writes_color;
  int32_t terminal;
  int32_t color[4];
} clwh_tf_rule;
typedef struct clwh_tf {
  int32_t n;
  clwh_tf_rule rules[CLWH_TF_MAX_RULES];
} clwh_tf;
int clwh_tf_parse(const char *source, clwh_tf *out);

int clwh_debug_float_conversions(clwh_ctx *ctx, clwh_mem *floats_in, uint64_t n, clwh_mem *i32_out, clwh_mem *u32_out);
int clwh_debug_wave_min(clwh_ctx *ctx, clwh_mem *u32_in, uint64_t n, clwh_mem *u32_out);
int clwh_debug_macro_table(clwh_ctx *ctx, void *host_out, uint64_t capacity, int32_t info_out[4]);
const char *clwh_strerror(int status);
int clwh_last_hip_error(void);
const char *clwh_version(void);
int clwh_ctx_set_timing(clwh_ctx *ctx, int enabled);
int clwh_ctx_timing_read(clwh_ctx *ctx, float *total_ms, int32_t *launches);
enum clwh_timer {
  CLWH_TIMER_BOUNCE = 0,
  CLWH_TIMER_PRIMARY = 1,
  CLWH_TIMER_FIXUP = 2,
  CLWH_TIMER_RESOLVE = 3,
  CLWH_TIMER_REPACK = 4,
  CLWH_TIMER_AO = 5,
  CLWH_TIMER_COUNT = 6
};
int clwh_ctx_timing_read_all(clwh_ctx *ctx, float *ms, int32_t *launches, int32_t n);

#ifdef __cplusplus
}
#endif
#endif
```

Measured before the change: 42150.

## Add per-voxel start-certificate table to skip marching for bounce rays that escape

Builds a per-voxel byte table at scene-pack time (row ballots plus Y/Z prefix scans, gated by a regularity check on the step field). For each octant it records whether a ray starting there can reach the volume boundary without meeting a surface event. The primary kernel stores this mask in the hit record, and the bounce kernel uses it together with a minimum direction-component bound to send qualifying bounce rays straight to the exit event without marching. This adds one volume-sized byte table and extra repack kernels, and adds a gather in the primary hit path. Correctness rests on the conservative certificate, which can be checked with a stats verification mode.

```diff
diff --git a/cl_volume_renderer_amd/csrc/bounce_device.hpp b/cl_volume_renderer_amd/csrc/bounce_device.hpp
--- a/cl_volume_renderer_amd/csrc/bounce_device.hpp
+++ b/cl_volume_renderer_amd/csrc/bounce_device.hpp
@@ -63,6 +63,12 @@
   const bool leaves = T * fabsf(d.x) >= fx || T * fabsf(d.y) >= fy || T * fabsf(d.z) >= fz;
   return box_min != 0 && budget > 5 && leaves && dmin >= 0.0009765625f && dsum == dsum;
 }
+__device__ __forceinline__ bool start_certificate(uint32_t mask, f3 d, float dmin_needed) {
+  const unsigned octant = (d.x < 0.0f ? 1u : 0u) | (d.y < 0.0f ? 2u : 0u) | (d.z < 0.0f ? 4u : 0u);
+  const float dmin = fminf(fminf(fabsf(d.x), fabsf(d.y)), fabsf(d.z));
+  const float dsum = d.x + d.y + d.z;
+  return ((mask >> octant) & 1u) != 0u && dmin >= dmin_needed && dsum == dsum;
+}
 __device__ __forceinline__ bool certify_exit(const RenderArgs &a, f3 p, f3 d, int budget) {
   int away;
   return certify_exit(a, p, d, budget, away);
@@ -88,8 +94,10 @@
 
 #ifdef CLVR_BOUNCE_STATS
 constexpr bool kBounceStats = true;
+constexpr bool kStartCertVerify = (CLVR_BOUNCE_STATS + 0) != 2;
 #else
 constexpr bool kBounceStats = false;
+constexpr bool kStartCertVerify = false;
 #endif
 template <bool ON> struct BounceStatsT;
 template <> struct BounceStatsT<false> {
@@ -101,6 +109,8 @@
   __device__ void refill(uint32_t) {}
   __device__ void fresh_items(int, int) {}
   __device__ void swap_point() {}
+  __device__ void start_cert(bool, bool) {}
+  __device__ void march_end(uint32_t *, int) {}
   template <bool TWO_RAYS> __device__ void flush(uint32_t *) {}
 };
 template <> struct BounceStatsT<true> {
@@ -136,6 +146,16 @@
     if (closing + n_fresh != 0u) event_phases += 1;
   }
   __device__ __forceinline__ void swap_point() { swaps += 1; }
+  uint32_t start_tried = 0, start_granted = 0;
+  bool start_open = false;
+  __device__ __forceinline__ void start_cert(bool tried, bool granted) {
+    start_tried += (uint32_t)__popcll(__ballot(tried)); start_granted += (uint32_t)__popcll(__ballot(granted));
+    start_open = start_open || granted;
+  }
+  __device__ __forceinline__ void march_end(uint32_t *counters, int ev) {
+    if (start_open && ev != EV_EXIT) atomicAdd(&counters[CTR_START_WRONG], 1u);
+    start_open = false;
+  }
   template <bool TWO_RAYS> __device__ __forceinline__ void flush(uint32_t *counters) {
     atomicAdd(&counters[CTR_STEP_ITERS], step_iters); atomicAdd(&counters[CTR_STEP_LANES], step_lanes);
     atomicAdd(&counters[CTR_EVENT_PHASES], event_phases); atomicAdd(&counters[CTR_EVENT_LANES], event_lanes);
@@ -144,6 +164,7 @@
     for (int k = 0; k < 4; ++k) atomicAdd(&counters[CTR_EV_KIND + k], ev_kind[k]);
     atomicAdd(&counters[CTR_CERT_PHASES], cert_phases); atomicAdd(&counters[CTR_CERT_LANES], cert_lanes);
     atomicAdd(&counters[CTR_CERT_GRANTED], cert_granted); atomicAdd(&counters[CTR_STEP_IDLE], step_idle);
+    atomicAdd(&counters[CTR_START_TRIED], start_tried); atomicAdd(&counters[CTR_START_GRANTED], start_granted);
   }
 };
 using BounceStats = BounceStatsT<kBounceStats>;
diff --git a/cl_volume_renderer_amd/csrc/clwh_context.hip b/cl_volume_renderer_amd/csrc/clwh_context.hip
--- a/cl_volume_renderer_amd/csrc/clwh_context.hip
+++ b/cl_volume_renderer_amd/csrc/clwh_context.hip
@@ -151,6 +151,7 @@
   if (const char *e = std::getenv("CLWH_TUNE_SDFBIT_REC")) t.sdfbit_rec_lds = std::strcmp(e, "lds") == 0 ? 1 : 0;
   if (const char *e = std::getenv("CLWH_TUNE_CERT")) t.cert_min_step = clamped(e, 0, 127);
   if (const char *e = std::getenv("CLWH_TUNE_CERT_HINT")) t.cert_hint = std::atoi(e) != 0;
+  if (const char *e = std::getenv("CLWH_TUNE_START_CERT")) t.start_cert = std::atoi(e) != 0;
   return t;
 }
 
diff --git a/cl_volume_renderer_amd/csrc/clwh_host.hpp b/cl_volume_renderer_amd/csrc/clwh_host.hpp
--- a/cl_volume_renderer_amd/csrc/clwh_host.hpp
+++ b/cl_volume_renderer_amd/csrc/clwh_host.hpp
@@ -93,6 +93,7 @@
   TfDev tf{};
   std::string tf_identity;
   int32_t macro_shift = 0;
+  bool start_table = false;
   int32_t dims[3] = {0, 0, 0};
   uint64_t generation = 0;
   Event ready;
@@ -115,6 +116,7 @@
   int32_t unit_block_log2 = 4;
   int32_t unit_group = 1, unit_affinity = 0, unit_queues = 8;
   int32_t cert_hint = 1;
+  int32_t start_cert = 1;
   int32_t cert_min_step = -1;
   uint32_t bounce_max_blocks = 2048;
   int32_t sdfbit_waves = 8;
diff --git a/cl_volume_renderer_amd/csrc/clwh_internal.hpp b/cl_volume_renderer_amd/csrc/clwh_internal.hpp
--- a/cl_volume_renderer_amd/csrc/clwh_internal.hpp
+++ b/cl_volume_renderer_amd/csrc/clwh_internal.hpp
@@ -32,7 +32,8 @@
   int32_t entry_hi;
   uint32_t xy;
   uint32_t pslot;
-  uint32_t pad[2];
+  uint32_t start_free;
+  uint32_t pad;
 };
 static_assert(sizeof(HitRec) == 64, "HitRec must be one 64-byte line");
 
@@ -46,7 +47,9 @@
   CTR_STEP_ITERS = 8, CTR_STEP_LANES, CTR_EVENT_PHASES, CTR_EVENT_LANES, CTR_REFILLS, CTR_REFILL_LANES,
   CTR_EV_KIND,
   CTR_CERT_PHASES = CTR_EV_KIND + 4, CTR_CERT_LANES, CTR_CERT_GRANTED,
-  CTR_SWAPS, CTR_STEP_IDLE, CTR_STATS_END,
+  CTR_SWAPS, CTR_STEP_IDLE,
+  CTR_START_TRIED, CTR_START_GRANTED, CTR_START_WRONG,
+  CTR_STATS_END,
   CTR_QUEUE_STRIDE = 32,
 };
 struct RenderArgs {
@@ -60,6 +63,8 @@
   int32_t cert_min_step;
   int32_t cert_min_lanes;
   int32_t cert_hint;
+  const uint8_t *start_free;
+  float start_cert_dmin;
   int32_t NBX, NBY;
   const uint32_t *env;
   int32_t env_w, env_h;
@@ -141,6 +146,27 @@
   return shift;
 }
 hipError_t launch_macro_table(const uint32_t *brick_min, int NBX, int NBY, int NBZ, uint8_t *macro, int X, int Y, int Z, int shift, hipStream_t s);
+hipError_t launch_start_table(const uint8_t *stepb, uint8_t *table, uint32_t *regular, int X, int Y, int Z, int NBX, int NBY, int NBZ, hipStream_t s);
+inline int start_cert_cap(int X, int Y, int Z) {
+  const int longest = X > Y ? (X > Z ? X : Z) : (Y > Z ? Y : Z);
+  return longest / 2 < 127 ? longest / 2 : 127;
+}
+inline float start_cert_dmin(int X, int Y, int Z) {
+  const double longest = (double)(X > Y ? (X > Z ? X : Z) : (Y > Z ? Y : Z));
+  const double reach = 1.7320508075688772 * (longest + 1.0), cap = (double)start_cert_cap(X, Y, Z);
+  for (int k = 1; k <= 64; ++k) {
+    const double dmin = (double)k / 64.0;
+    double t = 0.0;
+    for (int step = 0; step < 70 - 5 && t <= reach; ++step) {
+      const double m = (double)(long long)(t * dmin) - 2.0;
+      const double bound = m > cap ? cap : m;
+      t += bound < 1.0 ? 1.0 : bound;
+    }
+    if (t > reach) return (float)dmin;
+  }
+  return 2.0f;
+}
+constexpr uint64_t kStartTableBudget = 2ull << 30;
 hipError_t launch_primary(const RenderArgs &a, hipStream_t s);
 hipError_t launch_bounce(const RenderArgs &a, hipStream_t s);
 inline bool bounce_queues_fit(uint32_t n_hits, int32_t unit_block_log2, int32_t n_seeds) {
diff --git a/cl_volume_renderer_amd/csrc/clwh_render.hip b/cl_volume_renderer_amd/csrc/clwh_render.hip
--- a/cl_volume_renderer_amd/csrc/clwh_render.hip
+++ b/cl_volume_renderer_amd/csrc/clwh_render.hip
@@ -19,9 +19,14 @@
 
 struct PackedLayout {
   int X, Y, Z, NBX, NBY, NBZ, mshift, MNX, MNY, MNZ;
-  size_t records, n_bricks, off_stepb, off_brick_min, off_macro, bytes;
+  size_t records, n_bricks, off_stepb, off_brick_min, off_macro, off_start, bytes;
+  bool start_table;
 };
-static PackedLayout packed_layout(const clwh_mem *volume, int forced_macro_shift) {
+static bool wants_start_table(const Tuning &t, const TfDev &tf, const clwh_mem *volume) {
+  return t.start_cert != 0 && tf.uses_gradient == 0 && tf.border_class == 0 && fits_grid_yz(volume) &&
+         (uint64_t)volume->dims[0] * volume->dims[1] * volume->dims[2] <= kStartTableBudget;
+}
+static PackedLayout packed_layout(const clwh_mem *volume, int forced_macro_shift, bool start_table) {
   PackedLayout L;
   L.X = (int)volume->dims[0]; L.Y = (int)volume->dims[1]; L.Z = (int)volume->dims[2];
   L.NBX = (L.X + 7) / 8; L.NBY = (L.Y + 7) / 8; L.NBZ = (L.Z + 7) / 8;
@@ -33,13 +38,15 @@
   L.off_stepb = L.records * sizeof(uint2);
   L.off_brick_min = (L.records * (sizeof(uint2) + 1u) + 15u) & ~(size_t)15u;
   L.off_macro = (L.off_brick_min + L.n_bricks * sizeof(uint32_t) + 15u) & ~(size_t)15u;
-  L.bytes = L.off_macro + (size_t)L.MNX * L.MNY * L.MNZ * 8u;
+  L.off_start = (L.off_macro + (size_t)L.MNX * L.MNY * L.MNZ * 8u + 15u) & ~(size_t)15u;
+  L.start_table = start_table;
+  L.bytes = L.off_start + (start_table ? 16u + (size_t)L.X * L.Y * L.Z : 0u);
   return L;
 }
 
 static bool packed_matches(const PackedScene &p, int device, const PackedLayout &L, const clwh_mem *volume, const clwh_mem *sdf,
                            const TfDev &tf, const std::string &tf_identity) {
-  return !p.stale && p.device == device && p.data.bytes == L.bytes && p.macro_shift == L.mshift && p.vol == volume->dptr &&
+  return !p.stale && p.device == device && p.data.bytes == L.bytes && p.macro_shift == L.mshift && p.start_table == L.start_table && p.vol == volume->dptr &&
          p.sdf == sdf->dptr && p.vol_ver == volume->version() && p.sdf_ver == sdf->version() &&
          !std::memcmp(&p.tf, &tf, sizeof tf) && p.tf_identity == tf_identity;
 }
@@ -95,6 +102,10 @@
     if (e != hipSuccess) return e;
     return launch_macro_table(r.brick_min, L.NBX, L.NBY, L.NBZ, data + L.off_macro, L.X, L.Y, L.Z, L.mshift, ctx->stream);
   }));
+  if (L.start_table)
+    CLWH_TRY(timed(ctx, CLWH_TIMER_REPACK, [&] {
+      return launch_start_table(r.stepb, data + L.off_start + 16u, reinterpret_cast<uint32_t *>(data + L.off_start), L.X, L.Y, L.Z, L.NBX, L.NBY, L.NBZ, ctx->stream);
+    }));
   HIP_TRY(hipEventRecord(entry->ready.ev, ctx->stream));
   ctx->scene = entry;
   {
@@ -106,6 +117,7 @@
     entry->tf = tf;
     entry->tf_identity = tf_identity;
     entry->macro_shift = L.mshift;
+    entry->start_table = L.start_table;
     entry->dims[0] = L.X; entry->dims[1] = L.Y; entry->dims[2] = L.Z;
     entry->generation = ++g_packed_generation;
     entry->stale = false;
@@ -209,6 +221,7 @@
   a.unit_affinity = t.unit_affinity;
   a.unit_queues = t.unit_queues;
   a.cert_hint = t.cert_hint;
+  a.start_cert_dmin = start_cert_dmin(a.X, a.Y, a.Z);
   return CLWH_OK;
 }
 
@@ -217,7 +230,7 @@
   const uint8_t *cls_in = nullptr;
   CLWH_TRY(kernel_tf(k, d->volume, a.tf, &cls_in));
   a.tf.literal_gradient_taps = ctx->tune.literal_gradient;
-  const PackedLayout L = packed_layout(d->volume, ctx->tune.macro_shift);
+  const PackedLayout L = packed_layout(d->volume, ctx->tune.macro_shift, wants_start_table(ctx->tune, a.tf, d->volume));
   CLWH_TRY(ensure_packed(ctx, L, d->volume, d->sdf, a.tf, cls_in, k->jit ? k->jit->source : std::string()));
   const uint8_t *packed = ctx->scene->data.as<uint8_t>();
   a.grec = reinterpret_cast<const uint2 *>(packed);
@@ -227,6 +240,7 @@
   a.volume_lin = (const int16_t *)d->volume->dptr;
   a.sdf_lin = (const int8_t *)d->sdf->dptr;
   a.macro = packed + L.off_macro;
+  a.start_free = L.start_table ? packed + L.off_start + 16u : nullptr;
   a.macro_shift = L.mshift;
   a.MNX = L.MNX; a.MNY = L.MNY; a.MNZ = L.MNZ;
   bool zero_may_hit = a.tf.border_class != 0;
@@ -361,6 +375,9 @@
                h[CTR_EV_KIND + 1], h[CTR_EV_KIND + 2], h[CTR_EV_KIND + 3], h[CTR_CERT_PHASES], per(CTR_CERT_LANES, CTR_CERT_PHASES), h[CTR_CERT_GRANTED]);
   if (h[CTR_SWAPS]) std::fprintf(stderr, "[bounce stats] two rays per lane: %u swap points\n", h[CTR_SWAPS]);
   std::fprintf(stderr, "[bounce stats] per step iteration: avg_idle_lanes=%.2f (lane sum %u)\n", per(CTR_STEP_IDLE, CTR_STEP_ITERS), h[CTR_STEP_IDLE]);
+  std::fprintf(stderr, "[bounce stats] lane_steps=%u event_lanes=%u start certificates (%s) tried/granted/wrong=%u/%u/%u dmin=%.6f\n", h[CTR_STEP_LANES],
+               h[CTR_EVENT_LANES], (CLVR_BOUNCE_STATS + 0) == 2 ? "taken" : "verified: marched literally", h[CTR_START_TRIED], h[CTR_START_GRANTED],
+               h[CTR_START_WRONG], (double)a.start_cert_dmin);
   return CLWH_OK;
 }
 #endif
@@ -502,18 +519,19 @@
   return CLWH_OK;
 }
 
+static PackedLayout scene_layout(clwh_ctx *ctx) {
+  std::lock_guard<std::mutex> lock(g_scenes_mutex);
+  clwh_mem shape{};
+  for (int q = 0; q < 3; ++q) shape.dims[q] = (size_t)ctx->scene->dims[q];
+  return packed_layout(&shape, ctx->scene->macro_shift, ctx->scene->start_table);
+}
+
 int clwh_debug_macro_table(clwh_ctx *ctx, void *host_out, uint64_t capacity, int32_t info_out[4]) {
   if (!ctx || !info_out) return CLWH_ERR_INVALID_VALUE;
   if (!ctx->scene) return CLWH_ERR_BAD_ARGS;
-  PackedLayout L;
-  {
-    std::lock_guard<std::mutex> lock(g_scenes_mutex);
-    clwh_mem shape{};
-    for (int q = 0; q < 3; ++q) shape.dims[q] = (size_t)ctx->scene->dims[q];
-    L = packed_layout(&shape, ctx->scene->macro_shift);
-  }
+  const PackedLayout L = scene_layout(ctx);
   info_out[0] = L.MNX; info_out[1] = L.MNY; info_out[2] = L.MNZ; info_out[3] = L.mshift;
-  const size_t bytes = L.bytes - L.off_macro;
+  const size_t bytes = (size_t)L.MNX * L.MNY * L.MNZ * 8u;
   if (!host_out) return CLWH_OK;
   if (capacity < bytes || ctx->scene->data.bytes != L.bytes) return CLWH_ERR_SIZE_MISMATCH;
   HIP_TRY(hipSetDevice(ctx->device));
@@ -522,4 +540,39 @@
   return CLWH_OK;
 }
 
-}
+int clwh_debug_start_table(clwh_ctx *ctx, void *host_out, uint64_t capacity, int32_t info_out[4]) {
+  if (!ctx || !info_out) return CLWH_ERR_INVALID_VALUE;
+  if (!ctx->scene) return CLWH_ERR_BAD_ARGS;
+  const PackedLayout L = scene_layout(ctx);
+  info_out[0] = L.X; info_out[1] = L.Y; info_out[2] = L.Z; info_out[3] = L.start_table ? 1 : 0;
+  if (!host_out || !L.start_table) return CLWH_OK;
+  const size_t bytes = (size_t)L.X * L.Y * L.Z;
+  if (capacity < bytes || ctx->scene->data.bytes != L.bytes) return CLWH_ERR_SIZE_MISMATCH;
+  HIP_TRY(hipSetDevice(ctx->device));
+  HIP_TRY(hipMemcpyAsync(host_out, ctx->scene->data.as<uint8_t>() + L.off_start + 16u, bytes, hipMemcpyDeviceToHost, ctx->stream));
+  HIP_TRY(hipStreamSynchronize(ctx->stream));
+  return CLWH_OK;
+}
+
+int clwh_debug_start_cert_dmin(int32_t X, int32_t Y, int32_t Z, float *dmin_out) {
+  if (!dmin_out || X < 1 || Y < 1 || Z < 1) return CLWH_ERR_INVALID_VALUE;
+  *dmin_out = start_cert_dmin(X, Y, Z);
+  return CLWH_OK;
+}
+
+int clwh_debug_hit_records(clwh_ctx *ctx, void *host_out, uint64_t capacity, uint32_t *n_hits_out) {
+  if (!ctx || !n_hits_out) return CLWH_ERR_INVALID_VALUE;
+  PrimaryHits &p = ctx->primary;
+  if (!p.valid || !p.hits.ptr || !ctx->pass.counters.ptr) return CLWH_ERR_BAD_ARGS;
+  HIP_TRY(hipSetDevice(ctx->device));
+  HIP_TRY(hipMemcpyAsync(n_hits_out, ctx->pass.counters.as<uint32_t>() + CTR_HITS, sizeof(uint32_t), hipMemcpyDeviceToHost, ctx->stream));
+  HIP_TRY(hipStreamSynchronize(ctx->stream));
+  if (!host_out) return CLWH_OK;
+  const size_t bytes = (size_t)*n_hits_out * sizeof(HitRec);
+  if (capacity < bytes || p.hits.bytes < bytes) return CLWH_ERR_SIZE_MISMATCH;
+  HIP_TRY(hipMemcpyAsync(host_out, p.hits.ptr, bytes, hipMemcpyDeviceToHost, ctx->stream));
+  HIP_TRY(hipStreamSynchronize(ctx->stream));
+  return CLWH_OK;
+}
+
+}
diff --git a/cl_volume_renderer_amd/csrc/primary_kernels.hip b/cl_volume_renderer_amd/csrc/primary_kernels.hip
--- a/cl_volume_renderer_amd/csrc/primary_kernels.hip
+++ b/cl_volume_renderer_amd/csrc/primary_kernels.hip
@@ -58,7 +58,13 @@
     q1.z = __float_as_uint(normal.x); q1.w = __float_as_uint(normal.y);
     q2.x = __float_as_uint(normal.z); q2.y = current_color;
     q2.z = (uint32_t)((uint64_t)entry & 0xFFFFFFFFull); q2.w = (uint32_t)((uint64_t)entry >> 32);
-    q3.x = x | (y << 16); q3.y = pslot; q3.z = 0u; q3.w = 0u;
+    uint32_t start_free = 0u;
+    if (a.start_free) {
+      const f3 p = (current_ray.origin + current_ray.direction) + normal * 2.0f;
+      if (__float_as_uint(p.x) < __float_as_uint(dx) && __float_as_uint(p.y) < __float_as_uint(dy) && __float_as_uint(p.z) < __float_as_uint(dz))
+        start_free = a.start_free[((size_t)(int)p.z * (size_t)a.Y + (size_t)(int)p.y) * (size_t)a.X + (size_t)(int)p.x];
+    }
+    q3.x = x | (y << 16); q3.y = pslot; q3.z = start_free; q3.w = 0u;
     uint4 *dst = reinterpret_cast<uint4 *>(&a.hits[h]);
     dst[0] = q0; dst[1] = q1; dst[2] = q2; dst[3] = q3;
     a.pix_slot[pslot] = PIX_HIT | h;
diff --git a/cl_volume_renderer_amd/csrc/render_kernels.hip b/cl_volume_renderer_amd/csrc/render_kernels.hip
--- a/cl_volume_renderer_amd/csrc/render_kernels.hip
+++ b/cl_volume_renderer_amd/csrc/render_kernels.hip
@@ -31,11 +31,14 @@
   unsigned queue_dry = 0u;
   enum : int { C_START_X, C_START_Y, C_START_Z,
                C_NORMAL_X, C_NORMAL_Y, C_NORMAL_Z,
-               C_ENTRY_LO, C_ENTRY_HI, C_PIXEL, C_HIT, C_SEED,
+               C_ENTRY_LO,
+               C_ENTRY_HI,
+               C_PIXEL, C_HIT, C_SEED,
                C_FIX,
                C_BV_R, C_BV_G, C_BV_B, C_FIELDS };
   __shared__ uint32_t cold[C_FIELDS][kBounceThreads];
 #define COLD(f) cold[f][threadIdx.x]
+#define COLD_ENTRY_HI() ((uint32_t)((int32_t)(COLD(C_ENTRY_HI) << 8) >> 8))
   Ray ray{{0, 0, 0}, {0, 0, 0}};
   float atten = 0.0f, r_energy = 0.0f, g_energy = 0.0f, b_energy = 0.0f;
   uint32_t color = 0u;
@@ -47,6 +50,7 @@
   const bool cert_hint = a.cert_hint != 0;
   const int cert_min_lanes = a.cert_min_lanes;
   const int cert_at = a.cert_min_step != 0 ? a.cert_min_step : kCertNever;
+  const bool start_cert = !USE_GRAD && a.cert_min_step != 0;
   bool exhausted = false;
   BounceStats stats;
 
@@ -120,6 +124,7 @@
           march -= kOneStep;
         }
       }
+      stats.march_end(a.counters, ev);
       bool ended = false;
 
       if (ev == EV_EXIT) {
@@ -141,7 +146,7 @@
               uint32_t *rec = a.fixups + (size_t)slot * kFixupDwords;
               rec[0] = COLD(C_HIT);
               rec[1] = COLD(C_ENTRY_LO);
-              rec[2] = COLD(C_ENTRY_HI);
+              rec[2] = COLD_ENTRY_HI();
               rec[3] = COLD(C_PIXEL);
               rec[4] = COLD(C_BV_R); rec[5] = COLD(C_BV_G); rec[6] = COLD(C_BV_B);
             } else {
@@ -180,7 +185,7 @@
       if (ended && o > 2) {
         const int fix = (int)(COLD(C_FIX) >> 2) - 2;
         if (fix == -1)
-          finish_item<MODE>(a, (int64_t)(((uint64_t)COLD(C_ENTRY_HI) << 32) | (uint64_t)COLD(C_ENTRY_LO)), COLD(C_HIT), COLD(C_PIXEL) & 0xFFFFu,
+          finish_item<MODE>(a, (int64_t)(((uint64_t)COLD_ENTRY_HI() << 32) | (uint64_t)COLD(C_ENTRY_LO)), COLD(C_HIT), COLD(C_PIXEL) & 0xFFFFu,
                             COLD(C_PIXEL) >> 16, COLD(C_BV_R), COLD(C_BV_G), COLD(C_BV_B));
         else if (fix >= 0) a.fixups[(size_t)fix * kFixupDwords + 7] = COLD(C_FIX) & 3u;
         st = ST_IDLE;
@@ -242,7 +247,7 @@
             if (granted) {
               COLD(C_START_X) = __float_as_uint(start.x); COLD(C_START_Y) = __float_as_uint(start.y); COLD(C_START_Z) = __float_as_uint(start.z);
               COLD(C_NORMAL_X) = q1.z; COLD(C_NORMAL_Y) = q1.w; COLD(C_NORMAL_Z) = q2.x;
-              COLD(C_ENTRY_LO) = q2.z; COLD(C_ENTRY_HI) = q2.w;
+              COLD(C_ENTRY_LO) = q2.z; COLD(C_ENTRY_HI) = (q2.w & 0x00FFFFFFu) | (q3.z << 24);
               COLD(C_PIXEL) = q3.x;
               COLD(C_HIT) = h;
               COLD(C_SEED) = (uint32_t)a.seeds[s];
@@ -268,6 +273,7 @@
       continue;
     }
 
+    bool sc_tried = false, sc_granted = false;
     if (st >= ST_EVENT) {
       const int ev = st - ST_EVENT;
       bool start_path = (ev == EV_START);
@@ -313,15 +319,25 @@
         } else {
           atten = d;
           i = 8;
+          if (start_cert) {
+            sc_tried = true;
+            sc_granted = start_certificate(COLD(C_ENTRY_HI) >> 24, nr.direction, a.start_cert_dmin);
+          }
         }
         ray = nr;
       }
 
-      sd = (int)(vol.template step_i<SMALL>(f2i(ray.origin.x), f2i(ray.origin.y), f2i(ray.origin.z)) & 0x7Fu);
-      march = 70u * kOneStep + kCertReady;
-      st = ST_MARCH;
-    }
+      if (sc_granted && !kStartCertVerify) {
+        st = ST_EVENT + EV_EXIT;
+      } else {
+        sd = (int)(vol.template step_i<SMALL>(f2i(ray.origin.x), f2i(ray.origin.y), f2i(ray.origin.z)) & 0x7Fu);
+        march = 70u * kOneStep + kCertReady;
+        st = ST_MARCH;
+      }
+    }
+    stats.start_cert(sc_tried, sc_granted);
   }
+#undef COLD_ENTRY_HI
 #undef COLD
 }
 
diff --git a/cl_volume_renderer_amd/csrc/scene_kernels.hip b/cl_volume_renderer_amd/csrc/scene_kernels.hip
--- a/cl_volume_renderer_amd/csrc/scene_kernels.hip
+++ b/cl_volume_renderer_amd/csrc/scene_kernels.hip
@@ -218,4 +218,82 @@
   return hipGetLastError();
 }
 
-}
+
+__global__ __launch_bounds__(256) void k_start_regular(const uint8_t *__restrict__ stepb, int X, int Y, int Z, int NBX, int NBY, unsigned cap, uint32_t *regular) {
+  const unsigned brick = blockIdx.x;
+  const int bx = (int)(brick % (unsigned)NBX), by = (int)((brick / (unsigned)NBX) % (unsigned)NBY), bz = (int)(brick / (unsigned)(NBX * NBY));
+  auto at = [&](int x, int y, int z) -> unsigned { return stepb[VolumePacked::record_index(x, y, z, NBX, NBY)]; };
+  bool ok = true;
+  for (unsigned inner = threadIdx.x; inner < 512u; inner += 256u) {
+    unsigned ix, iy, iz;
+    VolumePacked::inner_coords(inner, ix, iy, iz);
+    const int x = bx * 8 + (int)ix, y = by * 8 + (int)iy, z = bz * 8 + (int)iz;
+    if (x >= X || y >= Y || z >= Z) continue;
+    const unsigned q = stepb[((size_t)brick << 9) + inner], s = q & 0x7Fu;
+    if (s >= 2u) {
+      unsigned m = 127u;
+      for (int c = 0; c < 8; ++c)
+        m = min(m, at(min(max(x + ((c & 1) ? 1 : -1), 0), X - 1), min(max(y + ((c & 2) ? 1 : -1), 0), Y - 1), min(max(z + ((c & 4) ? 1 : -1), 0), Z - 1)) & 0x7Fu);
+      ok = ok && s >= min(cap, m + 1u);
+    } else {
+      bool touches = false;
+      for (int dz = -1; dz <= 1; ++dz)
+        for (int dy = -1; dy <= 1; ++dy)
+          for (int dx = -1; dx <= 1; ++dx)
+            touches = touches || (at(min(max(x + dx, 0), X - 1), min(max(y + dy, 0), Y - 1), min(max(z + dz, 0), Z - 1)) & 0x80u) != 0u;
+      ok = ok && touches && (s == 1u || (q & 0x80u) != 0u);
+    }
+  }
+  if (!ok) *regular = 0u;
+}
+__global__ __launch_bounds__(256) void k_start_rows(const uint8_t *__restrict__ stepb, uint8_t *__restrict__ table, int X, int Y, int Z, int NBX, int NBY) {
+  const int lane = (int)(threadIdx.x & 63u), y = (int)blockIdx.x * 4 + (int)(threadIdx.x >> 6);
+  if (y >= Y) return;
+  for (int k = 0; k < 4; ++k) {
+    const int z = (int)blockIdx.y * 4 + k;
+    if (z >= Z) break;
+    int first = X, last = -1;
+    for (int x0 = 0; x0 < X; x0 += 64) {
+      const int x = x0 + lane;
+      const unsigned long long ev = __ballot(x < X && (stepb[VolumePacked::record_index(min(x, X - 1), y, z, NBX, NBY)] & 0x80u) != 0u);
+      if (ev != 0ull) {
+        if (first == X) first = x0 + __ffsll((long long)ev) - 1;
+        last = x0 + 63 - __clzll((long long)ev);
+      }
+    }
+    uint8_t *row = table + ((size_t)z * (size_t)Y + (size_t)y) * (size_t)X;
+    for (int x = lane; x < X; x += 64) row[x] = (uint8_t)((x > last ? 0x55u : 0u) | (x < first ? 0xAAu : 0u));
+  }
+}
+__global__ __launch_bounds__(256) void k_start_scan(uint8_t *__restrict__ table, int X, int Y, int Z, int axis, const uint32_t *regular) {
+  const int x = (int)(blockIdx.x * blockDim.x + threadIdx.x), other = (int)blockIdx.y;
+  if (x >= X) return;
+  const int len = axis == 1 ? Y : Z;
+  const size_t stride = axis == 1 ? (size_t)X : (size_t)X * (size_t)Y;
+  uint8_t *line = table + (axis == 1 ? (size_t)other * (size_t)Y * (size_t)X : (size_t)other * (size_t)X) + (size_t)x;
+  const unsigned up = axis == 1 ? 0x33u : 0x0Fu;
+  const unsigned keep = (regular == nullptr || *regular != 0u) ? 0xFFu : 0u;
+  unsigned run = 0xFFu;
+  for (int i = len - 1; i >= 0; --i) {
+    const unsigned v = line[(size_t)i * stride];
+    run &= v;
+    line[(size_t)i * stride] = (uint8_t)((v & ~up) | (run & up));
+  }
+  run = 0xFFu;
+  for (int i = 0; i < len; ++i) {
+    const unsigned v = line[(size_t)i * stride];
+    run &= v;
+    line[(size_t)i * stride] = (uint8_t)(((v & up) | (run & ~up)) & keep);
+  }
+}
+hipError_t launch_start_table(const uint8_t *stepb, uint8_t *table, uint32_t *regular, int X, int Y, int Z, int NBX, int NBY, int NBZ, hipStream_t s) {
+  hipError_t e = hipMemsetAsync(regular, 1, sizeof(uint32_t), s);
+  if (e != hipSuccess) return e;
+  hipLaunchKernelGGL(k_start_regular, dim3((unsigned)(NBX * NBY * NBZ)), dim3(256), 0, s, stepb, X, Y, Z, NBX, NBY, (unsigned)start_cert_cap(X, Y, Z), regular);
+  hipLaunchKernelGGL(k_start_rows, dim3(((unsigned)Y + 3u) / 4u, ((unsigned)Z + 3u) / 4u), dim3(256), 0, s, stepb, table, X, Y, Z, NBX, NBY);
+  hipLaunchKernelGGL(k_start_scan, dim3(((unsigned)X + 255u) / 256u, (unsigned)Z), dim3(256), 0, s, table, X, Y, Z, 1, (const uint32_t *)nullptr);
+  hipLaunchKernelGGL(k_start_scan, dim3(((unsigned)X + 255u) / 256u, (unsigned)Y), dim3(256), 0, s, table, X, Y, Z, 2, (const uint32_t *)regular);
+  return hipGetLastError();
+}
+
+}
diff --git a/cl_volume_renderer_amd/ffi.py b/cl_volume_renderer_amd/ffi.py
--- a/cl_volume_renderer_amd/ffi.py
+++ b/cl_volume_renderer_amd/ffi.py
@@ -221,6 +221,9 @@
     ("clwh_debug_float_conversions", C.c_int, [C.c_void_p, C.c_void_p, C.c_uint64, C.c_void_p, C.c_void_p]),
     ("clwh_debug_wave_min", C.c_int, [C.c_void_p, C.c_void_p, C.c_uint64, C.c_void_p]),
     ("clwh_debug_macro_table", C.c_int, [C.c_void_p, C.c_void_p, C.c_uint64, C.POINTER(C.c_int32)]),
+    ("clwh_debug_start_table", C.c_int, [C.c_void_p, C.c_void_p, C.c_uint64, C.POINTER(C.c_int32)]),
+    ("clwh_debug_start_cert_dmin", C.c_int, [C.c_int32, C.c_int32, C.c_int32, C.POINTER(C.c_float)]),
+    ("clwh_debug_hit_records", C.c_int, [C.c_void_p, C.c_void_p, C.c_uint64, C.POINTER(C.c_uint32)]),
     ("clwh_strerror", C.c_char_p, [C.c_int]),
     ("clwh_last_hip_error", C.c_int, []),
     ("clwh_version", C.c_char_p, []),
@@ -262,6 +265,12 @@
     tf = Tf()
     _check(lib().clwh_tf_parse(source.encode(), C.byref(tf)), "clwh_tf_parse")
     return tf
+
+
+def start_cert_dmin(X: int, Y: int, Z: int) -> float:
+    v = C.c_float(0)
+    _check(lib().clwh_debug_start_cert_dmin(X, Y, Z, C.byref(v)), "clwh_debug_start_cert_dmin")
+    return float(v.value)
 
 
 def cache_len(X, Y, Z) -> int:
@@ -605,6 +614,22 @@
         _check(lib().clwh_debug_macro_table(self.h, out.ctypes.data_as(C.c_void_p), C.c_uint64(out.nbytes), info), "clwh_debug_macro_table")
         return out, int(info[3])
 
+    def start_table(self):
+        info = (C.c_int32 * 4)()
+        _check(lib().clwh_debug_start_table(self.h, None, C.c_uint64(0), info), "clwh_debug_start_table")
+        if not info[3]:
+            return None
+        out = np.empty((info[2], info[1], info[0]), np.uint8)
+        _check(lib().clwh_debug_start_table(self.h, out.ctypes.data_as(C.c_void_p), C.c_uint64(out.nbytes), info), "clwh_debug_start_table")
+        return out
+
+    def hit_records(self):
+        n = C.c_uint32(0)
+        _check(lib().clwh_debug_hit_records(self.h, None, C.c_uint64(0), C.byref(n)), "clwh_debug_hit_records")
+        out = np.empty((int(n.value), 16), np.uint32)
+        _check(lib().clwh_debug_hit_records(self.h, out.ctypes.data_as(C.c_void_p), C.c_uint64(out.nbytes), C.byref(n)), "clwh_debug_hit_records")
+        return out[:int(n.value)]
+
     def image_wrap(self, device_ptr: int, dims, channels, dtype, shape=None) -> Mem:
         dtype = np.dtype(dtype)
         d = (C.c_size_t * 3)(*(list(dims) + [1, 1, 1])[:3])
diff --git a/include/clwh.h b/include/clwh.h
--- a/include/clwh.h
+++ b/include/clwh.h
@@ -286,6 +286,9 @@
 int clwh_debug_float_conversions(clwh_ctx *ctx, clwh_mem *floats_in, uint64_t n, clwh_mem *i32_out, clwh_mem *u32_out);
 int clwh_debug_wave_min(clwh_ctx *ctx, clwh_mem *u32_in, uint64_t n, clwh_mem *u32_out);
 int clwh_debug_macro_table(clwh_ctx *ctx, void *host_out, uint64_t capacity, int32_t info_out[4]);
+int clwh_debug_start_table(clwh_ctx *ctx, void *host_out, uint64_t capacity, int32_t info_out[4]);
+int clwh_debug_start_cert_dmin(int32_t X, int32_t Y, int32_t Z, float *dmin_out);
+int clwh_debug_hit_records(clwh_ctx *ctx, void *host_out, uint64_t capacity, uint32_t *n_hits_out);
 const char *clwh_strerror(int status);
 int clwh_last_hip_error(void);
 const char *clwh_version(void);
```

Result: faster. 42850 (median of 6 runs) (+1.7%).
